# KyleKWKim/LLM-guided-Multimodal-MIL

Hardware: AMD Instinct MI355X
Metric: bags/sec fwd+bwd, N=1024 patches D=512 (higher is better)
Workload: dtype f32; 1 GPU; 32 bags/GPU x 1024 patches x 512 dims, image-only gated-attention MIL fwd+BCE+bwd+allreduce+Adam (BASELINE config 2; x1 GPUs = 32 bags); bags_per_gpu=32, patches=1024, dim=512, global_bags=32, parallelism=dp1, mode=train (dropout 0.5 on patches + 0.25 before the head, in-kernel masks), accum=1, batches_cycled=4, launch=eager

## Files before the change

### include/mil_hip.h

```cpp
#ifndef MIL_HIP_H
#define MIL_HIP_H

#include <stddef.h>
#include <stdint.h>

#ifdef __cplusplus
extern "C" {
#endif

#define MIL_OK 0
#define MIL_EINVAL (-22)
#define MIL_ENOSPC (-28)

#define MIL_GATE_D 192
#define MIL_POOL_TILE 32
#define MIL_LOSS_BCE 0
#define MIL_LOSS_CE_ON_SIGMOID 1
#define MIL_SMALL_ROWS 64

int mil_abi_version(void);

int mil_dropout_keep_bits(uint32_t* bits, int rows, int cols, float p_drop, uint64_t seed, uint64_t offset,
                          const int32_t* offset_dev, void* stream);
int mil_dropout_keep_bits_pair(uint32_t* xbits, int R, uint32_t* mbits, int B, int L, uint64_t seed, uint64_t mseed,
// ... 264 lines not shown
int mil_attn_seq_bwd(const float* q, const float* k, const float* v, int ld, const float* o, const float* dout,
                     const float* lse, const int32_t* q_off, int B, int Tmax, int H, int C, int causal, float* dq,
                     float* dk, float* dv, int ldd, void* stream);
int mil_quickgelu(const float* x, const float* dy, float* out, size_t n, void* stream);
int mil_absorb_query(const float* qp, const float* Wk, int B, int H, int C, int E, float* Qp, void* stream);
int mil_absorb_query_pad(const float* qp, const float* Wk, int B, int H, int C, int E, int T, int THp, float scale,
                         const float* bias, float* Qp, float* cb, void* stream);
int mil_absorb_query_bwd_pad(const float* qp, const float* Wk, const float* dQp, int B, int H, int C, int E, int T, int THp,
                             float scale, const float* bias, const float* dcb, float* dqp, float* dWk, float* dbias,
                             void* stream);
int mil_absorb_query_bwd(const float* qp, const float* Wk, const float* dQp, int B, int H, int C, int E, float* dqp,
                         float* dWk, void* stream);
int mil_absorbed_pool_fwd(const float* keys, const float* pe, const float* Qp, const int32_t* k_off,
                          const int32_t* tile_map, const int32_t* bag_tile_off, int ntiles, int B, int H, int C, int E,
                          float* pooled, float* lse, float* workspace, void* stream);
int mil_absorbed_pool_attn(const float* keys, const float* pe, const float* Qp, const float* lse, const int32_t* k_off,
                           const int32_t* tile_map, int ntiles, int B, int H, int C, int E, float* attn, void* stream);
int mil_absorbed_pool_bwd(const float* keys, const float* pe, const float* Qp, const float* lse, const float* dpooled,
                          const float* pooled, const int32_t* k_off, const int32_t* tile_map,
                          const int32_t* bag_tile_off, int ntiles, int n_keys, int B, int H, int C, int E,
                          const float* dkeys_acc, float* dkeys, float* dQp, float* workspace, void* stream);
int mil_lnbr_absorbed_pool_value_fwd(const float* x, const float* o, const float* gamma, const float* beta, float eps,
                                     const float* pe, const float* Qp, const int32_t* k_off, const int32_t* tile_map,
                                     const int32_t* bag_tile_off, int ntiles, int B, int H, int C, int E, const float* Wv,
                                     const float* bv, float* y, float* stats, float* pooled, float* lse, float* o_attn,
                                     float* workspace, void* stream);
int mil_lnbr_absorbed_pool_bwd(const float* x, const float* o, const float* gamma, const float* beta, const float* stats, const float* y,
                               const float* pe, const float* Qp, const float* lse, const float* dpooled, const float* pooled,
                               const int32_t* k_off, const int32_t* tile_map, const int32_t* bag_tile_off, int ntiles,
                               int n_keys, int B, int H, int C, int E, const float* dy_acc, float* dx, float* d_o,
                               float* dgamma, float* dbeta, float* dQp, float* workspace, void* stream);
int mil_value_proj(const float* pooled, const float* Wv, const float* bv, int B, int H, int C, int E, float* o,
                   void* stream);
int mil_value_proj_pad(const float* pooled, const float* Wv, const float* bv, int B, int H, int C, int E, int T, int THp,
                       float* o, void* stream);
int mil_absorbed_pool_value_fwd(const float* keys, const float* pe, const float* Qp, const int32_t* k_off,
                                const int32_t* tile_map, const int32_t* bag_tile_off, int ntiles, int B, int H, int C, int E,
                                const float* Wv, const float* bv, float* pooled, float* lse, float* o, float* workspace,
                                void* stream);
int mil_value_proj_bwd(const float* dO, const float* Wv, const float* pooled, int B, int H, int C, int E, float* dpooled,
                       float* dWv, float* dbv, void* stream);
int mil_grp_col_softmax(float* S, int ld, const int32_t* grp_off, int G, int max_group_rows, int TH, void* stream);
int mil_grp_col_softmax_bwd(const float* A, const float* dA, int ld, const int32_t* grp_off, int G, int max_group_rows,
                            int TH, float* dS, void* stream);
size_t mil_grp_col_softmax_workspace_floats(int G, int max_group_rows, int ld);
int mil_grp_col_softmax_ws(float* S, int ld, const int32_t* grp_off, int G, int max_group_rows, int TH, float* ws, void* stream);
int mil_grp_col_softmax_bwd_ws(const float* A, const float* dA, int ld, const int32_t* grp_off, int G, int max_group_rows,
                               int TH, float* dS, float* ws, void* stream);
int mil_row_softmax_t(float* S, int ld, int R, int T, int H, void* stream);
int mil_row_softmax_t_bwd(const float* A, const float* dA, int ld, int R, int T, int H, float* dS, void* stream);

int mil_layernorm_fwd(const float* x, const float* gamma, const float* beta, int rows, int E, float eps, float* y,
                      float* stats, void* stream);
int mil_layernorm_bwd_blocks(int rows);
int mil_layernorm_bwd(const float* x, const float* gamma, const float* dy, const float* stats, int rows, int E,
                      float* dx, float* dgamma, float* dbeta, float* workspace, void* stream);
int mil_layernorm_bwd_res(const float* x, const float* gamma, const float* dy, const float* stats, const float* dres,
                          int rows, int E, float* dx, float* dgamma, float* dbeta, float* workspace, void* stream);

int mil_layernorm_bagrow_fwd(const float* x, const float* o, const int32_t* row_bag, const float* gamma, const float* beta,
                             int rows, int E, float eps, float* y, float* stats, void* stream);
int mil_layernorm_bagrow_bwd(const float* x, const float* o, const int32_t* row_bag, const int32_t* row_off, int B,
                             const float* gamma, const float* dy, const float* stats, int rows, int E, float* dx, float* d_o,
                             float* dgamma, float* dbeta, float* workspace, void* stream);
int mil_layernorm_bagrow_rows_per_block(int rows);

int mil_add_pe(const float* x, const float* pe, const int32_t* row_bag, const int32_t* row_off, int rows, int E,
               float* out, void* stream);
int mil_add_bag_row(const float* x, const float* o, const int32_t* row_bag, int rows, int E, float* out,
                    void* stream);
int mil_segment_colsum(const float* Y, const int32_t* row_off, int B, int max_rows, int E, float* out,
                       float* workspace, void* stream);
int mil_ct_map_tokens(const float* ct, int B, int C, int D, int HW, int reduce, float* out, void* stream);
int mil_sinusoid_pe(float* pe, int n, int E, void* stream);

int mil_embed_tokens(const int64_t* ids, const float* table, const float* pos, int nseq, int ctx, int W,
                     float* out, void* stream);
int mil_gather_eot(const int64_t* ids, const float* x, int nseq, int ctx, int W, float* out, void* stream);

int mil_adam_step(float* param, const float* grad, float* exp_avg, float* exp_avg_sq, size_t n,
                  int step, float lr, float beta1, float beta2, float eps, float weight_decay,
                  float grad_scale, void* stream);
int mil_adam_step_counted(float* param, const float* grad, float* exp_avg, float* exp_avg_sq, size_t n,
                          int32_t* step_counter, float lr, float beta1, float beta2, float eps, float weight_decay,
                          float grad_scale, void* stream);
int mil_adam_step_counted_noinc(float* param, const float* grad, float* exp_avg, float* exp_avg_sq, size_t n,
                                const int32_t* step_counter, float lr, float beta1, float beta2, float eps,
                                float weight_decay, float grad_scale, void* stream);

int mil_adam_step_dev(float* param, const float* grad, float* exp_avg, float* exp_avg_sq, size_t n, int32_t* step_counter,
                      const float* lr_dev, float beta1, float beta2, float eps, float weight_decay, float grad_scale,
                      int inc, void* stream);
#define MIL_ADAM_MAX_SEGS 8
int mil_adam_step_dev_segs(float* param, const float* grad, float* exp_avg, float* exp_avg_sq, const size_t* seg_begin,
                           const size_t* seg_end, int nseg, int32_t* step_counter, const float* lr_dev,
                           int32_t* done_counter, float beta1, float beta2, float eps, float weight_decay, float grad_scale,
                           int inc, void* stream);

int mil_sgd_step(float* param, const float* grad, size_t n, float lr, float weight_decay, float grad_scale,
                 void* stream);

#define MIL_STAGE_DROPBITS 0x01u
#define MIL_STAGE_GATE_FWD 0x02u
#define MIL_STAGE_POOL     0x04u
#define MIL_STAGE_TAIL     0x08u
#define MIL_STAGE_GATE_BWD 0x10u
#define MIL_STAGE_REDUCE   0x20u
#define MIL_STAGE_ADAM     0x40u
#define MIL_STAGE_TILEMAP  0x80u
#define MIL_STAGE_ALL      0xffu
#define MIL_STAGE_POOL_FUSED 0x100u
typedef struct mil_image_only_step {
    uint32_t struct_bytes;
    uint32_t stages;
    const void* x;
    const float* y;
    const int32_t* tile_map;
    const int32_t* bag_tile_off;
    int32_t R, L, B, C, T;
    const int32_t* bag_len_dev;
    int32_t* rows_dev;
    int32_t x_bf16;
    float loss_scale;
    int32_t loss_kind;
    int32_t accumulate;
    const float *Wv, *bv, *Wu, *bu, *w, *b, *Wf, *bf;
    const uint16_t *Wv16, *Wu16;
    float *dWv, *dbv, *dWu, *dbu, *dw, *db, *dWf, *dbf;
    float* loss_out;
    float* scores;
    float* gates;
    uint16_t* gates16;
    float* partials;
    float* hrow;
    float* ds;
    float* dw_ws;
    uint64_t dw_ws_floats;
    float *M, *Mdrop, *lse, *logits, *prob, *loss_bag, *dz, *dM, *cdot;
    int32_t train;
    int32_t bf16_grad_mfma;
    uint32_t* xbits;
    uint32_t* mbits;
    uint64_t seed, offset;
    const int32_t* offset_dev;
    float *param_flat, *grad_flat, *exp_avg, *exp_avg_sq;
    uint64_t n_param;
    int32_t adam_step;
    int32_t* adam_step_dev;
    float lr, beta1, beta2, eps, weight_decay, grad_scale;
    const float* lr_dev;
    float* tail_ws;
    int32_t* done_dev;
    const uint16_t* Wp;
} mil_image_only_step;

int mil_image_only_step_run(const mil_image_only_step* a, void* stream);
int mil_image_only_step_time(const mil_image_only_step* a, uint32_t stages, int warm, int iters, float* ms_out,
                             void* stream);

#define MIL_ROUTE_MAIN_R32 0
#define MIL_ROUTE_MAIN_FWD2 1
#define MIL_ROUTE_MAIN_FWD2_PW 2
#define MIL_ROUTE_MAIN_LEGACY 3
#define MIL_ROUTE_TAIL_NONE 0
#define MIL_ROUTE_TAIL_SMALL 1
#define MIL_ROUTE_TAIL_BIG 2
#define MIL_ROUTE_TAIL_KERNEL_NONE 0
#define MIL_ROUTE_TAIL_KERNEL_LINEAR_SMALL 1
#define MIL_ROUTE_TAIL_KERNEL_R32 2
#define MIL_ROUTE_BITS_NONE 0
#define MIL_ROUTE_BITS_GIVEN 1
#define MIL_ROUTE_BITS_IN_KERNEL 2
#define MIL_ROUTE_BITS_GENERATOR 3
#define MIL_ROUTE_DW_KG1 0
#define MIL_ROUTE_DW_KG2 1
#define MIL_ROUTE_DW2 2
typedef struct mil_gate_route {
    int32_t main, rt;
    int32_t tail, tail_rows, tail_kernel, tail_rt;
    int32_t bits, pool_fused;
    int32_t dw, S, kc;
} mil_gate_route;
int mil_gate_step_route(int R, int L, int C, int save_gates, int keep, int pieces, int fused_pool, int bucketed, int ncu,
                        mil_gate_route* out);

#define MIL_GEMM_KERNEL_NT2 0
#define MIL_GEMM_KERNEL_G64 1
#define MIL_GEMM_KERNEL_G64N 2
#define MIL_GEMM_KERNEL_TAIL 3
#define MIL_GEMM_KERNEL_NT 4
#define MIL_GEMM_KERNEL_NN 5
#define MIL_GEMM_KERNEL_TN 6
#define MIL_GEMM_KERNEL_TN2 7
#define MIL_GEMM_KERNEL_TN_AX 8
typedef struct mil_gemm_plan {
    int32_t kernel, S, kchunk;
    int32_t rows_main, main_kernel;
    int32_t rows_honoured;
    uint64_t workspace_floats;
} mil_gemm_plan;
int mil_gemm_route(int M, int N, int K, int a_mode, int b_mode, int lda, int ldb, int ldc, int act, int has_residual,
                   int accumulate, int aux_mode, int has_workspace, int bucketed, int aligned16, int ncu, mil_gemm_plan* out);
int mil_linear_bwd_params_route(int rows, int n_out, int k_in, int lddy, int ldy, int ldx, int aligned16, int ncu,
                                mil_gemm_plan* out);

int mil_cosine_embedding_loss(const float* x1, const float* x2, int B, int E, float scale, float* loss, float* dx1,
                              float* dx2, void* stream);

int mil_build_fusion_segs(const int32_t* len_dev, int B, int P, int cap, int32_t* k_off, int32_t* k_bag, int32_t* tile64,
                          int32_t* bag_tile64_off, int T64, int32_t* tile32, int32_t* bag_tile32_off, int T32,
                          int32_t* row_bag, int32_t* rows_out, float* ds_zero, void* stream);

int mil_build_fusion_segs_tail(const int32_t* len_dev, int B, int nseg, const int32_t* seg_rows, int cap, int32_t* k_off,
                               int32_t* k_bag, int32_t* tile64, int32_t* bag_tile64_off, int T64, int32_t* tile32,
                               int32_t* bag_tile32_off, int T32, int32_t* row_bag, int32_t* rows_out, float* ds_zero,
                               void* stream);

int mil_image_only_step_profile(const mil_image_only_step* a, const uint32_t* groups, int ngroups, int warm, int iters,
                                float* ms_out, void* stream);
int mil_image_only_step_profile_rot(const mil_image_only_step* a, const void* const* xs, const float* const* ys, int nrot,
                                    const uint32_t* groups, int ngroups, int warm, int iters, float* ms_out, void* stream);

int mil_tm_bgemm(const float* A, long sAb, long sAi, long sAk, const float* B, long sBb, long sBk, long sBj, float* C, long sCb,
                 long sCi, long sCj, const float* D, int batch, int M, int N, int K, float alpha, float beta, float diag, int splits,
                 void* stream);
int mil_tm_softmax_rows(float* x, long rows, int cols, void* stream);
int mil_tm_softmax_rows_bwd(const float* p, float* dp, long rows, int cols, void* stream);
int mil_tm_row_gather(const float* src, const float* extra, const int32_t* idx, int rows, int E, float* dst, void* stream);
int mil_tm_row_gather_bwd(const float* ddst, const int32_t* idx, int rows, int E, float* dsrc, float* dextra, void* stream);
int mil_tm_seq_index(const int32_t* len_dev, int B, const int32_t* s_of_bag, int32_t* idx_out, int idx_rows, int32_t* rows_dev_out,
                     int32_t* flag_dev, float* x_tail, int x_rows, int L, void* stream);
int mil_tm_seq_index_segs(const int32_t* table_dev, int B, int total, int x_rows, int32_t* idx_out, int idx_rows, int32_t* flag_dev,
                          void* stream);
int mil_tm_landmarks(const float* qkv, int n_pad, float qscale, float* qL, float* kL, void* stream);
int mil_tm_landmarks_bwd(const float* dqL, const float* dkL, int n_pad, float qscale, float* dqkv, void* stream);
int mil_tm_pinv_init(const float* A2, float* scale, int32_t* arg, float* Z0, void* stream);
int mil_tm_pinv_init_bwd(const float* dZ0, const float* Z0, const float* scale, const int32_t* arg, float* dA2, float* ws,
                         void* stream);
int mil_tm_resconv(const float* qkv, const float* w, int n_pad, float* out, void* stream);
int mil_tm_resconv_bwd(const float* dout, const float* qkv, const float* w, int n_pad, float* dqkv, float* dw, void* stream);
int mil_tm_ppeg_fwd(const float* x, int s, const float* W7, const float* b7, const float* W5, const float* b5, const float* W3,
                    const float* b3, float* y, void* stream);
int mil_tm_ppeg_bwd(const float* dy, const float* x, int s, const float* W7, const float* W5, const float* W3, float* dx,
                    float* dWf, float* db, void* stream);
int mil_tm_cls_attn(const float* A1, const float* Z, const float* A3, int n_pad, int pad, int s, int n, const int32_t* len_dev,
                    int bag, float* t_ws, float* out, void* stream);
size_t mil_tm_lmk_attn_ws_floats(int n_pad, int backward);
int mil_tm_lmk_attn_fwd(const float* qkv, const float* qL, int n_pad, float* W, float* lse, float* ws, void* stream);
int mil_tm_lmk_attn_bwd(const float* qkv, const float* qL, const float* W, const float* lse, const float* dW, int n_pad,
                        float* dqkv, float* dqL, float* ws, void* stream);

#ifdef __cplusplus
}
#endif
#endif
```

### llm-guided-multimodal-mil_amd/_lib.py

```python
from __future__ import annotations

import ctypes
import os
import re
from ctypes import c_long, c_float, c_int, c_int32, c_size_t, c_uint32, c_uint64, c_void_p
from typing import Dict, List, Tuple

_HERE = os.path.dirname(os.path.abspath(__file__))
LIB_PATH = os.path.join(_HERE, "libmil_hip.so")
HEADER_PATH = os.path.join(os.path.dirname(_HERE), "include", "mil_hip.h")
ABI_VERSION = 12

_P = c_void_p
SIGNATURES: Dict[str, Tuple[object, List[object]]] = {
    "mil_abi_version": (c_int, []),
    "mil_dropout_keep_bits": (c_int, [_P, c_int, c_int, c_float, c_uint64, c_uint64, _P, _P]),
    "mil_dropout_keep_bits_pair": (c_int, [_P, c_int, _P, c_int, c_int, c_uint64, c_uint64, c_uint64, _P, _P, _P, c_int, _P]),
    "mil_dropout_apply_bits": (c_int, [_P, _P, c_int, c_int, c_float, _P]),
    "mil_counter_add": (c_int, [_P, c_int, _P]),
    "mil_gate_scores_fwd": (c_int, [_P] * 9 + [c_int, c_int, c_int, _P, c_float, _P]),
    "mil_gate_scores_fwd_draw": (c_int, [_P] * 9 + [c_int, c_int, c_int, _P, c_float, _P, c_int, c_uint64, c_uint64, c_uint64, _P, _P]),
    "mil_attn_pool_fwd": (c_int, [_P] * 4 + [c_int, c_int, c_int, _P, _P, _P, _P, c_float, _P]),
    "mil_bag_softmax": (c_int, [_P] * 3 + [c_int, _P, _P]),
    "mil_attn_pool_partial": (c_int, [_P] * 3 + [c_int, c_int, _P, _P, c_float, _P]),
    "mil_attn_pool_partial_h": (c_int, [_P] * 3 + [c_int, c_int, _P, _P, c_int, _P, _P, c_float, _P, c_float, _P]),
    "mil_attn_pool_bwd_from_h": (c_int, [_P] * 6 + [c_int, c_int, _P, _P]),
    "mil_pool_merge_head": (c_int, [_P] * 2 + [c_int, c_int, c_int, _P, _P, c_int, _P, c_float] + [_P] * 12
                            + [_P, c_float, _P, c_int, _P]),
    "mil_pool_merge_head_ws": (c_int, [_P] * 2 + [c_int, c_int, c_int, _P, _P, c_int, _P, c_float] + [_P] * 12
                               + [_P, c_float, _P, c_int, _P, _P]),
    "mil_pool_tail_workspace_floats": (c_size_t, [c_int]),
    "mil_set_i32": (c_int, [_P, _P, c_int, _P]),
    "mil_head_fwd": (c_int, [_P] * 5 + [c_int, c_int, c_int, _P]),
    "mil_bce_fwd_bwd": (c_int, [_P] * 4 + [c_int, c_int, c_float, _P]),
    "mil_head_bwd": (c_int, [_P] * 8 + [c_int, c_int, c_int, _P]),
    "mil_head_bwd_params": (c_int, [_P] * 4 + [c_int, c_int, c_int, _P, _P, _P]),
    "mil_head_bwd_params_acc": (c_int, [_P] * 4 + [c_int, c_int, c_int, _P, _P, c_int, _P]),
    "mil_clip_contrastive_loss": (c_int, [_P, _P, c_int, c_int, c_int, _P, _P, _P, _P]),
    "mil_cosine_embedding_loss": (c_int, [_P, _P, c_int, c_int, c_float, _P, _P, _P, _P]),
    "mil_rowdot": (c_int, [_P] * 3 + [c_int, c_int, _P]),
    "mil_attn_pool_bwd": (c_int, [_P] * 6 + [c_int, c_int, _P, _P, _P, c_float, _P]),
    "mil_gate_bwd_workspace_floats": (c_size_t, [c_int, c_int]),
    "mil_gate_bwd_params": (c_int, [_P] * 4 + [c_int, c_int, c_int, _P, c_size_t] + [_P] * 6 + [c_int, _P, c_float, _P]),
    "mil_gate_bwd_params_head": (c_int, [_P] * 4 + [c_int, c_int, c_int, _P, c_size_t] + [_P] * 6 + [c_int] + [_P] * 4
                                 + [c_int, c_int, _P, _P, _P, c_float, _P]),
    "mil_gate_bwd_partials": (c_int, [_P] * 4 + [c_int, c_int, c_int, _P, c_size_t, _P, _P]),
    "mil_gate_bwd_partials_rows": (c_int, [_P] * 4 + [c_int, c_int, c_int, _P, c_size_t, _P, _P, _P]),
    "mil_build_tile_map": (c_int, [_P, c_int, _P, _P, _P, c_int, _P]),
    "mil_gate_bwd_reduce": (c_int, [_P, c_int, c_int] + [_P] * 6 + [c_int, c_float, _P]),
    "mil_gate_bwd_reduce_head": (c_int, [_P, c_int, c_int] + [_P] * 6 + [c_int, c_float] + [_P] * 4 + [c_int, c_int, _P, _P, _P]),
    "mil_gate_bwd_reduce_head_adam": (c_int, [_P, c_int, c_int] + [_P] * 6 + [c_int, c_float] + [_P] * 4 + [c_int, c_int, _P, _P]
                                      + [_P, _P, c_size_t, _P, _P, c_int] + [c_float] * 6 + [_P]),
    "mil_gate_bwd_input": (c_int, [_P] * 5 + [c_int, c_int, c_int, _P, _P, c_float, _P]),
    "mil_gate_bwd_input_pool": (c_int, [_P] * 5 + [c_int, c_int, c_int, _P, _P, c_float, _P, _P, _P, _P, _P]),
    "mil_image_only_step_run": (c_int, [_P, _P]),
    "mil_image_only_step_time": (c_int, [_P, c_uint32, c_int, c_int, _P, _P]),
    "mil_gate_step_route": (c_int, [c_int] * 9 + [_P]),
    "mil_gemm_route": (c_int, [c_int] * 16 + [_P]),
    "mil_linear_bwd_params_route": (c_int, [c_int] * 8 + [_P]),
    "mil_image_only_step_profile": (c_int, [_P, _P, c_int, c_int, c_int, _P, _P]),
    "mil_image_only_step_profile_rot": (c_int, [_P, _P, _P, c_int, _P, c_int, c_int, c_int, _P, _P]),
    "mil_patch_drop_select": (c_int, [_P, _P, _P, c_int, c_int, c_uint64, c_uint64, _P, _P]),
    "mil_cohort_feed": (c_int, [_P, _P, _P, _P, _P, _P]),
    "mil_cast_bf16": (c_int, [_P, _P, c_size_t, _P]),
    "mil_gate_pieces": (c_int, [_P, _P, _P, c_int, _P]),
    "mil_gate_scores_fwd_bf16": (c_int, [_P] * 9 + [c_int, c_int, c_int, _P, _P, c_float, _P]),
    "mil_attn_pool_partial_bf16": (c_int, [_P] * 3 + [c_int, c_int, _P, _P, c_float, _P]),
    "mil_attn_pool_partial_h_bf16": (c_int, [_P, _P, _P, c_int, c_int, _P, _P, c_int, _P, _P, c_float, _P, c_float, _P]),
    "mil_attn_pool_bwd_bf16": (c_int, [_P] * 6 + [c_int, c_int, _P, _P, c_float, _P]),
    "mil_gate_bwd_workspace_floats_bf16": (c_size_t, [c_int, c_int]),
    "mil_gate_bwd_params_bf16": (c_int, [_P] * 4 + [c_int, c_int, c_int, _P, c_size_t] + [_P] * 6 + [c_int, _P, c_float, _P]),
    "mil_gate_bwd_params_x16": (c_int, [_P] * 4 + [c_int, c_int, c_int, _P, c_size_t] + [_P] * 6 + [c_int, _P, c_float, _P]),
    "mil_gemm_workspace_floats": (c_size_t, [c_int] * 4),
    "mil_gemm": (c_int, [_P, c_int, c_int, _P, c_int, c_int, _P, c_int, c_int, c_int, c_int, _P, c_int, _P, c_int, c_int,
                         _P, c_size_t, _P]),
    "mil_gemm_rows": (c_int, [_P, c_int, c_int, _P, c_int, c_int, _P, c_int, c_int, c_int, c_int, _P, c_int, _P, c_int, c_int,
                         _P, c_size_t, _P, _P]),
    "mil_gemm_nt2_ok": (c_int, [c_int] * 5),
    "mil_gemm_tn2_ok": (c_int, [c_int] * 6),
    "mil_gemm_tn2_splits": (c_int, [c_int] * 3),
    "mil_gemm_tn2": (c_int, [_P, c_int, _P, c_int, c_int, _P, c_int, c_int, c_int, c_int, _P, _P, _P]),
    "mil_gemm_nt2": (c_int, [_P, c_int, _P, c_int, _P, c_int, c_int, c_int, c_int, _P, c_int, _P]),
    "mil_split_bf16": (c_int, [_P, _P, c_size_t, c_int, _P]),
    "mil_gemm_split": (c_int, [_P, c_int, _P, c_int, c_int, _P, c_int, c_int, c_int, c_int, _P, c_int, _P, c_int, _P, c_int,
                               c_int, _P]),
    "mil_gemm_grouped": (c_int, [_P, c_int, c_int, _P, c_int, c_int, _P, c_int, _P, c_int, c_int, c_int, c_int, c_int,
                                 c_long, c_long, _P, c_long, _P, c_int, _P, c_size_t, _P]),
    "mil_gemm_grouped_pad": (c_int, [_P, c_int, c_int, _P, c_int, c_int, _P, c_int, _P, c_int, c_int, c_int, c_int, c_int,
                                 c_long, c_long, _P, c_long, _P, c_int, _P, c_size_t, c_int, _P]),
    "mil_gemm_grouped_workspace_floats": (c_size_t, [c_int, c_int, c_int, c_int, c_int]),
    "mil_gemm_aux": (c_int, [_P, c_int, c_int, _P, c_int, c_int, _P, c_int, c_int, c_int, c_int, _P, c_int, _P, c_int, c_int,
                         _P, c_size_t, _P, c_int, c_int, _P]),
    "mil_colsum_workspace_floats": (c_size_t, [c_int, c_int]),
    "mil_colsum": (c_int, [_P, c_int, c_int, c_int, _P, c_int, _P, _P]),
    "mil_act_bwd": (c_int, [_P, _P, _P, c_size_t, c_int, _P]),
    "mil_linear_small_fwd": (c_int, [_P, c_int, _P, c_int, _P, c_int, _P, c_int, _P, c_int, c_int, c_int, c_int, _P]),
    "mil_linear_small_bwd": (c_int, [_P, c_int, _P, c_int, c_int, _P, c_int, _P, c_int, _P, c_int, _P, c_int, _P,
                                     c_int, c_int, c_int, _P]),
    "mil_linear_small_fwd_add": (c_int, [_P, c_int, _P, c_int, _P, _P, c_int, _P, c_int, _P, c_int, _P, c_int, c_int, c_int,
                                         c_int, _P]),
    "mil_linear_small_bwd_sum": (c_int, [_P, c_int, _P, _P, _P, _P, _P, c_int, c_int, _P, c_int, _P, c_int, _P, c_int, _P,
                                         c_int, _P, c_int, c_int, c_int, _P]),
    "mil_linear_small_bwd_split": (c_int, [_P, c_int, _P, c_int, c_int, _P, c_int, _P, c_int, c_int, c_int, c_int, _P]),
    "mil_linear_small_ln_bwd5": (c_int, [_P, c_int, _P, c_int, _P, c_int, _P, _P, _P, c_int, _P, _P, _P, c_int, _P, c_int, _P, _P,
                                         _P, c_int, c_int, _P]),
    "mil_sum4": (c_int, [_P, _P, _P, _P, _P, c_int, _P]),
    "mil_linear_small_ln_bwd3": (c_int, [_P, c_int, _P, c_int, _P, c_int, _P, c_int, _P, _P, _P, c_int, _P, c_int, _P, _P, _P,
                                         c_int, c_int, _P]),
    "mil_linear_small_dw_grouped": (c_int, [_P, c_int, _P]),
    "mil_linear_small_ln_fwd": (c_int, [_P, c_int, _P, _P, c_float, _P, c_int, _P, c_int, _P, c_int, _P, c_int, _P, c_int, _P, _P, _P,
                                        c_int, c_int, _P]),
    "mil_linear_small_ln_bwd": (c_int, [_P, c_int, _P, c_int, _P, c_int, _P, _P, _P, c_int, _P, c_int, _P, _P, _P, c_int, c_int, _P]),
    "mil_attn_rows_fwd": (c_int, [_P] * 6 + [c_int] * 4 + [_P, _P, _P]),
    "mil_attn_rows_bwd": (c_int, [_P] * 9 + [c_int] * 4 + [_P] * 4 + [_P]),
    "mil_attn_rows_bwd_general": (c_int, [_P] * 10 + [c_int, c_int, c_int, c_int] + [_P] * 5),
    "mil_attn_pool_fwd_mh": (c_int, [_P] * 6 + [c_int] * 5 + [_P] * 3 + [_P]),
    "mil_attn_pool_bwd_mh": (c_int, [_P] * 9 + [c_int] * 5 + [_P] * 4 + [_P]),
    "mil_attn_seq_fwd": (c_int, [_P] * 3 + [c_int, _P] + [c_int] * 5 + [_P, _P, _P]),
    "mil_attn_seq_bwd": (c_int, [_P] * 3 + [c_int] + [_P] * 4 + [c_int] * 5 + [_P] * 3 + [c_int, _P]),
    "mil_quickgelu": (c_int, [_P, _P, _P, c_size_t, _P]),
    "mil_absorb_query": (c_int, [_P, _P, c_int, c_int, c_int, c_int, _P, _P]),
    "mil_absorb_query_bwd": (c_int, [_P, _P, _P, c_int, c_int, c_int, c_int, _P, _P, _P]),
    "mil_absorb_query_pad": (c_int, [_P, _P, c_int, c_int, c_int, c_int, c_int, c_int, c_float, _P, _P, _P, _P]),
    "mil_absorb_query_bwd_pad": (c_int, [_P, _P, _P, c_int, c_int, c_int, c_int, c_int, c_int, c_float, _P, _P, _P, _P, _P, _P]),
    "mil_absorbed_pool_fwd": (c_int, [_P] * 6 + [c_int] * 5 + [_P] * 3 + [_P]),
    "mil_absorbed_pool_attn": (c_int, [_P] * 6 + [c_int] * 5 + [_P] + [_P]),
    "mil_absorbed_pool_bwd": (c_int, [_P] * 9 + [c_int] * 6 + [_P] * 4 + [_P]),
    "mil_lnbr_absorbed_pool_value_fwd": (c_int, [_P] * 4 + [c_float] + [_P] * 5 + [c_int] * 5 + [_P] * 8 + [_P]),
    "mil_lnbr_absorbed_pool_bwd": (c_int, [_P] * 14 + [c_int] * 6 + [_P] * 7 + [_P]),
    "mil_absorbed_pool_value_fwd": (c_int, [_P] * 6 + [c_int] * 5 + [_P] * 6 + [_P]),
    "mil_value_proj_bwd": (c_int, [_P] * 3 + [c_int] * 4 + [_P] * 3 + [_P]),
    "mil_grp_col_softmax": (c_int, [_P, c_int, _P, c_int, c_int, c_int, _P]),
    "mil_grp_col_softmax_bwd": (c_int, [_P, _P, c_int, _P, c_int, c_int, c_int, _P, _P]),
    "mil_grp_col_softmax_workspace_floats": (c_size_t, [c_int, c_int, c_int]),
    "mil_grp_col_softmax_ws": (c_int, [_P, c_int, _P, c_int, c_int, c_int, _P, _P]),
    "mil_grp_col_softmax_bwd_ws": (c_int, [_P, _P, c_int, _P, c_int, c_int, c_int, _P, _P, _P]),
    "mil_row_softmax_t": (c_int, [_P, c_int, c_int, c_int, c_int, _P]),
    "mil_row_softmax_t_bwd": (c_int, [_P, _P, c_int, c_int, c_int, c_int, _P, _P]),
    "mil_value_proj": (c_int, [_P, _P, _P, c_int, c_int, c_int, c_int, _P, _P]),
    "mil_value_proj_pad": (c_int, [_P, _P, _P, c_int, c_int, c_int, c_int, c_int, c_int, _P, _P]),
    "mil_layernorm_fwd": (c_int, [_P] * 3 + [c_int, c_int, c_float, _P, _P, _P]),
    "mil_layernorm_bwd_blocks": (c_int, [c_int]),
    "mil_layernorm_bwd": (c_int, [_P] * 4 + [c_int, c_int] + [_P] * 4 + [_P]),
    "mil_layernorm_bwd_res": (c_int, [_P] * 5 + [c_int, c_int] + [_P] * 4 + [_P]),
    "mil_layernorm_bagrow_fwd": (c_int, [_P] * 5 + [c_int, c_int, c_float, _P, _P, _P]),
    "mil_layernorm_bagrow_bwd": (c_int, [_P] * 4 + [c_int] + [_P] * 3 + [c_int, c_int] + [_P] * 5 + [_P]),
    "mil_layernorm_bagrow_rows_per_block": (c_int, [c_int]),
    "mil_build_fusion_segs": (c_int, [_P, c_int, c_int, c_int, _P, _P, _P, _P, c_int, _P, _P, c_int, _P, _P, _P, _P]),
    "mil_build_fusion_segs_tail": (c_int, [_P, c_int, c_int, _P, c_int, _P, _P, _P, _P, c_int, _P, _P, c_int, _P, _P, _P, _P]),
    "mil_add_pe": (c_int, [_P] * 4 + [c_int, c_int, _P, _P]),
    "mil_add_bag_row": (c_int, [_P, _P, _P, c_int, c_int, _P, _P]),
    "mil_segment_colsum": (c_int, [_P, _P, c_int, c_int, c_int, _P, _P, _P]),
    "mil_sinusoid_pe": (c_int, [_P, c_int, c_int, _P]),
    "mil_ct_map_tokens": (c_int, [_P, c_int, c_int, c_int, c_int, c_int, _P, _P]),
    "mil_embed_tokens": (c_int, [_P] * 3 + [c_int] * 3 + [_P, _P]),
    "mil_gather_eot": (c_int, [_P, _P, c_int, c_int, c_int, _P, _P]),
    "mil_adam_step": (c_int, [_P] * 4 + [c_size_t, c_int] + [c_float] * 6 + [_P]),
    "mil_adam_step_counted": (c_int, [_P] * 4 + [c_size_t, _P] + [c_float] * 6 + [_P]),
    "mil_adam_step_counted_noinc": (c_int, [_P] * 4 + [c_size_t, _P] + [c_float] * 6 + [_P]),
    "mil_adam_step_dev": (c_int, [_P] * 4 + [c_size_t, _P, _P] + [c_float] * 5 + [c_int, _P]),
    "mil_adam_step_dev_segs": (c_int, [_P] * 4 + [_P, _P, c_int, _P, _P, _P] + [c_float] * 5 + [c_int, _P]),
    "mil_sgd_step": (c_int, [_P, _P, c_size_t] + [c_float] * 3 + [_P]),
    "mil_linear_mid_fwd": (c_int, [_P, c_int, _P, c_int, _P, c_int, _P, c_int, _P, c_int, c_int, c_int, c_int, _P]),
    "mil_linear_mid_bwd": (c_int, [_P, c_int, _P, c_int, c_int, _P, c_int, _P, c_int, _P, c_int, _P, c_int, _P, c_int, c_int,
                                   c_int, _P]),
    "mil_linear_bwd_params_workspace_floats": (c_size_t, [c_int] * 3),
    "mil_linear_bwd_params": (c_int, [_P, c_int, _P, c_int, c_int, _P, c_int, c_int, c_int, c_int, _P, c_int, _P, c_int, _P,
                                      c_size_t, _P]),
    "mil_linear_bwd_params_rows": (c_int, [_P, c_int, _P, c_int, c_int, _P, c_int, c_int, c_int, c_int, _P, c_int, _P, c_int, _P,
                                      c_size_t, _P, _P]),
    "mil_tm_bgemm": (c_int, [_P, c_long, c_long, c_long, _P, c_long, c_long, c_long, _P, c_long, c_long, c_long, _P]
                     + [c_int] * 4 + [c_float] * 3 + [c_int, _P]),
    "mil_tm_softmax_rows": (c_int, [_P, c_long, c_int, _P]),
    "mil_tm_softmax_rows_bwd": (c_int, [_P, _P, c_long, c_int, _P]),
    "mil_tm_row_gather": (c_int, [_P, _P, _P, c_int, c_int, _P, _P]),
    "mil_tm_row_gather_bwd": (c_int, [_P, _P, c_int, c_int, _P, _P, _P]),
    "mil_tm_seq_index": (c_int, [_P, c_int, _P, _P, c_int, _P, _P, _P, c_int, c_int, _P]),
    "mil_tm_seq_index_segs": (c_int, [_P, c_int, c_int, c_int, _P, c_int, _P, _P]),
    "mil_tm_landmarks": (c_int, [_P, c_int, c_float, _P, _P, _P]),
    "mil_tm_landmarks_bwd": (c_int, [_P, _P, c_int, c_float, _P, _P]),
    "mil_tm_pinv_init": (c_int, [_P] * 4 + [_P]),
    "mil_tm_pinv_init_bwd": (c_int, [_P] * 6 + [_P]),
    "mil_tm_resconv": (c_int, [_P, _P, c_int, _P, _P]),
    "mil_tm_resconv_bwd": (c_int, [_P, _P, _P, c_int, _P, _P, _P]),
    "mil_tm_ppeg_fwd": (c_int, [_P, c_int] + [_P] * 7 + [_P]),
    "mil_tm_ppeg_bwd": (c_int, [_P, _P, c_int] + [_P] * 6 + [_P]),
    "mil_tm_cls_attn": (c_int, [_P, _P, _P, c_int, c_int, c_int, c_int, _P, c_int, _P, _P, _P]),
    "mil_tm_lmk_attn_ws_floats": (c_size_t, [c_int, c_int]),
    "mil_tm_lmk_attn_fwd": (c_int, [_P, _P, c_int, _P, _P, _P, _P]),
    "mil_tm_lmk_attn_bwd": (c_int, [_P, _P, _P, _P, _P, c_int, _P, _P, _P, _P]),
}
VALUE_RETURNING = frozenset(n for n, (res, _) in SIGNATURES.items() if res is c_size_t) | frozenset((
    "mil_abi_version", "mil_gemm_nt2_ok", "mil_gemm_tn2_ok", "mil_gemm_tn2_splits", "mil_layernorm_bwd_blocks",
    "mil_layernorm_bagrow_rows_per_block"))

STAGE_DROPBITS, STAGE_GATE_FWD, STAGE_POOL, STAGE_TAIL, STAGE_GATE_BWD, STAGE_REDUCE, STAGE_ADAM = 1, 2, 4, 8, 16, 32, 64
STAGE_TILEMAP = 0x80
STAGE_ALL = 0xff
STAGE_POOL_FUSED = 0x100


class SmallDwDesc(ctypes.Structure):
    _fields_ = [("dy", c_void_p), ("yv", c_void_p), ("x", c_void_p), ("dW", c_void_p), ("db", c_void_p),
                ("lddy", c_int32), ("ldyv", c_int32), ("ldx", c_int32), ("lddw", c_int32), ("act", c_int32),
                ("M", c_int32), ("N", c_int32), ("K", c_int32)]


class GateRoute(ctypes.Structure):
    _fields_ = [(n, c_int32) for n in ("main", "rt", "tail", "tail_rows", "tail_kernel", "tail_rt", "bits", "pool_fused",
                                       "dw", "S", "kc")]


class GemmPlan(ctypes.Structure):
    _fields_ = [(n, c_int32) for n in ("kernel", "S", "kchunk", "rows_main", "main_kernel", "rows_honoured")] + \
               [("workspace_floats", c_uint64)]


GEMM_KERNELS = ("NT2", "G64", "G64N", "TAIL", "NT", "NN", "TN", "TN2", "TN_AX")


SMALL_DW_MAX = 32
FEED_MAX_BAGS, FEED_MAX_AUX = 8, 4


class CohortFeedDesc(ctypes.Structure):
    _fields_ = [("struct_bytes", c_uint32), ("nb", c_int32), ("L", c_int32), ("dst_row0", c_int32), ("dst_bag0", c_int32),
                ("naux", c_int32), ("sel_off", c_int32 * FEED_MAX_BAGS), ("src_row0", c_int32 * FEED_MAX_BAGS),
                ("rows", c_int32 * FEED_MAX_BAGS), ("bag_id", c_int32 * FEED_MAX_BAGS), ("aux_words", c_int32 * FEED_MAX_AUX),
                ("aux_table", c_void_p * FEED_MAX_AUX), ("aux_dst", c_void_p * FEED_MAX_AUX)]


class ImageOnlyStep(ctypes.Structure):
    _fields_ = (
        [("struct_bytes", c_uint32), ("stages", c_uint32),
         ("x", _P), ("y", _P), ("tile_map", _P), ("bag_tile_off", _P),
         ("R", c_int32), ("L", c_int32), ("B", c_int32), ("C", c_int32), ("T", c_int32),
         ("bag_len_dev", _P), ("rows_dev", _P),
         ("x_bf16", c_int32), ("loss_scale", c_float), ("loss_kind", c_int32), ("accumulate", c_int32)]
        + [(n, _P) for n in ("Wv", "bv", "Wu", "bu", "w", "b", "Wf", "bf", "Wv16", "Wu16")]
        + [(n, _P) for n in ("dWv", "dbv", "dWu", "dbu", "dw", "db", "dWf", "dbf", "loss_out")]
        + [(n, _P) for n in ("scores", "gates", "gates16", "partials", "hrow", "ds", "dw_ws")]
        + [("dw_ws_floats", c_uint64)]
        + [(n, _P) for n in ("M", "Mdrop", "lse", "logits", "prob", "loss_bag", "dz", "dM", "cdot")]
        + [("train", c_int32), ("bf16_grad_mfma", c_int32), ("xbits", _P), ("mbits", _P), ("seed", c_uint64),
           ("offset", c_uint64), ("offset_dev", _P)]
        + [(n, _P) for n in ("param_flat", "grad_flat", "exp_avg", "exp_avg_sq")]
        + [("n_param", c_uint64), ("adam_step", c_int32), ("adam_step_dev", _P)]
        + [(n, c_float) for n in ("lr", "beta1", "beta2", "eps", "weight_decay", "grad_scale")]
        + [("lr_dev", _P), ("tail_ws", _P), ("done_dev", _P), ("Wp", _P)])


_lib = None
_checked = _checked_of = None


class MilHipError(RuntimeError):
    pass


def header_symbols() -> List[str]:
    text = open(HEADER_PATH).read()
    text = re.sub(r"/\*.*?\*/", "", text, flags=re.S)
    return sorted(set(re.findall(r"\b(mil_[a-z0-9_]+)\s*\(", text)))


def lib() -> ctypes.CDLL:
    global _lib
    if _lib is None:
        path = os.environ.get("MIL_HIP_LIB") or LIB_PATH
        if not os.path.exists(path):
            raise MilHipError(
                f"{path} is missing: the HIP library is not built and there is no fallback path. "
                "Run __graft_entry__.build() or `make -C llm-guided-multimodal-mil_amd/csrc`.")
        import torch
        handle = ctypes.CDLL(path, mode=ctypes.RTLD_GLOBAL)
        for name, (res, args) in SIGNATURES.items():
            fn = getattr(handle, name)
            fn.restype = res
            fn.argtypes = args
        got = handle.mil_abi_version()
        if got != ABI_VERSION:
            raise MilHipError(f"libmil_hip.so ABI {got} != expected {ABI_VERSION}")
        _lib = handle
    return _lib


def _raise_on_status(result, func, args):
    if result != 0:
        check(result, func.__name__)
    return result


def checked() -> ctypes.CDLL:
    global _checked, _checked_of
    if _checked_of is not _lib or _lib is None:
        raw = lib()
        handle = ctypes.CDLL(raw._name, mode=ctypes.RTLD_GLOBAL)
        for name, (res, args) in SIGNATURES.items():
            fn = getattr(handle, name)
            fn.restype = res
            fn.argtypes = args
            if name not in VALUE_RETURNING:
                fn.errcheck = _raise_on_status
        _checked, _checked_of = handle, raw
    return _checked


SHIM_DIR = os.path.join(_HERE, "csrc", "shim_build")
SHIM_SRC = os.path.join(_HERE, "csrc", "torch_shim.cpp")
_shim = False


def build_shim(verbose: bool = False):
    from torch.utils.cpp_extension import load
    os.makedirs(SHIM_DIR, exist_ok=True)
    return load(name="mil_torch_shim", sources=[SHIM_SRC], extra_ldflags=[f"-L{_HERE}", "-lmil_hip", f"-Wl,-rpath,{_HERE}"],
                extra_cflags=["-O2"], build_directory=SHIM_DIR, with_cuda=False, verbose=verbose)


def shim():
    global _shim
    if _shim is False:
        _shim = None
        path = os.path.join(SHIM_DIR, "mil_torch_shim.so")
        if os.environ.get("MIL_TORCH_SHIM", "0") == "1" and os.path.exists(path) and not os.environ.get("MIL_HIP_LIB"):
            import importlib.util
            lib()
            try:
                spec = importlib.util.spec_from_file_location("mil_torch_shim", path)
                mod = importlib.util.module_from_spec(spec)
                spec.loader.exec_module(mod)
                if mod.abi_version() == ABI_VERSION:
                    _shim = mod
            except (ImportError, OSError, AttributeError):
                _shim = None
    return _shim


def check(rc: int, what: str) -> None:
    if rc != 0:
        kind = {-22: "invalid argument (MIL_EINVAL)", -28: "workspace too small (MIL_ENOSPC)"}.get(
            rc, f"hipError {rc}" if rc > 0 else f"error {rc}")
        raise MilHipError(f"{what}: {kind}")
```

### llm-guided-multimodal-mil_amd/csrc/gate_fwd.hip

```cpp
#include "mil_internal.h"
#include "philox.h"
#include <type_traits>

#define GF_TM 128
#define GF_BK 32

typedef __attribute__((address_space(3))) void lds_void;
typedef __attribute__((address_space(3))) const f32x4 lds_cf4;
typedef __attribute__((address_space(3))) f32x4 lds_f4;
typedef __attribute__((address_space(3))) float lds_f32;

struct GateFwdCoord {
    int tid, lane, wave;
    int wr, wc;
    int r, h;
    int row0, rows_here;
    unsigned lds0;
};
template <bool UNIFORM_WAVE = true>
__device__ __forceinline__ GateFwdCoord gate_fwd_coord(const float* smem, int R) {
    GateFwdCoord co;
    co.tid = threadIdx.x;
    co.lane = co.tid & 63;
    co.wave = UNIFORM_WAVE ? __builtin_amdgcn_readfirstlane(co.tid >> 6) : co.tid >> 6;
    co.wr = co.wave >> 1;
    co.wc = co.wave & 1;
    co.r = co.lane & 31;
    co.h = co.lane >> 5;
    co.row0 = blockIdx.x * GF_TM;
    co.rows_here = min(GF_TM, R - co.row0);
    co.lds0 = (unsigned)(uintptr_t)(lds_void*)smem;
    return co;
}

__device__ __forceinline__ void gate_acc_clear(f32x16 (&acc)[3][2]) {
#pragma unroll
    for (int c = 0; c < 3; ++c)
#pragma unroll
        for (int u = 0; u < 2; ++u)
#pragma unroll
            for (int i = 0; i < 16; ++i) acc[c][u][i] = 0.f;
}

#define GF_SRED_OFF 0
#define GF_SC_OFF (2 * GF_TM)
#define GF_PRED_OFF 1024
#define GF_PRED_FLOATS(NQ) (4 * 2 * (NQ) * 256)
static_assert(GF_SRED_OFF + 2 * GF_TM <= GF_SC_OFF && GF_SC_OFF + GF_TM <= GF_PRED_OFF, "epilogue LDS regions overlap");

template <bool DROP>
__device__ __forceinline__ void gate_fwd_scores_epilogue(const GateFwdCoord co, const f32x16 (&acc)[3][2], const float* bv,
                                                         const float* bu, const float* wvec, const float* battn,
                                                         float* scores, float* gates, int R, float xscale, lds_f32* smem,
                                                         bool copy_scores) {
    float part[16];
#pragma unroll
    for (int i = 0; i < 16; ++i) part[i] = 0.f;
#pragma unroll
    for (int c = 0; c < 3; ++c) {
        const int d = 32 * (3 * co.wc + c) + co.r;
        const float bvd = bv[d], bud = bu[d], wd = wvec[d];
#pragma unroll
        for (int i = 0; i < 16; ++i) {
            const float v = fast_tanh(DROP ? fmaf(acc[c][0][i], xscale, bvd) : acc[c][0][i] + bvd);
            const float u = fast_sigmoid(DROP ? fmaf(acc[c][1][i], xscale, bud) : acc[c][1][i] + bud);
            part[i] += wd * v * u;
            if (gates != nullptr) {
                const int gr = co.row0 + 32 * co.wr + mfma32_row(i, co.h);
                if (gr < R) {
                    gates[(size_t)gr * GF_NG + d] = v;
                    gates[(size_t)gr * GF_NG + 192 + d] = u;
                }
            }
        }
    }
    lds_f32* sred = smem + GF_SRED_OFF;
#pragma unroll
    for (int i = 0; i < 16; ++i) {
        const float v = half_sum_lane31(part[i]);
        if (co.r == 31) sred[co.wc * GF_TM + 32 * co.wr + mfma32_row(i, co.h)] = v;
    }
    __syncthreads();
    if (co.tid < GF_TM) {
        const int gr = co.row0 + co.tid;
        const float sc = sred[co.tid] + sred[GF_TM + co.tid] + battn[0];
        if (gr < R) scores[gr] = sc;
        if (copy_scores) smem[GF_SC_OFF + co.tid] = gr < R ? sc : -INFINITY;
    }
}

template <bool DROP>
__global__ __launch_bounds__(512) void k_gate_fwd(const float* __restrict__ x, const float* __restrict__ Wv,
                                                       const float* __restrict__ bv, const float* __restrict__ Wu,
                                                       const float* __restrict__ bu, const float* __restrict__ wvec,
                                                       const float* __restrict__ battn, float* __restrict__ scores,
                                                       float* __restrict__ gates, int R, int L,
                                                       const uint32_t* __restrict__ xbits, float xscale) {
    __shared__ __attribute__((aligned(16))) float smem[2 * (GF_TM + GF_NG) * 32];
    float* xs = smem;
    float* ws = smem + 2 * GF_TM * 32;
    const GateFwdCoord co = gate_fwd_coord<false>(smem, R);
    const int lane = co.lane, wave = co.wave, wr = co.wr, wc = co.wc, r = co.r, h = co.h, row0 = co.row0;
    const int prow = lane >> 3, pch = lane & 7;
    const float* gsrc[8];
    int ldst[8];
#pragma unroll
    for (int i = 0; i < 8; ++i) {
        if (i < 2) {
            const int lr = (2 * wave + i) * 8 + prow;
            const int gr = min(row0 + lr, R - 1);
            gsrc[i] = x + (size_t)gr * L + 4 * (pch ^ ((lr >> 1) & 7));
            ldst[i] = (2 * wave + i) * 8 * 32;
        } else {
            const int wrow = (6 * wave + (i - 2)) * 8 + prow;
            gsrc[i] = (wrow < 192 ? Wv + (size_t)wrow * L : Wu + (size_t)(wrow - 192) * L) + 4 * (pch ^ ((wrow >> 1) & 7));
            ldst[i] = (6 * wave + (i - 2)) * 8 * 32;
        }
    }
    auto dma_piece = [&](int i, int buf, int k0) {
        float* dst = (i < 2 ? xs + buf * GF_TM * 32 : ws + buf * GF_NG * 32) + ldst[i];
        __builtin_amdgcn_global_load_lds(gsrc[i] + k0, (lds_void*)dst, 16, 0, 0);
    };
    f32x16 acc[3][2];
    gate_acc_clear(acc);

    const int nslice = L / GF_BK;
    const uint32_t* mrow = nullptr;
    unsigned mnext = 0;
    if (DROP) {
        mrow = xbits + (size_t)min(row0 + 32 * wr + r, R - 1) * nslice;
        mnext = mrow[0];
    }
#pragma unroll
    for (int i = 0; i < 8; ++i) dma_piece(i, 0, 0);
    __syncthreads();
    const int fx = (r >> 1) & 7;
    for (int s = 0; s < nslice; ++s) {
        const int buf = s & 1;
        const int k1 = min(s + 1, nslice - 1) * GF_BK;
        unsigned mcur = 0;
        if (DROP) {
            mcur = mnext >> (4 * h);
            mnext = mrow[min(s + 1, nslice - 1)];
        }
        const float* xa = xs + (buf * GF_TM + 32 * wr + r) * 32;
        const float* wb = ws + (buf * GF_NG + 32 * 3 * wc + r) * 32;
        f32x4 a[2], b[2][3][2];
        auto frag_piece = [&](int t, int q, int p) {
            const int ch = 4 * ((2 * t + h) ^ fx);
            if (p == 0) {
                a[q] = *reinterpret_cast<const f32x4*>(xa + ch);
            } else {
                const int c = (p - 1) >> 1, u = (p - 1) & 1;
                b[q][c][u] = *reinterpret_cast<const f32x4*>(wb + (u * 192 + 32 * c) * 32 + ch);
            }
        };
#pragma unroll
        for (int p = 0; p < 7; ++p) frag_piece(0, 0, p);
#pragma unroll
        for (int t = 0; t < 4; ++t) {
            const int q = t & 1;
#pragma unroll
            for (int j = 0; j < 4; ++j) {
                const int g = 4 * t + j;
                if (g < 8) dma_piece(g, buf ^ 1, k1);
                if (t < 3) {
                    frag_piece(t + 1, q ^ 1, 2 * j);
                    if (2 * j + 1 < 7) frag_piece(t + 1, q ^ 1, 2 * j + 1);
                }
                const float av = DROP ? keep_if(a[q][j], mcur, 8 * t + j) : a[q][j];
#pragma unroll
                for (int c = 0; c < 3; ++c)
#pragma unroll
                    for (int u = 0; u < 2; ++u)
                        acc[c][u] = __builtin_amdgcn_mfma_f32_32x32x2f32(av, b[q][c][u][j], acc[c][u], 0, 0, 0);
                __builtin_amdgcn_sched_barrier(0);
            }
        }
        __syncthreads();
    }
    gate_fwd_scores_epilogue<DROP>(co, acc, bv, bu, wvec, battn, scores, gates, R, xscale, (lds_f32*)smem, false);
}

#define GF2_XS_BYTES (GF_TM * 32 * 4)
#define GF2_WS_BYTES (GF_NG * 32 * 4)
#define GP_XS_BYTES (GF_TM * 16 * 4)
#define GP_WS_BYTES (GP_SLICE_ELEMS * 2)
constexpr int gate_fwd2_smem_floats(bool pw) { return pw ? 2 * (GP_XS_BYTES + GP_WS_BYTES) / 4 : 2 * (GF2_XS_BYTES + GF2_WS_BYTES) / 4; }
static_assert(GF_PRED_OFF + GF_PRED_FLOATS(2) <= gate_fwd2_smem_floats(false) &&
                  GF_PRED_OFF + GF_PRED_FLOATS(2) <= gate_fwd2_smem_floats(true),
              "the epilogue / pool regions must fit the LDS image of either K loop");

struct GateFwdGen {
    uint32_t* xbits_out;
    uint32_t* mbits_out;
    int B;
    uint32_t seed_lo, seed_hi, mseed_lo, mseed_hi;
    uint64_t offset;
    const int32_t* offset_dev;
};

template <bool DROP, bool GEN>
struct GateKeepWords {
    uint32_t* mlds;
    __amdgpu_buffer_rsrc_t srd_m;
    int vmask;
    unsigned w0;
    uint64_t off;

    __device__ __forceinline__ void init(const GateFwdCoord co, const uint32_t* xbits, const GateFwdGen& gen, uint32_t* lds,
                                         int L) {
        const int nslice = L / GF_BK;
        mlds = lds;
        vmask = 0;
        w0 = 0;
        off = 0;
        if (DROP && !GEN) {
            srd_m = __builtin_amdgcn_make_buffer_rsrc((void*)(xbits + (size_t)co.row0 * nslice), 0, co.rows_here * nslice * 4,
                                                      MIL_SRD_FLAGS);
            vmask = (32 * co.wr + co.r) * nslice * 4;
            w0 = __builtin_amdgcn_raw_buffer_load_b32(srd_m, vmask, 0, 0);
        }
        if (GEN) {
            off = gen.offset;
            if (gen.offset_dev != nullptr) off += (uint64_t)(uint32_t)gen.offset_dev[0];
            const size_t blk0 = (size_t)co.row0 * nslice / 4;
            const int nblk = co.rows_here * nslice / 4;
            for (int q = co.tid; q < nblk; q += 512) {
                const uint4 wds = philox_keep_words_half(blk0 + q, off, gen.seed_lo, gen.seed_hi);
                *reinterpret_cast<uint4*>(gen.xbits_out + 4 * (blk0 + q)) = wds;
                *reinterpret_cast<uint4*>(mlds + 4 * q) = wds;
            }
            if (blockIdx.x == 0 && gen.mbits_out != nullptr) {
                const int nw = gen.B * (L >> 5);
                for (int q = co.tid; 2 * q < nw; q += 512) {
                    const uint2 wds = philox_keep_words_quarter((uint64_t)q, off, gen.mseed_lo, gen.mseed_hi);
                    gen.mbits_out[2 * q] = wds.x;
                    gen.mbits_out[2 * q + 1] = wds.y;
                }
// ... 66 lines not shown
            mnext = kw.word(s1);
        }
        f32x4 a[2], b[2][3][2];
        auto frag_piece = [&](int t, int q, int p) {
            if (p == 0) {
                a[q] = *(lds_cf4*)(uintptr_t)(fa_addr[t] + (unsigned)(buf * GF2_XS_BYTES));
            } else {
                const int c = (p - 1) >> 1, u = (p - 1) & 1;
                b[q][c][u] = *(lds_cf4*)(uintptr_t)(fb_addr[buf][t] + (unsigned)((u * 192 + 32 * c) * 128));
            }
        };
#pragma unroll
        for (int p = 0; p < 7; ++p) frag_piece(0, 0, p);
#pragma unroll
        for (int t = 0; t < 4; ++t) {
            const int q = t & 1;
#pragma unroll
            for (int j = 0; j < 4; ++j) {
                const int g = 4 * t + j;
                if (g < 8) dma_piece(g, buf ^ 1, k1bytes);
                if (t < 3) {
                    frag_piece(t + 1, q ^ 1, 2 * j);
                    if (2 * j + 1 < 7) frag_piece(t + 1, q ^ 1, 2 * j + 1);
                }
                const float av = DROP ? keep_if(a[q][j], mcur, 8 * t + j) : a[q][j];
#pragma unroll
                for (int c = 0; c < 3; ++c)
#pragma unroll
                    for (int u = 0; u < 2; ++u)
                        acc[c][u] = __builtin_amdgcn_mfma_f32_32x32x2f32(av, b[q][c][u][j], acc[c][u], 0, 0, 0);
                __builtin_amdgcn_sched_barrier(0);
            }
        }
    };
    int s = 0;
    for (; s + 1 < nslice; s += 2) {
        slice(s, std::integral_constant<int, 0>{});
        __syncthreads();
        slice(s + 1, std::integral_constant<int, 1>{});
        __syncthreads();
    }
    if (s < nslice) {
        slice(s, std::integral_constant<int, 0>{});
        __syncthreads();
    }
}

template <bool DROP, bool GEN>
__device__ __forceinline__ void gate_kloop_pw(const GateFwdCoord co, const GateKeepWords<DROP, GEN>& kw, const float* x,
                                              const unsigned short* Wp, int L, f32x16 (&acc)[3][2]) {
    const int lane = co.lane, wave = co.wave, wr = co.wr, wc = co.wc, r = co.r, h = co.h;
    const unsigned lds0 = co.lds0;
    const int nslice = L / GF_BK, n16 = L / 16;
    const __amdgpu_buffer_rsrc_t srd_x =
        __builtin_amdgcn_make_buffer_rsrc((void*)(x + (size_t)co.row0 * L), 0, co.rows_here * L * 4, MIL_SRD_FLAGS);
    const __amdgpu_buffer_rsrc_t srd_p = __builtin_amdgcn_make_buffer_rsrc((void*)Wp, 0, n16 * GP_WS_BYTES, MIL_SRD_FLAGS);
    const int xrow = 16 * wave + (lane >> 2);
    const int xsrc = (xrow * L + 4 * ((lane & 3) ^ ((xrow >> 2) & 3))) * 4;
    auto dma16 = [&](int buf, int s16) {
        const unsigned xdst = lds0 + (unsigned)(buf * GP_XS_BYTES + wave * 1024);
        __builtin_amdgcn_raw_ptr_buffer_load_lds(srd_x, (lds_void*)(uintptr_t)xdst, 16, xsrc, s16 * 64, 0, 0);
#pragma unroll
        for (int i = 0; i < 5; ++i) {
            const int p = wave + 8 * i;
            if (i < 4 || p < 36) {
                const unsigned wdst = lds0 + (unsigned)(2 * GP_XS_BYTES + buf * GP_WS_BYTES + p * 1024);
                __builtin_amdgcn_raw_ptr_buffer_load_lds(srd_p, (lds_void*)(uintptr_t)wdst, 16, lane * 16,
                                                         s16 * GP_WS_BYTES + p * 1024, 0, 0);
            }
        }
    };
    const unsigned xr = (unsigned)((32 * wr + r) * 64);
    const unsigned pa0 = xr + 16u * (unsigned)((2 * h) ^ ((r >> 2) & 3));
    const unsigned pa1 = xr + 16u * (unsigned)((2 * h + 1) ^ ((r >> 2) & 3));
    const unsigned pb = (unsigned)(2 * GP_XS_BYTES + (h * GF_NG + 96 * wc + r) * 16);
    auto slice16 = [&](int s16, unsigned mw, auto buf_c) {
        constexpr int buf = decltype(buf_c)::value;
        const f32x4 xa0 = *(lds_cf4*)(uintptr_t)(lds0 + pa0 + (unsigned)(buf * GP_XS_BYTES));
        const f32x4 xa1 = *(lds_cf4*)(uintptr_t)(lds0 + pa1 + (unsigned)(buf * GP_XS_BYTES));
        f32x4 bq[3][3][2];
#pragma unroll
        for (int q = 2; q >= 0; --q)
#pragma unroll
            for (int c = 0; c < 3; ++c)
#pragma unroll
                for (int u = 0; u < 2; ++u)
                    bq[q][c][u] = *(lds_cf4*)(uintptr_t)(lds0 + pb + (unsigned)(buf * GP_WS_BYTES + (q * 2 * GF_NG + u * 192 + 32 * c) * 16));
        dma16(buf ^ 1, min(s16 + 1, n16 - 1));
        gp_bf16x8 ap[3];
#pragma unroll
        for (int j = 0; j < 8; ++j) {
            float v = j < 4 ? xa0[j] : xa1[j - 4];
            if (DROP) v = keep_if(v, mw, j);
            unsigned short p0, p1, p2;
            gp_split3(v, p0, p1, p2);
            ap[0][j] = __builtin_bit_cast(__bf16, p0);
            ap[1][j] = __builtin_bit_cast(__bf16, p1);
            ap[2][j] = __builtin_bit_cast(__bf16, p2);
        }
        constexpr int TP[6] = {0, 1, 2, 0, 1, 0}, TQ[6] = {2, 1, 0, 1, 0, 0};
#pragma unroll
        for (int t = 0; t < 6; ++t)
#pragma unroll
            for (int c = 0; c < 3; ++c)
#pragma unroll
                for (int u = 0; u < 2; ++u)
                    acc[c][u] = __builtin_amdgcn_mfma_f32_32x32x16_bf16(ap[TP[t]], __builtin_bit_cast(gp_bf16x8, bq[TQ[t]][c][u]),
                                                                        acc[c][u], 0, 0, 0);
        __builtin_amdgcn_sched_barrier(0);
    };
    dma16(0, 0);
    __syncthreads();
    unsigned mnext = kw.first();
    for (int s = 0; s < nslice; ++s) {
        unsigned mw = 0;
        if (DROP) {
            mw = mnext;
            mnext = kw.word(min(s + 1, nslice - 1));
        }
        slice16(2 * s, mw >> (8 * h), std::integral_constant<int, 0>{});
        __syncthreads();
        slice16(2 * s + 1, mw >> (16 + 8 * h), std::integral_constant<int, 1>{});
        __syncthreads();
    }
}

struct GateFwdPool {
    const int32_t* tile_map;
    float* partials;
    int T;
    const float* Wf;
    float* hrow;
    const uint32_t* mbits;
    float mscale;
};
template <int NQ>
struct GatePoolRows {
    f32x4 v[2][MIL_POOL_TILE / 4][NQ];
};
template <int NQ>
__device__ __forceinline__ void gate_pool_request_rows(const GateFwdCoord co, const float* x, int R, int L, GatePoolRows<NQ>& pv) {
    const int trow0 = co.row0 + 32 * co.wr;
    if (trow0 < R) {
#pragma unroll
        for (int j = 0; j < 2; ++j)
#pragma unroll
            for (int i = 0; i < MIL_POOL_TILE / 4; ++i) {
                const float* xr = x + (size_t)(trow0 + 2 * co.wc + j + 4 * i) * L + 4 * co.lane;
#pragma unroll
                for (int q = 0; q < NQ; ++q) pv.v[j][i][q] = *reinterpret_cast<const f32x4*>(xr + 256 * q);
            }
    }
}
template <bool DROP, bool GEN, int NQ>
__device__ __forceinline__ void gate_fwd_pool_pass(const GateFwdCoord co, const GateKeepWords<DROP, GEN>& kw, GatePoolRows<NQ>& pv,
                                                   const uint32_t* xbits, int R, int L, float xscale, const GateFwdGen& gen,
                                                   const GateFwdPool& pool, lds_f32* smem) {
    const int lane = co.lane, wr = co.wr, wc = co.wc;
    const int nslice = L / GF_BK;
    const lds_f32* sc_lds = smem + GF_SC_OFF;
    lds_f32* pred = smem + GF_PRED_OFF;
    __syncthreads();
    const int trow0 = co.row0 + 32 * wr;
    const bool live = trow0 < R;
    const int t = trow0 >> 5;
    const float s_ = lane < 32 ? sc_lds[32 * wr + lane] : -INFINITY;
    const float m_ = wave_allmax(s_);
    const float p_ = lane < 32 ? expf(s_ - m_) : 0.f;
    const float l_ = wave_allsum(p_);
    const float xs = DROP ? xscale : 1.0f;
    f32x4 pacc[2][NQ];
    if (live) {
        auto& v = pv.v;
        const int sh = 4 * (lane & 7);
        if (DROP) {
#pragma unroll
            for (int j = 0; j < 2; ++j)
#pragma unroll
                for (int i = 0; i < MIL_POOL_TILE / 4; ++i) {
                    const int rr = 2 * wc + j + 4 * i;
#pragma unroll
                    for (int q = 0; q < NQ; ++q) {
                        const unsigned wd = GEN ? kw.mlds[(32 * wr + rr) * nslice + 8 * q + (lane >> 3)]
                                                : xbits[(size_t)(trow0 + rr) * (L >> 5) + 8 * q + (lane >> 3)];
                        const unsigned mm = wd >> sh;
#pragma unroll
                        for (int e = 0; e < 4; ++e) v[j][i][q][e] = keep_if(v[j][i][q][e], mm, e);
                    }
                }
        }
#pragma unroll
        for (int j = 0; j < 2; ++j) {
#pragma unroll
            for (int q = 0; q < NQ; ++q) pacc[j][q] = f32x4{0, 0, 0, 0};
#pragma unroll
            for (int i = 0; i < MIL_POOL_TILE / 4; ++i) {
                const int rr = 2 * wc + j + 4 * i;
                const float pw = __int_as_float(__builtin_amdgcn_readlane(__float_as_int(p_), rr)) * xs;
#pragma unroll
                for (int q = 0; q < NQ; ++q) pacc[j][q] += pw * v[j][i][q];
            }
        }
        const int bag_ = pool.tile_map[4 * t];
        f32x4 wf[2][NQ];
#pragma unroll
        for (int c = 0; c < 2; ++c)
#pragma unroll
            for (int q = 0; q < NQ; ++q) {
                f32x4 w = *reinterpret_cast<const f32x4*>(pool.Wf + (size_t)c * L + 256 * q + 4 * lane) * xs;
                if (DROP) {
                    const int widx = bag_ * (L >> 5) + 8 * q + (lane >> 3);
                    unsigned wd;
                    if (GEN) {
                        const uint2 pr = philox_keep_words_quarter((uint64_t)(widx >> 1), kw.off, gen.mseed_lo, gen.mseed_hi);
                        wd = (widx & 1) ? pr.y : pr.x;
                    } else {
                        wd = pool.mbits[widx];
                    }
                    const unsigned mm = wd >> sh;
#pragma unroll
                    for (int e = 0; e < 4; ++e) w[e] = keep_if(w[e], mm, e) * pool.mscale;
                }
                wf[c][q] = w;
            }
#pragma unroll
        for (int j = 0; j < 2; ++j) {
            float d16[16];
#pragma unroll
            for (int c = 0; c < 2; ++c)
#pragma unroll
                for (int i = 0; i < MIL_POOL_TILE / 4; ++i) {
                    float d = 0.f;
#pragma unroll
                    for (int q = 0; q < NQ; ++q)
                        d += v[j][i][q][0] * wf[c][q][0] + v[j][i][q][1] * wf[c][q][1] + v[j][i][q][2] * wf[c][q][2] + v[j][i][q][3] * wf[c][q][3];
                    d16[2 * i + c] = d;
                }
            const float tot = wave_reduce16(d16, lane);
            const int k = wave_reduce16_index(lane), rr = 2 * wc + j + 4 * (k >> 1);
            if ((lane & 3) == 0) pool.hrow[(size_t)(trow0 + rr) * 2 + (k & 1)] = tot;
        }
        if (wc == 1) {
#pragma unroll
            for (int j = 0; j < 2; ++j)
#pragma unroll
                for (int q = 0; q < NQ; ++q)
                    *(lds_f4*)(pred + ((wr * 2 + j) * NQ + q) * 256 + 4 * lane) = pacc[j][q];
        }
    }
    __syncthreads();
    if (live && wc == 0) {
        float* out = pool.partials + (size_t)t * L;
#pragma unroll
        for (int q = 0; q < NQ; ++q) {
            f32x4 vv = pacc[0][q];
            vv += pacc[1][q];
            vv += *(lds_cf4*)(pred + ((wr * 2 + 0) * NQ + q) * 256 + 4 * lane);
            vv += *(lds_cf4*)(pred + ((wr * 2 + 1) * NQ + q) * 256 + 4 * lane);
            *reinterpret_cast<f32x4*>(out + 256 * q + 4 * lane) = vv;
        }
        if (lane == 0) {
            float* ml = pool.partials + (size_t)pool.T * L + 2 * t;
            ml[0] = m_;
            ml[1] = l_;
        }
    }
}

template <bool DROP, bool GEN, int PQ, bool PW = false>
__global__ __launch_bounds__(512) void k_gate_fwd2(const float* __restrict__ x, const float* __restrict__ Wv,
                                                   const float* __restrict__ bv, const float* __restrict__ Wu,
                                                   const float* __restrict__ bu, const float* __restrict__ wvec,
                                                   const float* __restrict__ battn, float* __restrict__ scores,
                                                   float* __restrict__ gates, int R, int L,
                                                   const uint32_t* __restrict__ xbits, float xscale, GateFwdGen gen,
                                                   GateFwdPool pool, const unsigned short* __restrict__ Wp = nullptr) {
    __shared__ __attribute__((aligned(16))) float smem[gate_fwd2_smem_floats(PW)];
    __shared__ __attribute__((aligned(16))) uint32_t mlds[GEN ? GF_TM * 32 : 4];
    const GateFwdCoord co = gate_fwd_coord(smem, R);
    GateKeepWords<DROP, GEN> kw;
    kw.init(co, xbits, gen, mlds, L);
    f32x16 acc[3][2];
    gate_acc_clear(acc);
    if constexpr (PW) gate_kloop_pw<DROP, GEN>(co, kw, x, Wp, L, acc);
    else gate_kloop_f32<DROP, GEN>(co, kw, x, Wv, Wu, L, acc);
    GatePoolRows<(PQ > 0 ? PQ : 1)> pv;
    if constexpr (PQ > 0) gate_pool_request_rows(co, x, R, L, pv);
    gate_fwd_scores_epilogue<DROP>(co, acc, bv, bu, wvec, battn, scores, gates, R, xscale, (lds_f32*)smem, PQ > 0);
    if constexpr (PQ > 0) gate_fwd_pool_pass<DROP, GEN, PQ>(co, kw, pv, xbits, R, L, xscale, gen, pool, (lds_f32*)smem);
}

#define GS_TM 32
#define GS_LS 36
#define GS_THREADS 768
template <bool DROP, int RT>
__global__ __launch_bounds__(GS_THREADS) void k_gate_fwd_r32(const float* __restrict__ x, const float* __restrict__ Wv,
                                                             const float* __restrict__ bv, const float* __restrict__ Wu,
                                                             const float* __restrict__ bu, const float* __restrict__ wvec,
                                                             const float* __restrict__ battn, float* __restrict__ scores,
                                                             float* __restrict__ gates, int R, int L,
                                                             const uint32_t* __restrict__ xbits, float xscale,
                                                             const int32_t* __restrict__ rows_dev) {
    constexpr int TM = GS_TM * RT;
    if (rows_dev != nullptr && (int)(blockIdx.x * TM) >= __builtin_amdgcn_readfirstlane(rows_dev[0])) return;
    __shared__ __attribute__((aligned(16))) float smem[2 * (TM + GF_NG) * GS_LS];
    float* xs = smem;
    float* ws = smem + 2 * TM * GS_LS;
    const int tid = threadIdx.x, lane = tid & 63, wave = tid >> 6;
    const int c = wave >> 1, isu = wave & 1;
    const int r = lane & 31, h = lane >> 5;
    const int row0 = blockIdx.x * TM;
    const float* wsrc[4];
    int wdst[4];
#pragma unroll
    for (int i = 0; i < 4; ++i) {
        const int id = tid + GS_THREADS * i, wrow = id >> 3, ch = id & 7;
        wsrc[i] = (wrow < 192 ? Wv + (size_t)wrow * L : Wu + (size_t)(wrow - 192) * L) + 4 * ch;
        wdst[i] = wrow * GS_LS + 4 * ch;
    }
    const int xrow = (tid % (256 * RT)) >> 3, xch = tid & 7;
    const float* xsrc = x + (size_t)min(row0 + xrow, R - 1) * L + 4 * xch;
    const uint32_t* msrc = DROP ? xbits + (size_t)min(row0 + xrow, R - 1) * (L / 32) : nullptr;
    const int xdst = xrow * GS_LS + 4 * xch;
    f32x4 wreg[2][4], xreg[2];
    unsigned mreg[2] = {0, 0};
    auto gload = [&](int set, int k0) {
#pragma unroll
        for (int i = 0; i < 4; ++i) wreg[set][i] = *reinterpret_cast<const f32x4*>(wsrc[i] + k0);
        xreg[set] = *reinterpret_cast<const f32x4*>(xsrc + k0);
        if (DROP) mreg[set] = msrc[k0 >> 5];
    };
    auto swrite = [&](int set, int buf) {
#pragma unroll
        for (int i = 0; i < 4; ++i) *reinterpret_cast<f32x4*>(ws + buf * GF_NG * GS_LS + wdst[i]) = wreg[set][i];
        if (tid < 256 * RT) {
            f32x4 v = xreg[set];
            if (DROP) {
                const unsigned m = mreg[set] >> (4 * xch);
#pragma unroll
                for (int e = 0; e < 4; ++e) v[e] = keep_if(v[e], m, e) * xscale;
            }
            *reinterpret_cast<f32x4*>(xs + buf * TM * GS_LS + xdst) = v;
        }
    };
    f32x16 acc[RT];
#pragma unroll
    for (int q = 0; q < RT; ++q)
#pragma unroll
        for (int i = 0; i < 16; ++i) acc[q][i] = 0.f;
    const int nslice = L / GF_BK;
    gload(0, 0);
    swrite(0, 0);
    gload(1, min(1, nslice - 1) * GF_BK);
    gload(0, min(2, nslice - 1) * GF_BK);
    __syncthreads();
    auto iteration = [&](int s, int set) {
        const int buf = s & 1;
        const float* xa = xs + buf * TM * GS_LS + r * GS_LS + 4 * h;
        const float* wb = ws + buf * GF_NG * GS_LS + (192 * isu + 32 * c + r) * GS_LS + 4 * h;
        f32x4 fa[RT][4], fb[4];
#pragma unroll
        for (int t = 0; t < 4; ++t) {
#pragma unroll
            for (int q = 0; q < RT; ++q) fa[q][t] = *reinterpret_cast<const f32x4*>(xa + q * GS_TM * GS_LS + 8 * t);
            fb[t] = *reinterpret_cast<const f32x4*>(wb + 8 * t);
        }
        swrite(set, buf ^ 1);
        gload(set, min(s + 3, nslice - 1) * GF_BK);
        __builtin_amdgcn_sched_barrier(0);
#pragma unroll
        for (int t = 0; t < 4; ++t)
#pragma unroll
            for (int jj = 0; jj < 4; ++jj)
#pragma unroll
                for (int q = 0; q < RT; ++q) acc[q] = __builtin_amdgcn_mfma_f32_32x32x2f32(fa[q][t][jj], fb[t][jj], acc[q], 0, 0, 0);
        __syncthreads();
    };
    for (int s = 0; s < nslice; s += 2) {
        iteration(s, 1);
        if (s + 1 < nslice) iteration(s + 1, 0);
    }
    const int d = 32 * c + r;
    float* uex = smem;
    float* sred = smem + 6 * 32 * 33;
#pragma unroll
    for (int q = 0; q < RT; ++q) {
        float gv[16];
        if (q > 0) __syncthreads();
        if (isu) {
            const float bud = bu[d];
#pragma unroll
            for (int i = 0; i < 16; ++i) {
                gv[i] = fast_sigmoid(acc[q][i] + bud);
                uex[(c * 32 + mfma32_row(i, h)) * 33 + r] = gv[i];
            }
        } else {
            const float bvd = bv[d];
#pragma unroll
            for (int i = 0; i < 16; ++i) gv[i] = fast_tanh(acc[q][i] + bvd);
        }
        if (gates != nullptr) {
#pragma unroll
            for (int i = 0; i < 16; ++i) {
                const int gr = row0 + GS_TM * q + mfma32_row(i, h);
                if (gr < R) gates[(size_t)gr * GF_NG + 192 * isu + d] = gv[i];
            }
        }
        __syncthreads();
        if (!isu) {
            const float wd = wvec[d];
#pragma unroll
            for (int i = 0; i < 16; ++i) {
                const int lr = mfma32_row(i, h);
                const float part = half_allsum(wd * gv[i] * uex[(c * 32 + lr) * 33 + r]);
                if (r == 0) sred[c * GS_TM + lr] = part;
            }
        }
        __syncthreads();
        if (tid < GS_TM && row0 + GS_TM * q + tid < R) {
            float sc = battn[0];
#pragma unroll
            for (int cc = 0; cc < 6; ++cc) sc += sred[cc * GS_TM + tid];
            scores[row0 + GS_TM * q + tid] = sc;
        }
    }
}

__global__ __launch_bounds__(64) void k_gate_tail_scores(const float* __restrict__ gates, const float* __restrict__ wvec,
                                                         const float* __restrict__ battn, float* __restrict__ scores) {
    const int row = blockIdx.x, lane = threadIdx.x;
    const float* gr = gates + (size_t)row * GF_NG;
    float v = 0.f;
#pragma unroll
    for (int q = 0; q < 3; ++q) v += wvec[64 * q + lane] * gr[64 * q + lane] * gr[192 + 64 * q + lane];
    v = wave_allsum(v);
    if (lane == 0) scores[row] = v + battn[0];
}

struct GateRouteIn {
    int R, L;
    bool save_gates;
    int keep;
    bool pieces;
    bool fused_pool;
};
int gate_tail_rows(int R, int tiles_per_round) {
    const int tail = R % GF_TM, full = R / GF_TM;
    return (tail >= 1 && tail <= MIL_SMALL_ROWS && full >= tiles_per_round && full % tiles_per_round == 0) ? tail : 0;
}
static inline int gate_r32_rt(int rows, int ncu) {
    const int tiles = (rows + GS_TM - 1) / GS_TM;
    return tiles <= ncu ? 1 : tiles <= 2 * ncu ? 2 : 3;
}
static mil_gate_route gate_route_plan(const GateRouteIn& in, int ncu) {
    const int R = in.R, L = in.L;
    mil_gate_route p{};
    const bool r32 = (R + GF_TM - 1) / GF_TM < (3 * ncu) / 4;
    const bool fwd2 = L <= 4096;
    p.main = r32 ? MIL_ROUTE_MAIN_R32 : !fwd2 ? MIL_ROUTE_MAIN_LEGACY : in.pieces ? MIL_ROUTE_MAIN_FWD2_PW : MIL_ROUTE_MAIN_FWD2;
    p.rt = r32 ? gate_r32_rt(R, ncu) : 0;
    if (!r32) {
        const int few = in.save_gates ? gate_tail_rows(R, ncu) : 0, per_round = GF_TM * ncu, over = R % per_round;
        if (few > 0) {
            p.tail = MIL_ROUTE_TAIL_SMALL;
            p.tail_rows = few;
        } else if (R >= per_round && over > 0 && over <= 1024) {
            p.tail = MIL_ROUTE_TAIL_BIG;
            p.tail_rows = over;
        }
    }
    if (p.tail != MIL_ROUTE_TAIL_NONE) {
        const bool small_linear = p.tail == MIL_ROUTE_TAIL_SMALL && in.keep == MIL_ROUTE_BITS_NONE;
        p.tail_kernel = small_linear ? MIL_ROUTE_TAIL_KERNEL_LINEAR_SMALL : MIL_ROUTE_TAIL_KERNEL_R32;
        p.tail_rt = small_linear ? 0 : gate_r32_rt(p.tail_rows, ncu);
    }
    const bool all_fwd2 = !r32 && p.tail == MIL_ROUTE_TAIL_NONE && fwd2;
    p.bits = in.keep == MIL_ROUTE_BITS_NONE || in.keep == MIL_ROUTE_BITS_GIVEN ? in.keep
             : all_fwd2 && L <= 1024 && (L % 128) == 0 ? MIL_ROUTE_BITS_IN_KERNEL : MIL_ROUTE_BITS_GENERATOR;
    p.pool_fused = in.fused_pool && all_fwd2 && L == 512 && (R % 32) == 0;
    p.dw = -1;
    if ((L % 128) == 0) {
        const GateDwPlan d = gate_dw_plan(R, L, ncu);
        p.dw = d.dw;
        p.S = d.S;
        p.kc = d.kc;
    }
    return p;
}

extern "C" int mil_gate_step_route(int R, int L, int C, int save_gates, int keep, int pieces, int fused_pool, int bucketed,
                                   int ncu, mil_gate_route* out) {
    if (!out || R <= 0 || L <= 0 || (L % GF_BK) != 0 || C <= 0) return MIL_EINVAL;
    if (keep != MIL_ROUTE_BITS_NONE && keep != MIL_ROUTE_BITS_GIVEN) keep = MIL_ROUTE_BITS_GENERATOR;
    (void)bucketed;
    *out = gate_route_plan(GateRouteIn{R, L, save_gates != 0, keep, pieces != 0, fused_pool != 0}, ncu > 0 ? ncu : MIL_NUM_CU);
    return MIL_OK;
}

using GateFwdR32Kernel = decltype(&k_gate_fwd_r32<false, 1>);
static const GateFwdR32Kernel GATE_FWD_R32_KERNELS[2][3] = {
    {k_gate_fwd_r32<false, 1>, k_gate_fwd_r32<false, 2>, k_gate_fwd_r32<false, 3>},
    {k_gate_fwd_r32<true, 1>, k_gate_fwd_r32<true, 2>, k_gate_fwd_r32<true, 3>}};
using GateFwd2Kernel = decltype(&k_gate_fwd2<false, false, 0, false>);
static const GateFwd2Kernel GATE_FWD2_KERNELS[3][2][2] = {
    {{k_gate_fwd2<false, false, 0, false>, k_gate_fwd2<false, false, 0, true>}, {k_gate_fwd2<false, false, 2, false>, k_gate_fwd2<false, false, 2, true>}},
    {{k_gate_fwd2<true, false, 0, false>, k_gate_fwd2<true, false, 0, true>}, {k_gate_fwd2<true, false, 2, false>, k_gate_fwd2<true, false, 2, true>}},
    {{k_gate_fwd2<true, true, 0, false>, k_gate_fwd2<true, true, 0, true>}, {k_gate_fwd2<true, true, 2, false>, k_gate_fwd2<true, true, 2, true>}}};

static int launch_gate_fwd_r32(const float* x, const float* Wv, const float* bv, const float* Wu, const float* bu,
                               const float* w, const float* b, float* scores, float* gates, int R, int L,
                               const uint32_t* xbits, float xscale, int rt, hipStream_t st, const int32_t* rows_dev = nullptr) {
    const dim3 grid((R + GS_TM * rt - 1) / (GS_TM * rt));
    const float xs = xbits ? xscale : 1.0f;
    hipLaunchKernelGGL(GATE_FWD_R32_KERNELS[xbits != nullptr][rt <= 1 ? 0 : rt == 2 ? 1 : 2], grid, dim3(GS_THREADS), 0, st, x, Wv, bv, Wu, bu, w, b, scores,
                       gates, R, L, xbits, xs, rows_dev);
    MIL_CHECK_LAUNCH();
    return MIL_OK;
}
static void launch_gate_fwd2(bool draw, bool pool_fused, bool pw, dim3 grid, hipStream_t st, const float* x, const float* Wv,
                             const float* bv, const float* Wu, const float* bu, const float* w, const float* b, float* scores,
                             float* gates, int R, int L, const uint32_t* xbits, float xs, const GateFwdGen& gen,
                             const GateFwdPool& pool, const uint16_t* Wp) {
    hipLaunchKernelGGL(GATE_FWD2_KERNELS[draw ? 2 : xbits ? 1 : 0][pool_fused][pw], grid, dim3(512), 0, st, x, Wv, bv, Wu, bu, w, b,
                       scores, gates, R, L, xbits, xs, gen, pool, pw ? (const unsigned short*)Wp : nullptr);
}

static int gate_scores_fwd_impl(const float* x, const float* Wv, const float* bv, const float* Wu, const float* bu,
                                const float* w, const float* b, float* scores, float* gates, int R, int L, int D,
                                const uint32_t* xbits, float xscale, const GateFwdGen* gen, void* stream,
                                const GateFwdPool* pool = nullptr, int* fused = nullptr, const int32_t* rows_dev = nullptr,
                                const TileMapJob* tmap = nullptr, const uint16_t* Wp = nullptr) {
    if (!x || !Wv || !bv || !Wu || !bu || !w || !b || !scores) return MIL_EINVAL;
    if (D != MIL_GATE_D || L <= 0 || (L % GF_BK) != 0 || R < 0) return MIL_EINVAL;
    if (R == 0) return MIL_OK;
    hipStream_t st = (hipStream_t)stream;
    if (fused != nullptr) *fused = 0;
    const bool pool_ok = pool != nullptr && fused != nullptr && pool->T * MIL_POOL_TILE == R && pool->tile_map &&
                         pool->partials && pool->Wf && pool->hrow &&
                         (gen ? gen->mbits_out != nullptr : (xbits != nullptr) == (pool->mbits != nullptr));
    const int keep = gen ? MIL_ROUTE_BITS_GENERATOR : xbits ? MIL_ROUTE_BITS_GIVEN : MIL_ROUTE_BITS_NONE;
    const mil_gate_route p = gate_route_plan(GateRouteIn{R, L, gates != nullptr, keep, Wp != nullptr, pool_ok}, MIL_NUM_CU);

    int rc = MIL_OK;
    if (p.bits == MIL_ROUTE_BITS_GENERATOR) {
        const uint64_t seed = ((uint64_t)gen->seed_hi << 32) | gen->seed_lo, mseed = ((uint64_t)gen->mseed_hi << 32) | gen->mseed_lo;
        if (gen->mbits_out != nullptr && tmap != nullptr) {
            rc = dropout_keep_bits_pair_tilemap(gen->xbits_out, R, gen->mbits_out, gen->B, L, seed, mseed, gen->offset,
                                                gen->offset_dev, *tmap, stream);
            tmap = nullptr;
        } else if (gen->mbits_out != nullptr)
            rc = dropout_keep_bits_pair(gen->xbits_out, R, gen->mbits_out, gen->B, L, seed, mseed, gen->offset, gen->offset_dev, stream);
        else
            rc = mil_dropout_keep_bits(gen->xbits_out, R, L, 0.5f, seed, gen->offset, gen->offset_dev, stream);
        if (rc != MIL_OK) return rc;
        xbits = gen->xbits_out;
    }
    if (tmap != nullptr) {
        rc = mil_build_tile_map(tmap->bag_len, tmap->B, tmap->tile_map, tmap->bag_tile_off, tmap->rows_out, tmap->T_cap, stream);
        if (rc != MIL_OK) return rc;
    }
    if (p.main == MIL_ROUTE_MAIN_R32)
        return launch_gate_fwd_r32(x, Wv, bv, Wu, bu, w, b, scores, gates, R, L, xbits, xscale, p.rt, st, rows_dev);

    const bool draw = p.bits == MIL_ROUTE_BITS_IN_KERNEL;
    if (draw) xbits = gen->xbits_out;
    const int Rm = R - p.tail_rows;
    const dim3 grid((Rm + GF_TM - 1) / GF_TM);
    const float xs = xbits ? xscale : 1.0f;
    if (p.main == MIL_ROUTE_MAIN_LEGACY) {
        hipLaunchKernelGGL(xbits ? k_gate_fwd<true> : k_gate_fwd<false>, grid, dim3(512), 0, st, x, Wv, bv, Wu, bu, w, b, scores, gates,
                           Rm, L, xbits, xs);
    } else {
        const GateFwdGen fgen = draw ? *gen : GateFwdGen{};
        const GateFwdPool fpool = p.pool_fused ? *pool : GateFwdPool{};
        launch_gate_fwd2(draw, p.pool_fused, p.main == MIL_ROUTE_MAIN_FWD2_PW, grid, st, x, Wv, bv, Wu, bu, w, b, scores, gates, Rm, L,
                         xbits, xs, fgen, fpool, Wp);
    }
    if (p.pool_fused) *fused = 1;
    MIL_CHECK_LAUNCH();
    if (p.tail_kernel == MIL_ROUTE_TAIL_KERNEL_R32)
        return launch_gate_fwd_r32(x + (size_t)Rm * L, Wv, bv, Wu, bu, w, b, scores + Rm,
                                   gates ? gates + (size_t)Rm * GF_NG : nullptr, p.tail_rows, L,
                                   xbits ? xbits + (size_t)Rm * (L / 32) : nullptr, xscale, p.tail_rt, st);
    if (p.tail_kernel == MIL_ROUTE_TAIL_KERNEL_LINEAR_SMALL) {
        const float* xt = x + (size_t)Rm * L;
        float* gt = gates + (size_t)Rm * GF_NG;
        rc = mil_linear_small_fwd(xt, L, Wv, L, bv, 1 , nullptr, 0, gt, GF_NG, p.tail_rows, MIL_GATE_D, L, stream);
        if (rc != MIL_OK) return rc;
        rc = mil_linear_small_fwd(xt, L, Wu, L, bu, 4 , nullptr, 0, gt + MIL_GATE_D, GF_NG, p.tail_rows, MIL_GATE_D, L,
                                  stream);
        if (rc != MIL_OK) return rc;
        hipLaunchKernelGGL(k_gate_tail_scores, dim3(p.tail_rows), dim3(64), 0, st, gt, w, b, scores + Rm);
        MIL_CHECK_LAUNCH();
    }
    return MIL_OK;
}

extern "C" int mil_gate_scores_fwd(const float* x, const float* Wv, const float* bv, const float* Wu, const float* bu,
                                   const float* w, const float* b, float* scores, float* gates, int R, int L, int D,
                                   const uint32_t* xbits, float xscale, void* stream) {
    return gate_scores_fwd_impl(x, Wv, bv, Wu, bu, w, b, scores, gates, R, L, D, xbits, xscale, nullptr, stream);
}

static GateFwdGen gate_fwd_gen(uint32_t* xbits_out, uint32_t* mbits_out, int B, uint64_t seed, uint64_t mseed, uint64_t offset,
                               const int32_t* offset_dev) {
    GateFwdGen g{};
    g.xbits_out = xbits_out;
    g.mbits_out = mbits_out;
    g.B = B;
    g.seed_lo = (uint32_t)seed;
    g.seed_hi = (uint32_t)(seed >> 32);
    g.mseed_lo = (uint32_t)mseed;
    g.mseed_hi = (uint32_t)(mseed >> 32);
    g.offset = offset;
    g.offset_dev = offset_dev;
    return g;
}

extern "C" int mil_gate_scores_fwd_draw(const float* x, const float* Wv, const float* bv, const float* Wu, const float* bu,
                                        const float* w, const float* b, float* scores, float* gates, int R, int L, int D,
                                        uint32_t* xbits_out, float xscale, uint32_t* mbits_out, int B, uint64_t seed,
                                        uint64_t mseed, uint64_t offset, const int32_t* offset_dev, void* stream) {
    if (!xbits_out || (L % 64) != 0 || (mbits_out && B <= 0)) return MIL_EINVAL;
    const GateFwdGen gen = gate_fwd_gen(xbits_out, mbits_out, B, seed, mseed, offset, offset_dev);
    return gate_scores_fwd_impl(x, Wv, bv, Wu, bu, w, b, scores, gates, R, L, D, nullptr, xscale, &gen, stream);
}

int gate_fwd_rows_dev(const float* x, const float* Wv, const float* bv, const float* Wu, const float* bu, const float* w,
                      const float* b, float* scores, float* gates, int R, int L, int draw, uint32_t* xbits, float xscale,
                      uint32_t* mbits, int B, uint64_t seed, uint64_t mseed, uint64_t offset, const int32_t* offset_dev,
                      const int32_t* rows_dev, void* stream, const TileMapJob* tmap, const uint16_t* Wp) {
    if (draw && (!xbits || (L % 64) != 0 || (mbits && B <= 0))) return MIL_EINVAL;
    const GateFwdGen gen = gate_fwd_gen(xbits, mbits, B, seed, mseed, offset, offset_dev);
    return gate_scores_fwd_impl(x, Wv, bv, Wu, bu, w, b, scores, gates, R, L, MIL_GATE_D, draw ? nullptr : xbits, xscale,
                                draw ? &gen : nullptr, stream, nullptr, nullptr, rows_dev, tmap, Wp);
}

int gate_fwd_with_pool(const float* x, const float* Wv, const float* bv, const float* Wu, const float* bu, const float* w,
                       const float* b, float* scores, float* gates, int R, int L, int draw, uint32_t* xbits, float xscale,
                       uint32_t* mbits, float mscale, int B, uint64_t seed, uint64_t mseed, uint64_t offset,
                       const int32_t* offset_dev, const int32_t* tile_map, int T, float* partials, const float* Wf, float* hrow,
                       int* fused, void* stream, const uint16_t* Wp) {
    if (draw && (!xbits || !mbits || (L % 64) != 0 || B <= 0)) return MIL_EINVAL;
    GateFwdPool pl{};
    pl.tile_map = tile_map;
    pl.partials = partials;
    pl.T = T;
    pl.Wf = Wf;
    pl.hrow = hrow;
    pl.mbits = draw ? nullptr : mbits;
    pl.mscale = mscale;
    const GateFwdGen gen = gate_fwd_gen(xbits, mbits, B, seed, mseed, offset, offset_dev);
    return gate_scores_fwd_impl(x, Wv, bv, Wu, bu, w, b, scores, gates, R, L, MIL_GATE_D, draw ? nullptr : xbits, xscale,
                                draw ? &gen : nullptr, stream, &pl, fused, nullptr, nullptr, Wp);
}

__global__ __launch_bounds__(256) void k_gate_pieces(const float* __restrict__ Wv, const float* __restrict__ Wu,
                                                     unsigned short* __restrict__ Wp, int L) {
    const int L4 = L / 4;
    const int idx = blockIdx.x * 256 + threadIdx.x;
    if (idx >= GF_NG * L4) return;
    const int n = idx / L4, k = 4 * (idx % L4);
    const float* src = (n < MIL_GATE_D ? Wv + (size_t)n * L : Wu + (size_t)(n - MIL_GATE_D) * L) + k;
    gp_store4(Wp, n, k, *reinterpret_cast<const f32x4*>(src));
}

extern "C" int mil_gate_pieces(const float* Wv, const float* Wu, uint16_t* Wp, int L, void* stream) {
    if (!Wv || !Wu || !Wp || L <= 0 || (L % 32) != 0) return MIL_EINVAL;
    if ((reinterpret_cast<uintptr_t>(Wv) | reinterpret_cast<uintptr_t>(Wu) | reinterpret_cast<uintptr_t>(Wp)) & 15) return MIL_EINVAL;
    hipLaunchKernelGGL(k_gate_pieces, dim3((GF_NG * (L / 4) + 255) / 256), dim3(256), 0, (hipStream_t)stream, Wv, Wu,
                       (unsigned short*)Wp, L);
    MIL_CHECK_LAUNCH();
    return MIL_OK;
}
```

### llm-guided-multimodal-mil_amd/csrc/head_loss.hip

```cpp
#include "mil_common.h"

template <int NT>
__device__ __forceinline__ float block_allsum_nt(float v, float* red) {
    const int tid = threadIdx.x;
    v = wave_allsum(v);
    __syncthreads();
    if ((tid & 63) == 0) red[tid >> 6] = v;
    __syncthreads();
    float t = red[0];
#pragma unroll
    for (int w = 1; w < NT / 64; ++w) t += red[w];
    return t;
}
__device__ __forceinline__ float block_allsum_256(float v, float* red) {
    const int tid = threadIdx.x;
    v = wave_allsum(v);
    __syncthreads();
    if ((tid & 63) == 0) red[tid >> 6] = v;
    __syncthreads();
    return red[0] + red[1] + red[2] + red[3];
}

__global__ __launch_bounds__(256) void k_head_fwd(const float* __restrict__ M, const float* __restrict__ Wf,
                                                  const float* __restrict__ bf, float* __restrict__ z,
                                                  float* __restrict__ p, int L, int C) {
    __shared__ float red[4];
    const int b = blockIdx.x, tid = threadIdx.x;
    for (int c = 0; c < C; ++c) {
        float v = 0.f;
        for (int j = tid; j < L; j += 256) v += M[(size_t)b * L + j] * Wf[(size_t)c * L + j];
        v = block_allsum_256(v, red);
        if (tid == 0) {
            const float zz = v + bf[c];
            z[b * C + c] = zz;
            p[b * C + c] = 1.0f / (1.0f + expf(-zz));
        }
    }
}

__global__ __launch_bounds__(256) void k_bce_fwd_bwd(const float* __restrict__ p, const float* __restrict__ y,
                                                     float* __restrict__ loss_sum, float* __restrict__ dz, int n,
                                                     float scale) {
    __shared__ float red[4];
    float acc = 0.f;
    for (int i = threadIdx.x; i < n; i += 256) {
        const float pi = p[i], yi = y[i];
        const float lp = fmaxf(logf(pi), -100.0f);
        const float l1p = fmaxf(logf(1.0f - pi), -100.0f);
        acc += -(yi * lp + (1.0f - yi) * l1p);
        dz[i] = (pi - yi) * scale;
    }
    acc = block_allsum_256(acc, red);
    if (threadIdx.x == 0) atomicAdd(loss_sum, acc * scale);
}

__global__ __launch_bounds__(256) void k_head_bwd_dm(const float* __restrict__ dz_or_dp, const float* __restrict__ p,
                                                     const float* __restrict__ M, const float* __restrict__ Wf,
                                                     float* __restrict__ dM, float* __restrict__ cdot, int L, int C) {
    __shared__ float red[4];
    __shared__ float dzs[32];
    const int b = blockIdx.x, tid = threadIdx.x;
    if (tid < C) {
        float g = dz_or_dp[b * C + tid];
        if (p != nullptr) { const float pp = p[b * C + tid]; g = g * pp * (1.0f - pp); }
        dzs[tid] = g;
    }
    __syncthreads();
    float dot = 0.f;
    for (int j = tid; j < L; j += 256) {
        float v = 0.f;
        for (int c = 0; c < C; ++c) v += dzs[c] * Wf[(size_t)c * L + j];
        dM[(size_t)b * L + j] = v;
        dot += v * M[(size_t)b * L + j];
    }
    dot = block_allsum_256(dot, red);
    if (tid == 0) cdot[b] = dot;
}

__global__ __launch_bounds__(256) void k_head_bwd_params(const float* __restrict__ dz_or_dp, const float* __restrict__ p,
                                                         const float* __restrict__ M, float* __restrict__ dWf,
                                                         float* __restrict__ dbf, int B, int L, int C,
                                                         const float* __restrict__ loss_bag, float* __restrict__ loss_out,
                                                         int accumulate) {
    __shared__ float red[4][64];
    const int nlb = (L + 63) / 64;
    const int lane = threadIdx.x & 63, g = threadIdx.x >> 6;
    if ((int)blockIdx.x < C * nlb) {
        const int c = blockIdx.x / nlb, j = (blockIdx.x % nlb) * 64 + lane;
        float v = 0.f;
        if (j < L)
            for (int b = g; b < B; b += 4) {
                float gz = dz_or_dp[b * C + c];
                if (p != nullptr) { const float pp = p[b * C + c]; gz = gz * pp * (1.0f - pp); }
                v += gz * M[(size_t)b * L + j];
            }
        red[g][lane] = v;
        __syncthreads();
        if (g == 0 && j < L) {
            const float t = red[0][lane] + red[1][lane] + red[2][lane] + red[3][lane];
            dWf[(size_t)c * L + j] = accumulate ? dWf[(size_t)c * L + j] + t : t;
        }
    } else {
        if ((int)threadIdx.x < C) {
            const int c = threadIdx.x;
            float v = 0.f;
            for (int b = 0; b < B; ++b) {
                float gz = dz_or_dp[b * C + c];
                if (p != nullptr) { const float pp = p[b * C + c]; gz = gz * pp * (1.0f - pp); }
                v += gz;
            }
            dbf[c] = accumulate ? dbf[c] + v : v;
        }
        if (loss_bag != nullptr && g == 1) {
            float v = 0.f;
            for (int b = lane; b < B; b += 64) v += loss_bag[b];
            v = wave_allsum(v);
            if (lane == 0) loss_out[0] = accumulate ? loss_out[0] + v : v;
        }
    }
}


template <int AD_U>
__global__ __launch_bounds__(256) void k_adam(float* __restrict__ param, const float* __restrict__ grad,
                                              float* __restrict__ m, float* __restrict__ v, size_t n, float lr, float b1,
                                              float b2, float eps, float wd, float gscale, float bc1, float bc2_sqrt,
                                              const int* __restrict__ step_dev, const float* __restrict__ lr_dev) {
    __shared__ float bc[2];
    if (step_dev != nullptr) {
        if (threadIdx.x == 0) {
            const double st = (double)(*step_dev + 1);
            bc[0] = (float)(1.0 - pow((double)b1, st));
            bc[1] = (float)sqrt(1.0 - pow((double)b2, st));
        }
        __syncthreads();
        bc1 = bc[0];
        bc2_sqrt = bc[1];
    }
    if (lr_dev != nullptr) lr = *lr_dev;
    const float lr_bc1 = lr / bc1;
    const size_t base = (size_t)blockIdx.x * (256 * 4 * AD_U);
    if (base + 256 * 4 * AD_U <= n) {
        f32x4 p4[AD_U], g4[AD_U], m4[AD_U], v4[AD_U];
#pragma unroll
        for (int u = 0; u < AD_U; ++u) {
            const size_t i = base + ((size_t)u * 256 + threadIdx.x) * 4;
            p4[u] = *reinterpret_cast<const f32x4*>(param + i);
            g4[u] = *reinterpret_cast<const f32x4*>(grad + i);
            m4[u] = *reinterpret_cast<const f32x4*>(m + i);
            v4[u] = *reinterpret_cast<const f32x4*>(v + i);
        }
#pragma unroll
        for (int u = 0; u < AD_U; ++u) {
// ... 703 lines not shown
#pragma unroll
    for (int i = 0; i < 5; ++i) sums[i] = wave_allsum(sums[i]);
    if (lane == 0)
#pragma unroll
        for (int i = 0; i < 5; ++i) red[wv][1 + i] = sums[i];
    __syncthreads();
    if (tid < 6) {
        float* o = ws + ((size_t)b * TAIL_S_MAX + s) * 8;
        o[tid] = tid == 0 ? m : (red[0][tid] + red[1][tid]) + (red[2][tid] + red[3][tid]);
    }
}

__global__ __launch_bounds__(256) void k_tail_apply(const float* __restrict__ partials, const int32_t* __restrict__ bag_tile_off,
                                                    int T, int L, const float* __restrict__ Wf, const float* __restrict__ bf,
                                                    int C, const float* __restrict__ y, float scale, float* __restrict__ M,
                                                    float* __restrict__ lse, float* __restrict__ z, float* __restrict__ p,
                                                    float* __restrict__ loss_sum, float* __restrict__ dz,
                                                    float* __restrict__ dM, float* __restrict__ cdot,
                                                    const int32_t* __restrict__ tile_map, const float* __restrict__ scores,
                                                    const float* __restrict__ hrow, float* __restrict__ ds,
                                                    const uint32_t* __restrict__ mbits, float mscale,
                                                    float* __restrict__ Mdrop, int loss_kind, int S,
                                                    const float* __restrict__ ws) {
    constexpr int DSP = 4;
    __shared__ __attribute__((aligned(16))) float part_lds[16 * 64];
    const int b = blockIdx.x, yb = blockIdx.y, tid = threadIdx.x;
    const int t0 = bag_tile_off[b], t1 = bag_tile_off[b + 1], nt = t1 - t0;
    int row[DSP];
    float sc[DSP], hh[DSP][4];
    if (yb < S) tail_rows_load<DSP>(tile_map, scores, hrow, C, t0, t1, yb, S, tid, row, sc, hh);
    const float* wb = ws + (size_t)b * TAIL_S_MAX * 8;
    float m = -INFINITY;
    for (int i = 0; i < S; ++i) m = fmaxf(m, wb[8 * i]);
    float sums[5] = {0.f, 0.f, 0.f, 0.f, 0.f};
    for (int i = 0; i < S; ++i) {
        const float mw = wb[8 * i];
        const float f = mw > -INFINITY ? expf(mw - m) : 0.f;
#pragma unroll
        for (int q = 0; q < 5; ++q) sums[q] += f * wb[8 * i + 1 + q];
    }
    const float l = sums[0];
    const float inv = nt > 0 && l > 0.f ? 1.0f / l : 0.f;
    const float lse_b = nt > 0 ? m + logf(l) : -INFINITY;
    float bfr[4], yr[4], zz[4], pp[4], dzr[4];
    float lossacc = 0.f, dot = 0.f;
#pragma unroll
    for (int c = 0; c < 4; ++c) {
        bfr[c] = c < C ? bf[c] : 0.f;
        yr[c] = c < C ? y[b * C + c] : 0.f;
        zz[c] = sums[1 + c] * inv + bfr[c];
        pp[c] = 1.0f / (1.0f + expf(-zz[c]));
        dzr[c] = 0.f;
    }
    if (loss_kind == 0) {
#pragma unroll
        for (int c = 0; c < 4; ++c)
            if (c < C) {
                lossacc += -(yr[c] * fmaxf(logf(pp[c]), -100.0f) + (1.0f - yr[c]) * fmaxf(logf(1.0f - pp[c]), -100.0f));
                dzr[c] = (pp[c] - yr[c]) * scale;
            }
    } else {
        float mx = -INFINITY, se = 0.f, sy = 0.f;
#pragma unroll
        for (int c = 0; c < 4; ++c) if (c < C) mx = fmaxf(mx, pp[c]);
#pragma unroll
        for (int c = 0; c < 4; ++c) if (c < C) se += expf(pp[c] - mx);
        const float lse_p = mx + logf(se);
#pragma unroll
        for (int c = 0; c < 4; ++c)
            if (c < C) {
                sy += yr[c];
                lossacc += -yr[c] * (pp[c] - lse_p);
            }
#pragma unroll
        for (int c = 0; c < 4; ++c)
            if (c < C) dzr[c] = (expf(pp[c] - lse_p) * sy - yr[c]) * scale * pp[c] * (1.0f - pp[c]);
    }
#pragma unroll
    for (int c = 0; c < 4; ++c) dot += dzr[c] * (zz[c] - bfr[c]);
    if (yb < S) {
#pragma unroll
        for (int k = 0; k < DSP; ++k)
            if (row[k] >= 0) {
                float gd = 0.f;
#pragma unroll
                for (int c = 0; c < 4; ++c) gd += dzr[c] * hh[k][c];
                ds[row[k]] = expf(sc[k] - m) * inv * (gd - dot);
            }
        for (int g8 = t0 + (DSP * S + yb) * 8 + (tid >> 5); g8 < t1; g8 += 8 * S) {
            const int row0 = tile_map[4 * g8 + 1], nrows = tile_map[4 * g8 + 2], lr = tid & 31;
            if (lr < nrows) {
                const size_t r_ = (size_t)(row0 + lr);
                float gd = 0.f;
                for (int c = 0; c < C; ++c) gd += dzr[c] * hrow[r_ * C + c];
                ds[r_] = expf(scores[r_] - m) * inv * (gd - dot);
            }
        }
        if (yb == 0) {
            if (tid == 0) {
                lse[b] = lse_b;
                cdot[b] = dot;
                loss_sum[b] = lossacc * scale;
            }
#pragma unroll
            for (int c = 0; c < 4; ++c)
                if (tid == c && c < C) {
                    z[b * C + c] = zz[c];
                    p[b * C + c] = pp[c];
                    dz[b * C + c] = dzr[c];
                }
            for (int j = tid; j < L; j += 256) {
                float keep = 1.0f;
                if (mbits != nullptr) keep = ((mbits[(size_t)b * (L >> 5) + (j >> 5)] >> (j & 31)) & 1u) ? mscale : 0.f;
                float d = 0.f;
                for (int c = 0; c < C; ++c) d += dzr[c] * Wf[(size_t)c * L + j];
                dM[(size_t)b * L + j] = d * keep;
            }
        }
        return;
    }
    const int j0 = 64 * (yb - S), c4 = tid & 15, tg = tid >> 4;
    const float* ml = partials + (size_t)T * L;
    f32x4 acc = {0, 0, 0, 0};
    int k = tg;
    for (; k + 48 < nt; k += 64) {
        f32x4 v[4];
        float w[4];
#pragma unroll
        for (int e = 0; e < 4; ++e) {
            v[e] = *reinterpret_cast<const f32x4*>(partials + (size_t)(t0 + k + 16 * e) * L + j0 + 4 * c4);
            w[e] = ml[2 * (t0 + k + 16 * e)];
        }
#pragma unroll
        for (int e = 0; e < 4; ++e) acc += expf(w[e] - lse_b) * v[e];
    }
    for (; k < nt; k += 16)
        acc += expf(ml[2 * (t0 + k)] - lse_b) * *reinterpret_cast<const f32x4*>(partials + (size_t)(t0 + k) * L + j0 + 4 * c4);
    *reinterpret_cast<f32x4*>(part_lds + tg * 64 + 4 * c4) = acc;
    __syncthreads();
    if (tid < 64) {
        float v = 0.f;
#pragma unroll
        for (int q = 0; q < 16; ++q) v += part_lds[q * 64 + tid];
        const int j = j0 + tid;
        M[(size_t)b * L + j] = v;
        if (Mdrop != nullptr) {
            float keep = 1.0f;
            if (mbits != nullptr) keep = ((mbits[(size_t)b * (L >> 5) + (j >> 5)] >> (j & 31)) & 1u) ? mscale : 0.f;
            Mdrop[(size_t)b * L + j] = v * keep;
        }
    }
}

extern "C" size_t mil_pool_tail_workspace_floats(int B) { return (size_t)(B > 0 ? B : 0) * TAIL_S_MAX * 8; }

extern "C" int mil_pool_merge_head_ws(const float* partials, const int32_t* bag_tile_off, int T, int B, int L,
                                      const float* Wf, const float* bf, int C, const float* y, float scale, float* M,
                                      float* lse, float* z, float* p, float* loss_sum, float* dz, float* dM, float* cdot,
                                      const int32_t* tile_map, const float* scores, const float* hrow, float* ds,
                                      const uint32_t* mbits, float mscale, float* Mdrop, int loss_kind, float* tail_ws,
                                      void* stream) {
    if (!partials || !bag_tile_off || !Wf || !bf || !M || !lse || !z || !p) return MIL_EINVAL;
    if (loss_kind != MIL_LOSS_BCE && loss_kind != MIL_LOSS_CE_ON_SIGMOID) return MIL_EINVAL;
    if (y && (!loss_sum || !dz || !dM || !cdot)) return MIL_EINVAL;
    if (ds && (!y || !tile_map || !scores || !hrow)) return MIL_EINVAL;
    if (!(L == 256 || L == 512 || L == 768 || L == 1024) || C <= 0 || C > 32 || B < 0) return MIL_EINVAL;
    if (B == 0) return MIL_OK;
    const char* tail_env = getenv("MIL_TAIL_H");
    const bool short_chain = C <= 4 && y && ds && hrow && !(tail_env != nullptr && tail_env[0] == '0');
    if (short_chain && tail_ws != nullptr && T >= 64 * B && B <= 8 && (tail_env == nullptr || tail_env[0] != '1')) {
        int S = (T / B + 31) / 32;
        if (S > TAIL_S_MAX) S = TAIL_S_MAX;
        hipLaunchKernelGGL(k_tail_stats, dim3(B, S), dim3(256), 0, (hipStream_t)stream, bag_tile_off, tile_map, scores, hrow, C, S,
                           tail_ws);
        MIL_CHECK_LAUNCH();
        hipLaunchKernelGGL(k_tail_apply, dim3(B, S + L / 64), dim3(256), 0, (hipStream_t)stream, partials, bag_tile_off, T, L, Wf, bf,
                           C, y, scale, M, lse, z, p, loss_sum, dz, dM, cdot, tile_map, scores, hrow, ds, mbits, mscale, Mdrop,
                           loss_kind, S, (const float*)tail_ws);
        MIL_CHECK_LAUNCH();
        return MIL_OK;
    }
    if (short_chain) {
        if (T >= 48 * B)
            hipLaunchKernelGGL(k_pool_tail_h<1024>, dim3(B, 2), dim3(1024), 0, (hipStream_t)stream, partials, bag_tile_off, T, L, Wf, bf,
                               C, y, scale, M, lse, z, p, loss_sum, dz, dM, cdot, tile_map, scores, hrow, ds, mbits, mscale, Mdrop,
                               loss_kind);
        else
            hipLaunchKernelGGL(k_pool_tail_h<256>, dim3(B, 2), dim3(256), 0, (hipStream_t)stream, partials, bag_tile_off, T, L, Wf, bf,
                               C, y, scale, M, lse, z, p, loss_sum, dz, dM, cdot, tile_map, scores, hrow, ds, mbits, mscale, Mdrop,
                               loss_kind);
        MIL_CHECK_LAUNCH();
        return MIL_OK;
    }
    if (T >= 48 * B)
        hipLaunchKernelGGL(k_pool_merge_head<1024>, dim3(B), dim3(1024), 0, (hipStream_t)stream, partials, bag_tile_off, T, L, Wf,
                           bf, C, y, scale, M, lse, z, p, loss_sum, dz, dM, cdot, tile_map, scores, hrow, ds, mbits, mscale,
                           Mdrop, loss_kind);
    else
        hipLaunchKernelGGL(k_pool_merge_head<256>, dim3(B), dim3(256), 0, (hipStream_t)stream, partials, bag_tile_off, T, L, Wf,
                           bf, C, y, scale, M, lse, z, p, loss_sum, dz, dM, cdot, tile_map, scores, hrow, ds, mbits, mscale,
                           Mdrop, loss_kind);
    MIL_CHECK_LAUNCH();
    return MIL_OK;
}

extern "C" int mil_pool_merge_head(const float* partials, const int32_t* bag_tile_off, int T, int B, int L,
                                   const float* Wf, const float* bf, int C, const float* y, float scale, float* M,
                                   float* lse, float* z, float* p, float* loss_sum, float* dz, float* dM, float* cdot,
                                   const int32_t* tile_map, const float* scores, const float* hrow, float* ds,
                                   const uint32_t* mbits, float mscale, float* Mdrop, int loss_kind, void* stream) {
    return mil_pool_merge_head_ws(partials, bag_tile_off, T, B, L, Wf, bf, C, y, scale, M, lse, z, p, loss_sum, dz, dM, cdot, tile_map,
                                  scores, hrow, ds, mbits, mscale, Mdrop, loss_kind, nullptr, stream);
}

extern "C" int mil_head_fwd(const float* M, const float* Wf, const float* bf, float* z, float* p, int B, int L, int C,
                            void* stream) {
    if (!M || !Wf || !bf || !z || !p) return MIL_EINVAL;
    if (B < 0 || L <= 0 || C <= 0 || C > 32) return MIL_EINVAL;
    if (B == 0) return MIL_OK;
    hipLaunchKernelGGL(k_head_fwd, dim3(B), dim3(256), 0, (hipStream_t)stream, M, Wf, bf, z, p, L, C);
    MIL_CHECK_LAUNCH();
    return MIL_OK;
}

extern "C" int mil_bce_fwd_bwd(const float* p, const float* y, float* loss_sum, float* dz, int B, int C, float scale,
                               void* stream) {
    if (!p || !y || !loss_sum || !dz) return MIL_EINVAL;
    if (B <= 0 || C <= 0) return MIL_EINVAL;
    hipLaunchKernelGGL(k_bce_fwd_bwd, dim3(1), dim3(256), 0, (hipStream_t)stream, p, y, loss_sum, dz, B * C, scale);
    MIL_CHECK_LAUNCH();
    return MIL_OK;
}

extern "C" int mil_head_bwd(const float* dz_or_dp, const float* p, const float* M, const float* Wf, float* dM,
                            float* dWf, float* dbf, float* cdot, int B, int L, int C, void* stream) {
    if (!dz_or_dp || !M || !Wf || !dM || !dWf || !dbf || !cdot) return MIL_EINVAL;
    if (B <= 0 || L <= 0 || C <= 0 || C > 32) return MIL_EINVAL;
    hipStream_t st = (hipStream_t)stream;
    hipLaunchKernelGGL(k_head_bwd_dm, dim3(B), dim3(256), 0, st, dz_or_dp, p, M, Wf, dM, cdot, L, C);
    MIL_CHECK_LAUNCH();
    hipLaunchKernelGGL(k_head_bwd_params, dim3(C * ((L + 63) / 64) + 1), dim3(256), 0, st, dz_or_dp, p, M, dWf, dbf, B, L,
                       C, (const float*)nullptr, (float*)nullptr, 0);
    MIL_CHECK_LAUNCH();
    return MIL_OK;
}

extern "C" int mil_head_bwd_params_acc(const float* dz, const float* M, float* dWf, float* dbf, int B, int L, int C,
                                       const float* loss_bag, float* loss_out, int accumulate, void* stream) {
    if (!dz || !M || !dWf || !dbf) return MIL_EINVAL;
    if (B <= 0 || L <= 0 || C <= 0 || C > 32 || (loss_bag && !loss_out)) return MIL_EINVAL;
    hipLaunchKernelGGL(k_head_bwd_params, dim3(C * ((L + 63) / 64) + 1), dim3(256), 0, (hipStream_t)stream, dz,
                       (const float*)nullptr, M, dWf, dbf, B, L, C, loss_bag, loss_out, accumulate);
    MIL_CHECK_LAUNCH();
    return MIL_OK;
}
extern "C" int mil_head_bwd_params(const float* dz, const float* M, float* dWf, float* dbf, int B, int L, int C,
                                   const float* loss_bag, float* loss_out, void* stream) {
    return mil_head_bwd_params_acc(dz, M, dWf, dbf, B, L, C, loss_bag, loss_out, 0, stream);
}

static void launch_adam(float* param, const float* grad, float* m, float* v, size_t n, float lr, float b1, float b2,
                        float eps, float wd, float gscale, float bc1, float bc2_sqrt, const int* step_dev, hipStream_t st,
                        const float* lr_dev = nullptr) {
    if (n >= ((size_t)1 << 21))
        hipLaunchKernelGGL(k_adam<4>, dim3((unsigned)((n + 4095) / 4096)), dim3(256), 0, st, param, grad, m, v, n, lr, b1, b2, eps,
                           wd, gscale, bc1, bc2_sqrt, step_dev, lr_dev);
    else
        hipLaunchKernelGGL(k_adam<1>, dim3((unsigned)((n + 1023) / 1024)), dim3(256), 0, st, param, grad, m, v, n, lr, b1, b2, eps,
                           wd, gscale, bc1, bc2_sqrt, step_dev, lr_dev);
}

extern "C" int mil_adam_step(float* param, const float* grad, float* exp_avg, float* exp_avg_sq, size_t n, int step,
                             float lr, float beta1, float beta2, float eps, float weight_decay, float grad_scale,
                             void* stream) {
    if (!param || !grad || !exp_avg || !exp_avg_sq || step < 1) return MIL_EINVAL;
    if (n == 0) return MIL_OK;
    if ((reinterpret_cast<uintptr_t>(param) | reinterpret_cast<uintptr_t>(grad) | reinterpret_cast<uintptr_t>(exp_avg) |
         reinterpret_cast<uintptr_t>(exp_avg_sq)) & 15)
        return MIL_EINVAL;
    const double bc1 = 1.0 - pow((double)beta1, (double)step);
    const double bc2 = 1.0 - pow((double)beta2, (double)step);
    launch_adam(param, grad, exp_avg, exp_avg_sq, n, lr, beta1, beta2, eps, weight_decay, grad_scale, (float)bc1,
                (float)sqrt(bc2), (const int*)nullptr, (hipStream_t)stream);
    MIL_CHECK_LAUNCH();
    return MIL_OK;
}

extern "C" int mil_adam_step_counted_noinc(float* param, const float* grad, float* exp_avg, float* exp_avg_sq, size_t n,
                                           const int32_t* step_counter, float lr, float beta1, float beta2, float eps,
                                           float weight_decay, float grad_scale, void* stream) {
    if (!param || !grad || !exp_avg || !exp_avg_sq || !step_counter) return MIL_EINVAL;
    if ((reinterpret_cast<uintptr_t>(param) | reinterpret_cast<uintptr_t>(grad) | reinterpret_cast<uintptr_t>(exp_avg) |
         reinterpret_cast<uintptr_t>(exp_avg_sq)) & 15)
        return MIL_EINVAL;
    if (n == 0) return MIL_OK;
    launch_adam(param, grad, exp_avg, exp_avg_sq, n, lr, beta1, beta2, eps, weight_decay, grad_scale, 1.f, 1.f,
                (const int*)step_counter, (hipStream_t)stream);
    MIL_CHECK_LAUNCH();
    return MIL_OK;
}
extern "C" int mil_adam_step_counted(float* param, const float* grad, float* exp_avg, float* exp_avg_sq, size_t n,
                                     int32_t* step_counter, float lr, float beta1, float beta2, float eps,
                                     float weight_decay, float grad_scale, void* stream) {
    if (!param || !grad || !exp_avg || !exp_avg_sq || !step_counter) return MIL_EINVAL;
    if ((reinterpret_cast<uintptr_t>(param) | reinterpret_cast<uintptr_t>(grad) | reinterpret_cast<uintptr_t>(exp_avg) |
         reinterpret_cast<uintptr_t>(exp_avg_sq)) & 15)
        return MIL_EINVAL;
    hipStream_t st = (hipStream_t)stream;
    if (n > 0) {
        launch_adam(param, grad, exp_avg, exp_avg_sq, n, lr, beta1, beta2, eps, weight_decay, grad_scale, 1.f, 1.f,
                    (const int*)step_counter, st);
        MIL_CHECK_LAUNCH();
    }
    hipLaunchKernelGGL(k_step_inc, dim3(1), dim3(1), 0, st, step_counter);
    MIL_CHECK_LAUNCH();
    return MIL_OK;
}

extern "C" int mil_adam_step_dev(float* param, const float* grad, float* exp_avg, float* exp_avg_sq, size_t n,
                                 int32_t* step_counter, const float* lr_dev, float beta1, float beta2, float eps,
                                 float weight_decay, float grad_scale, int inc, void* stream) {
    if (!param || !grad || !exp_avg || !exp_avg_sq || !step_counter || !lr_dev) return MIL_EINVAL;
    if ((reinterpret_cast<uintptr_t>(param) | reinterpret_cast<uintptr_t>(grad) | reinterpret_cast<uintptr_t>(exp_avg) |
// ... 185 lines not shown
```

### llm-guided-multimodal-mil_amd/csrc/mil_internal.h

```cpp
#pragma once
#include "mil_common.h"

#define MIL_HIDDEN __attribute__((visibility("hidden")))

MIL_HIDDEN int gate_tail_rows(int R, int tiles_per_round);
int gate_fwd_with_pool(const float* x, const float* Wv, const float* bv, const float* Wu, const float* bu, const float* w,
                       const float* b, float* scores, float* gates, int R, int L, int draw, uint32_t* xbits, float xscale,
                       uint32_t* mbits, float mscale, int B, uint64_t seed, uint64_t mseed, uint64_t offset,
                       const int32_t* offset_dev, const int32_t* tile_map, int T, float* partials, const float* Wf, float* hrow,
                       int* fused, void* stream, const uint16_t* Wp);
int gate_fwd_rows_dev(const float* x, const float* Wv, const float* bv, const float* Wu, const float* bu, const float* w,
                      const float* b, float* scores, float* gates, int R, int L, int draw, uint32_t* xbits, float xscale,
                      uint32_t* mbits, int B, uint64_t seed, uint64_t mseed, uint64_t offset, const int32_t* offset_dev,
                      const int32_t* rows_dev, void* stream, const TileMapJob* tmap, const uint16_t* Wp);

struct GateDwPlan {
    int dw, S, kc;
};
MIL_HIDDEN GateDwPlan gate_dw_plan(int R, int L, int ncu);
int gate_bwd_reduce_head_adam_impl(const float* workspace, int R, int L, float* dWv, float* dbv, float* dWu, float* dbu,
                                   float* dw, float* db, int accumulate, float xscale, const float* dz, const float* M,
                                   float* dWf, float* dbf, int B, int C, const float* loss_bag, float* loss_out,
                                   float* param_flat, const float* grad_flat, size_t n_param, float* exp_avg,
                                   float* exp_avg_sq, int step, const int* step_dev, float lr, const float* lr_dev, float beta1,
                                   float beta2, float eps, float weight_decay, float grad_scale, void* stream,
                                   int* done = nullptr, uint16_t* Wp = nullptr);

int gate_bwd_params_bf16_tail(const uint16_t* x, const uint16_t* gates, const float* ds, const float* w, int R, int L,
                              float* workspace, size_t workspace_floats, float* dWv, float* dbv, float* dWu, float* dbu,
                              float* dw, float* db, int accumulate, const uint32_t* xbits, float xscale, const float* dz,
                              const float* M, float* dWf, float* dbf, int B, int C, const float* loss_bag, float* loss_out,
                              float* param_flat, const float* grad_flat, size_t n_param, float* exp_avg, float* exp_avg_sq,
                              int step, const int* step_dev, float lr, const float* lr_dev, float beta1, float beta2, float eps,
                              float weight_decay, float grad_scale, uint16_t* Wv16, uint16_t* Wu16, void* stream, int* done);
int gate_fwd_bf16_with_pool(const uint16_t* x, const uint16_t* Wv, const float* bv, const uint16_t* Wu, const float* bu,
                            const float* w, const float* b, float* scores, uint16_t* gates16, int R, int L, const uint32_t* xbits,
                            float xscale, const int32_t* tile_map, int T, float* partials, const float* Wf, float* hrow,
                            const uint32_t* mbits, float mscale, int* fused, void* stream);

int dropout_keep_bits_pair(uint32_t* xbits, int R, uint32_t* mbits, int B, int L, uint64_t seed, uint64_t mseed, uint64_t offset,
                           const int32_t* offset_dev, void* stream);
int dropout_keep_bits_pair_tilemap(uint32_t* xbits, int R, uint32_t* mbits, int B, int L, uint64_t seed, uint64_t mseed,
                                   uint64_t offset, const int32_t* offset_dev, const TileMapJob& tm, void* stream);

MIL_HIDDEN int gemm_tn2_plan(int rows, int N, int K, int ncu, int* KC_out);
MIL_HIDDEN int gemm_tn2_ok(int lddy, int ldy, int ldx, int rows, int N, int K, int ncu);
int mil_gemm_tn2_rows(const float* dY, int lddy, const float* Y, int ldy, int act, const float* X, int ldx, int rows, int N, int K,
                      float* partial, float* cs_partial, const int32_t* rows_dev, void* stream);
```

### llm-guided-multimodal-mil_amd/csrc/step.hip

```cpp
#include <stdlib.h>

#include "mil_internal.h"

static int step_check(const mil_image_only_step* a) {
    if (!a || a->struct_bytes != sizeof(mil_image_only_step)) return MIL_EINVAL;
    if (!a->x || !a->tile_map || !a->bag_tile_off) return MIL_EINVAL;
    if (a->R < 0 || a->B < 0 || a->T < 0 || a->L <= 0 || a->C <= 0 || a->C > 32) return MIL_EINVAL;
    if (!a->Wv || !a->bv || !a->Wu || !a->bu || !a->w || !a->b || !a->Wf || !a->bf) return MIL_EINVAL;
    if (!a->scores || !a->partials || !a->M || !a->lse || !a->logits || !a->prob) return MIL_EINVAL;
    if (a->x_bf16 && (!a->Wv16 || !a->Wu16)) return MIL_EINVAL;
    if (a->bag_len_dev && (a->x_bf16 || !a->rows_dev || a->B > 1024)) return MIL_EINVAL;
    if (a->train && (!a->xbits || !a->mbits || !a->Mdrop)) return MIL_EINVAL;
    if (a->lr_dev && !a->adam_step_dev) return MIL_EINVAL;
    if (a->y) {
        if ((!a->gates && !a->gates16) || !a->ds || !a->loss_bag || !a->dz || !a->dM || !a->cdot) return MIL_EINVAL;
    }
    return MIL_OK;
}

static bool fuse_pool_enabled() {
    const char* e = getenv("MIL_FUSE_POOL");
    return e == nullptr || e[0] != '0';
}

static bool fuse_pool16_enabled(bool train) {
    const char* e = getenv("MIL_FUSE_POOL16");
    (void)train;
    return e != nullptr && e[0] != '0';
}

extern "C" int mil_abi_version(void) { return 12; }

extern "C" int mil_image_only_step_run(const mil_image_only_step* a, void* stream) {
    int rc = step_check(a);
    if (rc != MIL_OK) return rc;
    const uint32_t st = a->stages;
    const bool train = a->train != 0;
    const bool grads = a->y != nullptr;
    const float xscale = train ? 2.0f : 1.0f;
    const float mscale = train ? 1.0f / 0.75f : 1.0f;
    const uint32_t* xbits = train ? a->xbits : nullptr;
    const uint32_t* mbits = train ? a->mbits : nullptr;
    const bool use_h = a->hrow != nullptr && grads && a->C <= 4;
    const uint16_t* Wp = (!a->x_bf16 && a->Wp) ? a->Wp : nullptr;
    bool adam_in_reduce = false;
    int pool_fused = 0;

    const bool draw_in_fwd = (st & MIL_STAGE_DROPBITS) && (st & MIL_STAGE_GATE_FWD) && train && !a->x_bf16;
    const bool gen_launch = (st & MIL_STAGE_DROPBITS) && train && !draw_in_fwd;
    const bool want_tmap = (st & MIL_STAGE_TILEMAP) && a->bag_len_dev;
    const TileMapJob tmj{a->bag_len_dev, a->B, const_cast<int32_t*>(a->tile_map), const_cast<int32_t*>(a->bag_tile_off), a->rows_dev,
                         a->T};
    const bool tmap_with_fwd = want_tmap && (st & MIL_STAGE_GATE_FWD) && !a->x_bf16 && a->rows_dev != nullptr && !gen_launch;
    if (want_tmap && gen_launch) {
        rc = dropout_keep_bits_pair_tilemap(a->xbits, a->R, a->mbits, a->B, a->L, a->seed, a->seed ^ 0x9E3779B97F4A7C15ull,
                                            a->offset, a->offset_dev, tmj, stream);
        if (rc != MIL_OK) return rc;
    } else if (want_tmap && !tmap_with_fwd) {
        rc = mil_build_tile_map(a->bag_len_dev, a->B, const_cast<int32_t*>(a->tile_map), const_cast<int32_t*>(a->bag_tile_off),
                                a->rows_dev, a->T, stream);
        if (rc != MIL_OK) return rc;
    }
    if (gen_launch && !((st & MIL_STAGE_TILEMAP) && a->bag_len_dev)) {
        rc = dropout_keep_bits_pair(a->xbits, a->R, a->mbits, a->B, a->L, a->seed, a->seed ^ 0x9E3779B97F4A7C15ull, a->offset,
                                    a->offset_dev, stream);
        if (rc != MIL_OK) return rc;
    }
    if (st & MIL_STAGE_GATE_FWD) {
        float* gates = grads ? a->gates : nullptr;
        const bool g16 = a->x_bf16 && a->bf16_grad_mfma && (a->L % 256) == 0 && a->gates16 != nullptr;
        if (a->x_bf16 && g16 && grads && (st & MIL_STAGE_POOL) && (st & MIL_STAGE_POOL_FUSED) && use_h && a->C == 2 &&
            fuse_pool_enabled() && fuse_pool16_enabled(train))
            rc = gate_fwd_bf16_with_pool((const uint16_t*)a->x, a->Wv16, a->bv, a->Wu16, a->bu, a->w, a->b, a->scores, a->gates16,
                                         a->R, a->L, xbits, xscale, a->tile_map, a->T, a->partials, a->Wf, a->hrow, mbits, mscale,
                                         &pool_fused, stream);
        else if (a->x_bf16)
            rc = mil_gate_scores_fwd_bf16((const uint16_t*)a->x, a->Wv16, a->bv, a->Wu16, a->bu, a->w, a->b, a->scores,
                                          g16 ? nullptr : gates, a->R, a->L, MIL_GATE_D, (grads && g16) ? a->gates16 : nullptr,
                                          xbits, xscale, stream);
        else if ((st & MIL_STAGE_POOL) && (st & MIL_STAGE_POOL_FUSED) && use_h && a->C == 2 && !a->bag_len_dev &&
                 (!train || draw_in_fwd) && fuse_pool_enabled())
            rc = gate_fwd_with_pool((const float*)a->x, a->Wv, a->bv, a->Wu, a->bu, a->w, a->b, a->scores, gates, a->R, a->L,
                                    draw_in_fwd ? 1 : 0, a->xbits, xscale, a->mbits, mscale, a->B, a->seed,
                                    a->seed ^ 0x9E3779B97F4A7C15ull, a->offset, a->offset_dev, a->tile_map, a->T, a->partials,
                                    a->Wf, a->hrow, &pool_fused, stream, Wp);
        else if (a->bag_len_dev && a->rows_dev)
            rc = gate_fwd_rows_dev((const float*)a->x, a->Wv, a->bv, a->Wu, a->bu, a->w, a->b, a->scores, gates, a->R, a->L,
                                   draw_in_fwd ? 1 : 0, a->xbits, xscale, a->mbits, a->B, a->seed, a->seed ^ 0x9E3779B97F4A7C15ull,
                                   a->offset, a->offset_dev, a->rows_dev, stream, tmap_with_fwd ? &tmj : nullptr, Wp);
        else if (Wp != nullptr)
            rc = gate_fwd_rows_dev((const float*)a->x, a->Wv, a->bv, a->Wu, a->bu, a->w, a->b, a->scores, gates, a->R, a->L,
                                   draw_in_fwd ? 1 : 0, draw_in_fwd ? a->xbits : const_cast<uint32_t*>(xbits), xscale, a->mbits,
                                   a->B, a->seed, a->seed ^ 0x9E3779B97F4A7C15ull, a->offset, a->offset_dev, nullptr, stream,
                                   nullptr, Wp);
        else if (draw_in_fwd)
            rc = mil_gate_scores_fwd_draw((const float*)a->x, a->Wv, a->bv, a->Wu, a->bu, a->w, a->b, a->scores, gates, a->R,
                                          a->L, MIL_GATE_D, a->xbits, xscale, a->mbits, a->B, a->seed,
                                          a->seed ^ 0x9E3779B97F4A7C15ull, a->offset, a->offset_dev, stream);
        else
            rc = mil_gate_scores_fwd((const float*)a->x, a->Wv, a->bv, a->Wu, a->bu, a->w, a->b, a->scores, gates, a->R, a->L,
                                     MIL_GATE_D, xbits, xscale, stream);
        if (rc != MIL_OK) return rc;
    }
    if ((st & MIL_STAGE_POOL) && !pool_fused) {
        if (a->x_bf16) {
            rc = use_h ? mil_attn_pool_partial_h_bf16((const uint16_t*)a->x, a->scores, a->tile_map, a->T, a->L, a->partials,
                                                      a->Wf, a->C, a->hrow, xbits, xscale, mbits, mscale, stream)
                       : mil_attn_pool_partial_bf16((const uint16_t*)a->x, a->scores, a->tile_map, a->T, a->L, a->partials,
                                                    xbits, xscale, stream);
        } else {
            rc = use_h ? mil_attn_pool_partial_h((const float*)a->x, a->scores, a->tile_map, a->T, a->L, a->partials, a->Wf,
                                                 a->C, a->hrow, xbits, xscale, mbits, mscale, stream)
                       : mil_attn_pool_partial((const float*)a->x, a->scores, a->tile_map, a->T, a->L, a->partials, xbits,
                                               xscale, stream);
        }
        if (rc != MIL_OK) return rc;
    }
    if (st & MIL_STAGE_TAIL) {
        rc = mil_pool_merge_head_ws(a->partials, a->bag_tile_off, a->T, a->B, a->L, a->Wf, a->bf, a->C, a->y, a->loss_scale, a->M,
                                    a->lse, a->logits, a->prob, grads ? a->loss_bag : nullptr, grads ? a->dz : nullptr,
                                    grads ? a->dM : nullptr, grads ? a->cdot : nullptr, use_h ? a->tile_map : nullptr,
                                    use_h ? a->scores : nullptr, use_h ? a->hrow : nullptr, use_h ? a->ds : nullptr, mbits, mscale,
                                    train ? a->Mdrop : nullptr, a->loss_kind, a->tail_ws, stream);
        if (rc != MIL_OK) return rc;
        if (grads && !use_h) {
            rc = a->x_bf16 ? mil_attn_pool_bwd_bf16((const uint16_t*)a->x, a->scores, a->lse, a->dM, a->cdot, a->tile_map, a->T,
                                                    a->L, a->ds, xbits, xscale, stream)
                           : mil_attn_pool_bwd((const float*)a->x, a->scores, a->lse, a->dM, a->cdot, a->tile_map, a->T, a->L,
                                               a->ds, nullptr, xbits, xscale, stream);
            if (rc != MIL_OK) return rc;
        }
    }
    if (!grads) return MIL_OK;
    if (!a->dWv || !a->dbv || !a->dWu || !a->dbu || !a->dw || !a->db || !a->dWf || !a->dbf || !a->loss_out || !a->dw_ws)
        return (st & (MIL_STAGE_GATE_BWD | MIL_STAGE_REDUCE)) ? MIL_EINVAL : MIL_OK;
    const float* Mhead = train ? a->Mdrop : a->M;
    if (a->x_bf16) {
        const bool tail16 = a->bf16_grad_mfma && (a->L % 256) == 0 && a->gates16 && (st & MIL_STAGE_GATE_BWD) &&
                            (st & MIL_STAGE_REDUCE);
        if (tail16) {
            adam_in_reduce = (st & MIL_STAGE_ADAM) && a->param_flat && a->grad_flat && a->exp_avg && a->exp_avg_sq &&
                             (a->adam_step_dev || a->adam_step >= 1);
            rc = gate_bwd_params_bf16_tail((const uint16_t*)a->x, a->gates16, a->ds, a->w, a->R, a->L, a->dw_ws,
                                           (size_t)a->dw_ws_floats, a->dWv, a->dbv, a->dWu, a->dbu, a->dw, a->db, a->accumulate,
                                           xbits, xscale, a->dz, Mhead, a->dWf, a->dbf, a->B, a->C, a->loss_bag, a->loss_out,
                                           adam_in_reduce ? a->param_flat : nullptr, a->grad_flat, (size_t)a->n_param, a->exp_avg,
                                           a->exp_avg_sq, a->adam_step, a->adam_step_dev, a->lr, a->lr_dev, a->beta1, a->beta2,
                                           a->eps, a->weight_decay, a->grad_scale, const_cast<uint16_t*>(a->Wv16),
                                           const_cast<uint16_t*>(a->Wu16), stream, a->done_dev);
            if (rc == MIL_OK && adam_in_reduce && a->adam_step_dev && !a->done_dev) rc = mil_counter_add(a->adam_step_dev, 1, stream);
            if (rc != MIL_OK) return rc;
        } else if (st & (MIL_STAGE_GATE_BWD | MIL_STAGE_REDUCE)) {
            if (a->bf16_grad_mfma && (a->L % 256) == 0 && a->gates16)
                rc = mil_gate_bwd_params_bf16((const uint16_t*)a->x, a->gates16, a->ds, a->w, a->R, a->L, MIL_GATE_D, a->dw_ws,
                                              (size_t)a->dw_ws_floats, a->dWv, a->dbv, a->dWu, a->dbu, a->dw, a->db,
                                              a->accumulate, xbits, xscale, stream);
            else
                rc = mil_gate_bwd_params_x16((const uint16_t*)a->x, a->gates, a->ds, a->w, a->R, a->L, MIL_GATE_D, a->dw_ws,
                                             (size_t)a->dw_ws_floats, a->dWv, a->dbv, a->dWu, a->dbu, a->dw, a->db,
                                             a->accumulate, xbits, xscale, stream);
            if (rc != MIL_OK) return rc;
        }
        if ((st & MIL_STAGE_REDUCE) && !tail16) {
            rc = mil_head_bwd_params_acc(a->dz, Mhead, a->dWf, a->dbf, a->B, a->L, a->C, a->loss_bag, a->loss_out, a->accumulate,
                                         stream);
            if (rc != MIL_OK) return rc;
        }
    } else {
        if (st & MIL_STAGE_GATE_BWD) {
            rc = mil_gate_bwd_partials_rows((const float*)a->x, a->gates, a->ds, a->w, a->R, a->L, MIL_GATE_D, a->dw_ws,
                                            (size_t)a->dw_ws_floats, xbits, a->bag_len_dev ? a->rows_dev : nullptr, stream);
            if (rc != MIL_OK) return rc;
        }
        if (st & MIL_STAGE_REDUCE) {
            adam_in_reduce = (st & MIL_STAGE_ADAM) && a->param_flat && a->grad_flat && a->exp_avg && a->exp_avg_sq &&
                             (a->adam_step_dev || a->adam_step >= 1);
            if (adam_in_reduce) {
                rc = gate_bwd_reduce_head_adam_impl(a->dw_ws, a->R, a->L, a->dWv, a->dbv, a->dWu, a->dbu, a->dw, a->db,
                                                    a->accumulate, xscale, a->dz, Mhead, a->dWf, a->dbf, a->B, a->C, a->loss_bag,
                                                    a->loss_out, a->param_flat, a->grad_flat, (size_t)a->n_param, a->exp_avg,
                                                    a->exp_avg_sq, a->adam_step, a->adam_step_dev, a->lr, a->lr_dev, a->beta1,
                                                    a->beta2, a->eps, a->weight_decay, a->grad_scale, stream, a->done_dev,
                                                    const_cast<uint16_t*>(a->Wp));
                if (rc == MIL_OK && a->adam_step_dev && !a->done_dev) rc = mil_counter_add(a->adam_step_dev, 1, stream);
            }
            else
                rc = mil_gate_bwd_reduce_head(a->dw_ws, a->R, a->L, a->dWv, a->dbv, a->dWu, a->dbu, a->dw, a->db, a->accumulate,
                                              xscale, a->dz, Mhead, a->dWf, a->dbf, a->B, a->C, a->loss_bag, a->loss_out, stream);
            if (rc != MIL_OK) return rc;
        }
    }
    if ((st & MIL_STAGE_ADAM) && !adam_in_reduce) {
        if (!a->param_flat || !a->grad_flat || !a->exp_avg || !a->exp_avg_sq) return MIL_EINVAL;
        if (a->adam_step_dev && a->lr_dev)
            rc = mil_adam_step_dev(a->param_flat, a->grad_flat, a->exp_avg, a->exp_avg_sq, (size_t)a->n_param,
                                   a->adam_step_dev, a->lr_dev, a->beta1, a->beta2, a->eps, a->weight_decay, a->grad_scale, 1,
                                   stream);
        else if (a->adam_step_dev)
            rc = mil_adam_step_counted(a->param_flat, a->grad_flat, a->exp_avg, a->exp_avg_sq, (size_t)a->n_param,
                                       a->adam_step_dev, a->lr, a->beta1, a->beta2, a->eps, a->weight_decay, a->grad_scale,
                                       stream);
        else
            rc = mil_adam_step(a->param_flat, a->grad_flat, a->exp_avg, a->exp_avg_sq, (size_t)a->n_param, a->adam_step, a->lr,
                               a->beta1, a->beta2, a->eps, a->weight_decay, a->grad_scale, stream);
        if (rc != MIL_OK) return rc;
        if (!a->x_bf16 && a->Wp) {
            rc = mil_gate_pieces(a->Wv, a->Wu, const_cast<uint16_t*>(a->Wp), a->L, stream);
            if (rc != MIL_OK) return rc;
        }
        if (a->x_bf16) {
            rc = mil_cast_bf16(a->Wv, const_cast<uint16_t*>(a->Wv16), (size_t)MIL_GATE_D * a->L, stream);
            if (rc != MIL_OK) return rc;
            rc = mil_cast_bf16(a->Wu, const_cast<uint16_t*>(a->Wu16), (size_t)MIL_GATE_D * a->L, stream);
            if (rc != MIL_OK) return rc;
        }
    }
    return MIL_OK;
}

extern "C" int mil_image_only_step_time(const mil_image_only_step* a, uint32_t stages, int warm, int iters, float* ms_out,
                                        void* stream) {
    if (!a || !ms_out || iters <= 0 || warm < 0) return MIL_EINVAL;
    mil_image_only_step s = *a;
    s.stages = stages;
    hipStream_t st = (hipStream_t)stream;
    hipEvent_t e0, e1;
    if (hipEventCreate(&e0) != hipSuccess) return MIL_EINVAL;
    if (hipEventCreate(&e1) != hipSuccess) { (void)hipEventDestroy(e0); return MIL_EINVAL; }
    int rc = MIL_OK;
    for (int i = 0; i < warm && rc == MIL_OK; ++i) rc = mil_image_only_step_run(&s, stream);
    if (rc == MIL_OK) {
        (void)hipEventRecord(e0, st);
        for (int i = 0; i < iters && rc == MIL_OK; ++i) rc = mil_image_only_step_run(&s, stream);
        (void)hipEventRecord(e1, st);
        const hipError_t e = hipEventSynchronize(e1);
        if (rc == MIL_OK && e != hipSuccess) rc = (int)e;
        float ms = 0.f;
        if (rc == MIL_OK && hipEventElapsedTime(&ms, e0, e1) == hipSuccess) *ms_out = ms / (float)iters;
    }
    (void)hipEventDestroy(e0);
    (void)hipEventDestroy(e1);
    return rc;
}

extern "C" int mil_image_only_step_profile_rot(const mil_image_only_step* a, const void* const* xs, const float* const* ys,
                                               int nrot, const uint32_t* groups, int ngroups, int warm, int iters,
                                               float* ms_out, void* stream) {
    if (!a || !groups || !ms_out || ngroups <= 0 || ngroups > 16 || iters <= 0 || iters > 256 || warm < 0) return MIL_EINVAL;
    if (nrot < 0 || nrot > 64 || (nrot > 0 && (!xs || !ys))) return MIL_EINVAL;
    for (int i = 0; i < nrot; ++i)
        if (!xs[i] || !ys[i]) return MIL_EINVAL;
    mil_image_only_step s = *a;
    hipStream_t st = (hipStream_t)stream;
    const int per = ngroups + 1, nev = per * iters;
    hipEvent_t* ev = (hipEvent_t*)malloc(sizeof(hipEvent_t) * (size_t)nev);
    if (!ev) return MIL_EINVAL;
    int made = 0, rc = MIL_OK, turn = 0;
    for (; made < nev; ++made)
        if (hipEventCreate(&ev[made]) != hipSuccess) { rc = MIL_EINVAL; break; }
    for (int i = 0; i < warm && rc == MIL_OK; ++i, ++turn) {
        if (nrot > 0) { s.x = xs[turn % nrot]; s.y = ys[turn % nrot]; }
        for (int g = 0; g < ngroups && rc == MIL_OK; ++g) { s.stages = groups[g]; rc = mil_image_only_step_run(&s, stream); }
    }
    for (int i = 0; i < iters && rc == MIL_OK; ++i, ++turn) {
        if (nrot > 0) { s.x = xs[turn % nrot]; s.y = ys[turn % nrot]; }
        (void)hipEventRecord(ev[i * per], st);
        for (int g = 0; g < ngroups && rc == MIL_OK; ++g) {
            s.stages = groups[g];
            rc = mil_image_only_step_run(&s, stream);
            (void)hipEventRecord(ev[i * per + g + 1], st);
        }
    }
    if (rc == MIL_OK && hipStreamSynchronize(st) != hipSuccess) rc = MIL_EINVAL;
    if (rc == MIL_OK) {
        for (int g = 0; g <= ngroups; ++g) ms_out[g] = 0.f;
        for (int i = 0; i < iters; ++i) {
            float ms = 0.f;
            for (int g = 0; g < ngroups; ++g)
                if (hipEventElapsedTime(&ms, ev[i * per + g], ev[i * per + g + 1]) == hipSuccess) ms_out[g] += ms;
            if (hipEventElapsedTime(&ms, ev[i * per], ev[i * per + ngroups]) == hipSuccess) ms_out[ngroups] += ms;
        }
        for (int g = 0; g <= ngroups; ++g) ms_out[g] /= (float)iters;
    }
    for (int i = 0; i < made; ++i) (void)hipEventDestroy(ev[i]);
    free(ev);
    return rc;
}

extern "C" int mil_image_only_step_profile(const mil_image_only_step* a, const uint32_t* groups, int ngroups, int warm,
                                           int iters, float* ms_out, void* stream) {
    return mil_image_only_step_profile_rot(a, nullptr, nullptr, 0, groups, ngroups, warm, iters, ms_out, stream);
}
```

### llm-guided-multimodal-mil_amd/trainer.py

```python
from __future__ import annotations

from typing import Dict, Optional

import os

import torch
import torch.distributed as dist

import ctypes

from . import _lib, ops
from .bags import BagLayout, DeviceBagLayout, bucket_rows
from .dist_utils import allreduce_flat, broadcast_flat

PARAM_ORDER = [
    "aggregator.attention_V.0.weight", "aggregator.attention_V.0.bias",
    "aggregator.attention_U.0.weight", "aggregator.attention_U.0.bias",
    "aggregator.attention_weights.weight", "aggregator.attention_weights.bias",
    "fc.1.weight", "fc.1.bias",
]


class FlatParams:

    def __init__(self, params: Dict[str, torch.Tensor], device, order=None):
        self.order = list(order or params.keys())
        self.shapes = {k: tuple(params[k].shape) for k in self.order}
        sizes = [int(params[k].numel()) for k in self.order]
        self.offsets = {}
        off = 0
        for k, n in zip(self.order, sizes):
            self.offsets[k] = off
            off += (n + 3) // 4 * 4
        self.numel = off
        self.flat = torch.zeros(off, device=device, dtype=torch.float32)
        self.grad_ext = torch.zeros(off + 4, device=device, dtype=torch.float32)
        self.grad = self.grad_ext[:off]
        self.loss_slot = self.grad_ext[off:off + 1]
        self.exp_avg = torch.zeros_like(self.flat)
        self.exp_avg_sq = torch.zeros_like(self.flat)
        for k in self.order:
            self.view(self.flat, k).copy_(params[k])

    def view(self, buf: torch.Tensor, k: str) -> torch.Tensor:
        o = self.offsets[k]
        n = 1
        for s in self.shapes[k]:
            n *= s
        return buf[o:o + n].view(self.shapes[k])

    def p(self, k):
        return self.view(self.flat, k)

    def g(self, k):
        return self.view(self.grad, k)

    def state_dict(self):
        return {k: self.p(k).clone() for k in self.order}


class ImageOnlyTrainer:

    def __init__(self, params: Dict[str, torch.Tensor], device, lr: float = 1e-5, betas=(0.9, 0.999),
                 weight_decay: float = 1e-7, eps: float = 1e-8, world_size: int = 1, bf16_grad_mfma: bool = True,
                 train_mode: bool = False, accum: int = 1, seed: int = 1234, counted: bool = False,
                 loss: Optional[str] = None):
        self.device = device
        self.fp = FlatParams(params, device, PARAM_ORDER)
        self.lr, self.betas, self.wd, self.eps = lr, betas, weight_decay, eps
        self.world = world_size
        self.force_collectives = os.environ.get("MIL_FORCE_COLLECTIVES") == "1"
        self.bf16_grad_mfma = bf16_grad_mfma
        self.step_count = 0
        C = int(params["fc.1.weight"].shape[0])
        self.loss = loss if loss is not None else ("ce" if C > 2 else "bce")
        if self.loss not in ("bce", "ce"):
            raise ValueError("loss must be 'bce' or 'ce'")
        self.loss_sum = self.fp.loss_slot
        self.train_mode = bool(train_mode)
        self.seed, self.drop_pass = int(seed), 0
        self.accum = max(1, int(accum))
        self._micro = 0
        self.step_counter = torch.zeros(1, device=device, dtype=torch.int32) if counted else None
        self.lr_dev = torch.full((1,), float(lr), device=device, dtype=torch.float32) if counted else None
        self.done_dev = torch.zeros(1, device=device, dtype=torch.int32) if counted else None
        self._lr_on_dev = float(lr)
        self._ws: Dict[str, torch.Tensor] = {}
        self._args: Optional[_lib.ImageOnlyStep] = None
        self._args_key = None
        self._keep = None
        self._w16: Optional[Dict[str, torch.Tensor]] = None
        self._w16_version, self._param_version = -1, 0
        self._wp: Optional[torch.Tensor] = None
        self._wp_version = -1
        self.gate_pieces = os.environ.get("MIL_GATE_PIECES", "1") != "0"
        self._graph = None
        self.last = {}
        if self.world > 1:
            broadcast_flat(self.fp.flat, src=0)

    def _buf(self, name: str, numel: int, dtype=torch.float32) -> torch.Tensor:
        t = self._ws.get(name)
        if t is None or t.numel() < numel or t.dtype != dtype:
            t = self._ws[name] = torch.empty(max(1, numel), device=self.device, dtype=dtype)
        return t

    def _shadows(self):
        fp = self.fp
        if self._w16 is None:
            self._w16 = {k: torch.empty(fp.p(k).shape, device=self.device, dtype=torch.bfloat16)
                         for k in ("aggregator.attention_V.0.weight", "aggregator.attention_U.0.weight")}
        if self._w16_version != self._param_version:
            for k, t in self._w16.items():
                ops.cast_bf16(fp.p(k), out=t)
            self._w16_version = self._param_version
        return self._w16

    def _pieces(self):
        fp = self.fp
        Wv, Wu = fp.p("aggregator.attention_V.0.weight"), fp.p("aggregator.attention_U.0.weight")
        if self._wp is None:
            self._wp = torch.empty(3 * 2 * Wv.numel(), device=self.device, dtype=torch.int16)
        if self._wp_version != self._param_version and not torch.cuda.is_current_stream_capturing():
            _lib.checked().mil_gate_pieces(Wv.data_ptr(), Wu.data_ptr(), self._wp.data_ptr(), Wv.shape[1], ops._stream())
            self._wp_version = self._param_version
        return self._wp

    def _fill(self, x: torch.Tensor, layout: BagLayout, y: Optional[torch.Tensor], global_bags: Optional[int]):
        b16 = x.dtype == torch.bfloat16
        if not x.is_cuda or x.dtype not in (torch.float32, torch.bfloat16):
            raise _lib.MilHipError("ImageOnlyTrainer: x must be a float32 / bfloat16 tensor on the MI355X (no CPU path)")
        if not x.is_contiguous():
            x = x.contiguous()
        R, L = x.shape
        if R != layout.R:
            raise _lib.MilHipError(f"ImageOnlyTrainer: x has {R} rows but the bag layout covers {layout.R}")
        fp = self.fp
        C = fp.p("fc.1.weight").shape[0]
        if fp.p("fc.1.weight").shape[1] != L:
            raise _lib.MilHipError("ImageOnlyTrainer: the head's input width must equal the patch width L")
        train = self.train_mode and y is not None
        key = (x.data_ptr(), R, L, b16, id(layout), None if y is None else y.data_ptr(), global_bags, train)
        if self._args is not None and key == self._args_key:
            return self._args
        B, T = layout.B, layout.T
        a = _lib.ImageOnlyStep()
        a.struct_bytes = ctypes.sizeof(_lib.ImageOnlyStep)
        pv = lambda t: None if t is None else t.data_ptr()
        a.x, a.y, a.tile_map, a.bag_tile_off = pv(x), pv(y), pv(layout.tile_map), pv(layout.bag_tile_off)
        a.R, a.L, a.B, a.C, a.T, a.x_bf16 = R, L, B, C, T, int(b16)
        if isinstance(layout, DeviceBagLayout):
            if b16:
                raise _lib.MilHipError("device-side bag lengths are supported on the fp32 path only")
            a.bag_len_dev, a.rows_dev = pv(layout.bag_len_dev), pv(layout.rows_dev)
        nb = global_bags if global_bags is not None else B * self.world
        a.loss_kind = 1 if self.loss == "ce" else 0
        a.loss_scale = 1.0 / (max(1, nb) * (C if self.loss == "bce" else 1) * self.accum)
        names = {"Wv": "aggregator.attention_V.0.weight", "bv": "aggregator.attention_V.0.bias",
                 "Wu": "aggregator.attention_U.0.weight", "bu": "aggregator.attention_U.0.bias",
                 "w": "aggregator.attention_weights.weight", "b": "aggregator.attention_weights.bias",
                 "Wf": "fc.1.weight", "bf": "fc.1.bias"}
        for f, k in names.items():
            setattr(a, f, fp.p(k).data_ptr())
            setattr(a, "d" + f, fp.g(k).data_ptr())
        if b16:
            w16 = self._shadows()
            a.Wv16, a.Wu16 = w16[names["Wv"]].data_ptr(), w16[names["Wu"]].data_ptr()
        elif self.gate_pieces and L % 32 == 0:
            a.Wp = self._pieces().data_ptr()
        a.loss_out = self.loss_sum.data_ptr()
        grads = y is not None
        st = dict(scores=self._buf("scores", R), partials=self._buf("partials", T * (L + 2)),
                  M=self._buf("M", B * L), lse=self._buf("lse", B), logits=self._buf("logits", B * C),
                  prob=self._buf("prob", B * C), tail_ws=self._buf("tail_ws", _lib.lib().mil_pool_tail_workspace_floats(B)))
        if grads:
            if b16:
                need = _lib.lib().mil_gate_bwd_workspace_floats_bf16(R, L) if (self.bf16_grad_mfma and L % 256 == 0) else \
                    _lib.lib().mil_gate_bwd_workspace_floats(R, L)
            else:
                need = _lib.lib().mil_gate_bwd_workspace_floats(R, L)
            if b16 and os.environ.get("MIL_BF16_GATES") == "0":
                self.bf16_grad_mfma = False
            g16 = b16 and self.bf16_grad_mfma and L % 256 == 0
            st.update(gates=None if g16 else self._buf("gates", R * 2 * ops.GATE_D),
                      gates16=self._buf("gates16", R * 2 * ops.GATE_D, torch.bfloat16) if g16 else None, ds=self._buf("ds", R),
                      hrow=self._buf("hrow", R * C) if C <= 4 else None, dw_ws=self._buf("dw_ws", need),
                      Mdrop=self._buf("Mdrop", B * L), loss_bag=self._buf("loss_bag", B), dz=self._buf("dz", B * C),
                      dM=self._buf("dM", B * L), cdot=self._buf("cdot", B))
            a.dw_ws_floats = st["dw_ws"].numel()
        if train:
            st.update(xbits=self._buf("xbits", R * (L // 32), torch.int32), mbits=self._buf("mbits", B * (L // 32), torch.int32))
        for k, t in st.items():
            setattr(a, k, pv(t))
        a.train, a.bf16_grad_mfma, a.seed = int(train), int(self.bf16_grad_mfma), self.seed
        a.offset_dev = pv(self.step_counter)
        a.param_flat, a.grad_flat = fp.flat.data_ptr(), fp.grad.data_ptr()
        a.exp_avg, a.exp_avg_sq, a.n_param = fp.exp_avg.data_ptr(), fp.exp_avg_sq.data_ptr(), fp.flat.numel()
        a.adam_step_dev = pv(self.step_counter)
        a.lr_dev = pv(self.lr_dev)
        a.done_dev = pv(self.done_dev)
        a.tail_ws = st["tail_ws"].data_ptr()
        a.beta1, a.beta2, a.eps, a.weight_decay, a.grad_scale = self.betas[0], self.betas[1], self.eps, self.wd, 1.0
        self._args, self._args_key = a, key
        self._keep = (x, y, layout, dict(st), self._w16)
        self.last = dict(x=x, layout=layout, scores=st["scores"][:R], M=st["M"][:B * L].view(B, L), lse=st["lse"][:B],
                         logits=st["logits"][:B * C].view(B, C), prob=st["prob"][:B * C].view(B, C))
        if grads:
            gsaved = st["gates"] if st["gates"] is not None else st["gates16"]
            self.last.update(gates=gsaved[:R * 2 * ops.GATE_D].view(R, 2 * ops.GATE_D), ds=st["ds"][:R],
                             hrow=None if st["hrow"] is None else st["hrow"][:R * C].view(R, C),
                             dz=st["dz"][:B * C].view(B, C), dM=st["dM"][:B * L].view(B, L), cdot=st["cdot"][:B],
                             loss_bag=st["loss_bag"][:B], Mdrop=st["Mdrop"][:B * L].view(B, L))
        if train:
            self.last.update(xbits=st["xbits"][:R * (L // 32)].view(R, L // 32), mbits=st["mbits"][:B * (L // 32)].view(B, L // 32))
        return a

    def _sync_lr(self):
        if self.lr_dev is not None and self._lr_on_dev != float(self.lr) and not torch.cuda.is_current_stream_capturing():
            self.lr_dev.fill_(float(self.lr))
            self._lr_on_dev = float(self.lr)

    def _run(self, a, stages: int, keep=None):
        self._sync_lr()
        if a.Wp and self._wp_version != self._param_version:
            self._pieces()
        keep = self._keep if keep is None else keep
        if getattr(keep[2], "aligned32", False) and (stages & _lib.STAGE_GATE_FWD) and (stages & _lib.STAGE_POOL):
            stages |= _lib.STAGE_POOL_FUSED
        a.stages = stages
        a.accumulate = int(self._micro > 0)
        a.lr = self.lr
        a.adam_step = self.step_count + 1
        a.offset = (self._micro << 32) | (0 if self.step_counter is not None else (self.drop_pass & 0xFFFFFFFF))
        _lib.checked().mil_image_only_step_run(ctypes.byref(a), ops._stream())

    def forward(self, x: torch.Tensor, layout: BagLayout, y: Optional[torch.Tensor] = None,
                global_bags: Optional[int] = None):
        a = self._fill(x, layout, y, global_bags)
        if a.train:
            self.drop_pass += 1
        self._run(a, _lib.STAGE_TILEMAP | _lib.STAGE_DROPBITS | _lib.STAGE_GATE_FWD | _lib.STAGE_POOL | _lib.STAGE_TAIL)
        return self.last["prob"], self.last["logits"]

    def backward(self):
        if self._args is None or not self._args.y:
            raise _lib.MilHipError("ImageOnlyTrainer.backward: call forward(x, layout, y) with labels first")
        self._run(self._args, _lib.STAGE_GATE_BWD | _lib.STAGE_REDUCE)
        return self.loss_sum

    def reduce_only(self):
        if self.world > 1 or self.force_collectives:
            allreduce_flat(self.fp.grad_ext)

    def _adam(self, a=None, keep=None):
        a = self._args if a is None else a
        self._run(a, _lib.STAGE_ADAM, keep)
        self.step_count += 1
        self._param_version += 1
        if a.x_bf16:
            self._w16_version = self._param_version
        if a.Wp:
            self._wp_version = self._param_version

    def reduce_and_step(self, a=None, keep=None):
        self.reduce_only()
        self._adam(a, keep)

    def train_step(self, x: torch.Tensor, layout: BagLayout, y: torch.Tensor):
        a = self._fill(x, layout, y, None)
        if a.train:
            self.drop_pass += 1
        last = self._micro == self.accum - 1
        fused_adam = last and not (self.world > 1 or self.force_collectives)
        self._run(a, _lib.STAGE_ALL if fused_adam else _lib.STAGE_ALL & ~_lib.STAGE_ADAM)
        if fused_adam:
            self.step_count += 1
            self._param_version += 1
            if a.x_bf16:
                self._w16_version = self._param_version
            if a.Wp:
                self._wp_version = self._param_version
        elif last:
            self.reduce_and_step()
        self._micro = 0 if last else self._micro + 1
        return self.loss_sum, self.last["prob"]

    def reset_dropout_stream(self):
        self.drop_pass = 0

    def model_state_dict(self, prefix_map=(("aggregator.", "extractor_pathology."),)):
        out = {}
        for k, v in self.fp.state_dict().items():
            for a, b in prefix_map:
                if k.startswith(a):
                    k = b + k[len(a):]
                    break
            out[k] = v
        return out

    def load_model_state_dict(self, sd, prefix_map=(("extractor_pathology.", "aggregator."),)):
        for k, v in sd.items():
            for a, b in prefix_map:
                if k.startswith(a):
                    k = b + k[len(a):]
                    break
            if k in self.fp.offsets:
                self.fp.p(k).copy_(v)
        self._param_version += 1

    def optimizer_state_dict(self):
        step = int(self.step_counter.item()) if self.step_counter is not None else self.step_count
        return {"step": step, "exp_avg": self.fp.exp_avg.clone(), "exp_avg_sq": self.fp.exp_avg_sq.clone(),
                "order": list(self.fp.order), "drop_pass": self.drop_pass,
                "param_groups": [{"lr": self.lr, "betas": tuple(self.betas), "eps": self.eps, "weight_decay": self.wd}]}

    def load_optimizer_state_dict(self, sd):
        if list(sd.get("order", self.fp.order)) != list(self.fp.order):
            raise ValueError("optimizer state was saved for another parameter order")
        self.fp.exp_avg.copy_(sd["exp_avg"])
        self.fp.exp_avg_sq.copy_(sd["exp_avg_sq"])
        self.step_count = int(sd["step"])
        self.drop_pass = int(sd.get("drop_pass", 0))
        if self.step_counter is not None:
            self.step_counter.fill_(self.step_count)

    def time_pieces(self, x: torch.Tensor, layout: BagLayout, y: torch.Tensor, iters: int = 20, warm: int = 3):
        a = self._fill(x, layout, y, None)
        self._run(a, _lib.STAGE_ALL & ~_lib.STAGE_ADAM)
        fwd = _lib.STAGE_GATE_FWD | (_lib.STAGE_DROPBITS if a.train else 0)
        groups = [("gate_fwd", fwd), ("pool_partial", _lib.STAGE_POOL),
                  ("merge_head_loss_ds", _lib.STAGE_TAIL), ("gate_bwd_dw", _lib.STAGE_GATE_BWD),
                  ("gate_bwd_reduce_and_head_params", _lib.STAGE_REDUCE)]
        if a.x_bf16:
            groups = [g for g in groups if g[0] not in ("gate_bwd_dw", "gate_bwd_reduce_and_head_params")]
            groups.append(("gate_bwd_dw", _lib.STAGE_GATE_BWD | _lib.STAGE_REDUCE))
        if not a.x_bf16 and getattr(layout, "aligned32", False):
            groups.append(("gate_fwd_with_pool_fused", fwd | _lib.STAGE_POOL | _lib.STAGE_POOL_FUSED))
        out = {}
        ms = ctypes.c_float(0.0)
        for name, stg in groups:
            a.accumulate = 0
            _lib.checked().mil_image_only_step_time(ctypes.byref(a), stg, warm, iters, ctypes.byref(ms), ops._stream())
            out[name] = float(ms.value)
        fp = self.fp
        a2 = _lib.ImageOnlyStep.from_buffer_copy(a)
        scratch = [fp.flat.clone(), fp.exp_avg.clone(), fp.exp_avg_sq.clone()]
        a2.param_flat, a2.exp_avg, a2.exp_avg_sq = (t.data_ptr() for t in scratch)
        if a2.Wp:
            scratch.append(self._wp.clone())
            a2.Wp = scratch[-1].data_ptr()
        a2.adam_step_dev, a2.adam_step, a2.lr, a2.x_bf16 = None, 1, self.lr, 0
        _lib.checked().mil_image_only_step_time(ctypes.byref(a2), _lib.STAGE_ADAM, warm, iters, ctypes.byref(ms), ops._stream())
        out["adam"] = float(ms.value)
        return out

    def time_step_groups(self, x: torch.Tensor, layout: BagLayout, y: torch.Tensor, iters: int = 50, warm: int = 5, rot=None):
        a = self._fill(x, layout, y, None)
        self._run(a, _lib.STAGE_ALL & ~_lib.STAGE_ADAM)
        fp = self.fp
        a2 = _lib.ImageOnlyStep.from_buffer_copy(a)
        scratch = [fp.flat.clone(), fp.exp_avg.clone(), fp.exp_avg_sq.clone()]
        a2.param_flat, a2.exp_avg, a2.exp_avg_sq = (t.data_ptr() for t in scratch)
        if a2.Wp:
            scratch.append(self._wp.clone())
            a2.Wp = scratch[-1].data_ptr()
        a2.adam_step_dev, a2.lr_dev, a2.adam_step, a2.lr, a2.accumulate = None, None, 1, self.lr, 0
        S = _lib
        fwd = S.STAGE_TILEMAP | S.STAGE_DROPBITS | S.STAGE_GATE_FWD
        fused_pool = getattr(layout, "aligned32", False) and (not a.x_bf16 or (a.L in (512, 1024) and a.R >= 256 * 256
                                                                               and bool(a.gates16) and a.C == 2
                                                                               and os.environ.get("MIL_FUSE_POOL", "1") != "0"
                                                                               and os.environ.get("MIL_FUSE_POOL16", "0") != "0"))
        groups = []
        if fused_pool:
            groups.append(("gate_fwd_with_pool_fused", fwd | S.STAGE_POOL | S.STAGE_POOL_FUSED))
        else:
            groups += [("gate_fwd", fwd), ("pool_partial", S.STAGE_POOL)]
        groups.append(("merge_head_loss_ds", S.STAGE_TAIL))
        collective = self.world > 1 or self.force_collectives
        if a.x_bf16 and collective:
            groups += [("gate_bwd_dw_reduce_head", S.STAGE_GATE_BWD | S.STAGE_REDUCE), ("adam", S.STAGE_ADAM)]
        elif a.x_bf16:
            groups += [("gate_bwd_dw_reduce_head_adam", S.STAGE_GATE_BWD | S.STAGE_REDUCE | S.STAGE_ADAM)]
        elif collective:
            groups += [("gate_bwd_dw", S.STAGE_GATE_BWD), ("gate_bwd_reduce_head", S.STAGE_REDUCE), ("adam", S.STAGE_ADAM)]
        else:
            groups += [("gate_bwd_dw", S.STAGE_GATE_BWD), ("gate_bwd_reduce_head_adam", S.STAGE_REDUCE | S.STAGE_ADAM)]
        masks = (ctypes.c_uint32 * len(groups))(*[m for _, m in groups])
        nb = 5 if iters >= 20 else 1
        per = max(1, iters // nb)
        runs = []
        nrot = len(rot) if rot else 0
        for xr, yr in (rot or []):
            if xr.shape != x.shape or xr.dtype != x.dtype or yr.shape != y.shape or not xr.is_contiguous():
                raise _lib.MilHipError("time_step_groups: every rotated batch must have the shape of the first")
        xs_arr = (ctypes.c_void_p * max(1, nrot))(*[t[0].data_ptr() for t in (rot or [])])
        ys_arr = (ctypes.c_void_p * max(1, nrot))(*[t[1].data_ptr() for t in (rot or [])])
        for b in range(nb):
            out = (ctypes.c_float * (len(groups) + 1))()
            _lib.checked().mil_image_only_step_profile_rot(ctypes.byref(a2), xs_arr if nrot else None, ys_arr if nrot else None,
                                                           nrot, masks, len(groups), warm if b == 0 else 1, per, out,
                                                           ops._stream())
            runs.append([float(v) for v in out])
        med = [sorted(r[i] for r in runs)[nb // 2] for i in range(len(groups) + 1)]
        return {n: med[i] for i, (n, _) in enumerate(groups)}, med[len(groups)]

    def capture(self, x: torch.Tensor, layout: BagLayout, y: torch.Tensor, collective_in_graph: Optional[bool] = None):
        if self.accum != 1:
            raise _lib.MilHipError("ImageOnlyTrainer.capture: gradient accumulation (accum > 1) cannot be replayed from one graph")
        a = self._fill(x, layout, y, None)
        if a.train and self.step_counter is None:
            raise _lib.MilHipError("ImageOnlyTrainer.capture in train mode needs counted=True: the dropout stream position "
                                   "must live on the device, or every replay would draw the same mask")
        collective = self.world > 1 or self.force_collectives
        if collective_in_graph is None:
            collective_in_graph = os.environ.get("MIL_GRAPH_COLLECTIVE") == "1"
        collective_in_graph = bool(collective_in_graph) and collective and self.step_counter is not None and self.accum == 1
        in_graph_adam = self.step_counter is not None and self.accum == 1 and (not collective or collective_in_graph)
        stages = _lib.STAGE_ALL if in_graph_adam else _lib.STAGE_ALL & ~_lib.STAGE_ADAM
        side = torch.cuda.Stream()
        side.wait_stream(torch.cuda.current_stream())
        with torch.cuda.stream(side):
            self._run(a, _lib.STAGE_ALL & ~_lib.STAGE_ADAM)
            if collective_in_graph:
                self.reduce_only()
        torch.cuda.current_stream().wait_stream(side)
        graph = torch.cuda.CUDAGraph()
        with torch.cuda.graph(graph):
            if collective_in_graph:
                self._run(a, _lib.STAGE_ALL & ~_lib.STAGE_ADAM)
                self.reduce_only()
                self._run(a, _lib.STAGE_ADAM)
            else:
                self._run(a, stages)
        self._graph = dict(graph=graph, keep=(self._keep, dict(self._ws)), args=a, adam=in_graph_adam, last=dict(self.last),
                           collective=collective_in_graph)
        return self

    def replay_step(self):
        g = self._graph
        self._sync_lr()
        g["graph"].replay()
        self.last = g["last"]
        if g["adam"]:
            self.step_count += 1
            self._param_version += 1
            if g["args"].Wp:
                self._wp_version = self._param_version
        else:
            self.reduce_and_step(g["args"], g["keep"][0])
        return self.loss_sum, self.last["prob"]


class RaggedImageOnlyStepper:

    class Slot:
        def __init__(self, cap, B, L, C, device):
            self.cap, self.visits, self.graph = cap, 0, None
            self.x = torch.zeros((cap, L), device=device, dtype=torch.float32)
            self.y = torch.zeros((B, C), device=device, dtype=torch.float32)
            self.layout = DeviceBagLayout(cap, B, device)

    def __init__(self, trainer: ImageOnlyTrainer, B: int = 1, use_graph: bool = True):
        self.tr, self.B, self.use_graph = trainer, int(B), bool(use_graph)
        if self.use_graph and trainer.step_counter is None:
            raise ValueError("graph replay needs ImageOnlyTrainer(counted=True): step number and dropout stream on the device")
        self.slots = {}
        self.replays = self.eager_steps = 0

    def slot(self, n_rows: int) -> "RaggedImageOnlyStepper.Slot":
        cap = bucket_rows(n_rows)
        s = self.slots.get(cap)
        if s is None:
            L = self.tr.fp.p("fc.1.weight").shape[1]
            C = self.tr.fp.p("fc.1.weight").shape[0]
            s = self.slots[cap] = self.Slot(cap, self.B, L, C, self.tr.device)
        return s

    def step(self, slot: "RaggedImageOnlyStepper.Slot", lengths, on_device: bool = False):
        tr = self.tr
        if on_device:
            slot.layout.note_lengths(lengths)
        else:
            slot.layout.set_lengths(lengths)
        slot.visits += 1
        if slot.graph is None and self.use_graph and slot.visits >= 2:
            tr.capture(slot.x, slot.layout, slot.y)
            slot.graph = tr._graph
        if slot.graph is not None:
            tr._graph = slot.graph
            self.replays += 1
            return tr.replay_step()
        self.eager_steps += 1
        return tr.train_step(slot.x, slot.layout, slot.y)
```

Baseline: 187,900 bags/s.

## Fuse pool merge, head and loss tail into fused gate-forward kernel via last-block tickets

The gate-forward+pool kernel now publishes scores, h-rows, partials and max/sum values with agent-scope atomic stores. A per-bag ticket counter lets the last finishing workgroup for each bag run the merge, classifier head, BCE loss, dM and ds computation in-kernel. This removes the separate merge_head_loss launch and the round trip of reloading partials. The cost is atomic publish stores, extra LDS/register pressure from the tail path, and serialised per-bag tail work on the last block, which could delay the kernel's end.

```diff
diff --git a/include/mil_hip.h b/include/mil_hip.h
--- a/include/mil_hip.h
+++ b/include/mil_hip.h
@@ -440,9 +440,11 @@
     float* tail_ws;
     int32_t* done_dev;
     const uint16_t* Wp;
+    int32_t* tail_cnt;
 } mil_image_only_step;
 
 int mil_image_only_step_run(const mil_image_only_step* a, void* stream);
+int mil_image_only_step_tail_fused(const mil_image_only_step* a, int* tail_fused);
 int mil_image_only_step_time(const mil_image_only_step* a, uint32_t stages, int warm, int iters, float* ms_out,
                              void* stream);
 
@@ -468,6 +470,7 @@
     int32_t tail, tail_rows, tail_kernel, tail_rt;
     int32_t bits, pool_fused;
     int32_t dw, S, kc;
+    int32_t tail_fused;
 } mil_gate_route;
 int mil_gate_step_route(int R, int L, int C, int save_gates, int keep, int pieces, int fused_pool, int bucketed, int ncu,
                         mil_gate_route* out);
diff --git a/llm-guided-multimodal-mil_amd/_lib.py b/llm-guided-multimodal-mil_amd/_lib.py
--- a/llm-guided-multimodal-mil_amd/_lib.py
+++ b/llm-guided-multimodal-mil_amd/_lib.py
@@ -9,7 +9,7 @@
 _HERE = os.path.dirname(os.path.abspath(__file__))
 LIB_PATH = os.path.join(_HERE, "libmil_hip.so")
 HEADER_PATH = os.path.join(os.path.dirname(_HERE), "include", "mil_hip.h")
-ABI_VERSION = 12
+ABI_VERSION = 13
 
 _P = c_void_p
 SIGNATURES: Dict[str, Tuple[object, List[object]]] = {
@@ -54,6 +54,7 @@
     "mil_gate_bwd_input": (c_int, [_P] * 5 + [c_int, c_int, c_int, _P, _P, c_float, _P]),
     "mil_gate_bwd_input_pool": (c_int, [_P] * 5 + [c_int, c_int, c_int, _P, _P, c_float, _P, _P, _P, _P, _P]),
     "mil_image_only_step_run": (c_int, [_P, _P]),
+    "mil_image_only_step_tail_fused": (c_int, [_P, _P]),
     "mil_image_only_step_time": (c_int, [_P, c_uint32, c_int, c_int, _P, _P]),
     "mil_gate_step_route": (c_int, [c_int] * 9 + [_P]),
     "mil_gemm_route": (c_int, [c_int] * 16 + [_P]),
@@ -208,7 +209,7 @@
 
 class GateRoute(ctypes.Structure):
     _fields_ = [(n, c_int32) for n in ("main", "rt", "tail", "tail_rows", "tail_kernel", "tail_rt", "bits", "pool_fused",
-                                       "dw", "S", "kc")]
+                                       "dw", "S", "kc", "tail_fused")]
 
 
 class GemmPlan(ctypes.Structure):
@@ -247,7 +248,7 @@
         + [(n, _P) for n in ("param_flat", "grad_flat", "exp_avg", "exp_avg_sq")]
         + [("n_param", c_uint64), ("adam_step", c_int32), ("adam_step_dev", _P)]
         + [(n, c_float) for n in ("lr", "beta1", "beta2", "eps", "weight_decay", "grad_scale")]
-        + [("lr_dev", _P), ("tail_ws", _P), ("done_dev", _P), ("Wp", _P)])
+        + [("lr_dev", _P), ("tail_ws", _P), ("done_dev", _P), ("Wp", _P), ("tail_cnt", _P)])
 
 
 _lib = None
diff --git a/llm-guided-multimodal-mil_amd/csrc/gate_fwd.hip b/llm-guided-multimodal-mil_amd/csrc/gate_fwd.hip
--- a/llm-guided-multimodal-mil_amd/csrc/gate_fwd.hip
+++ b/llm-guided-multimodal-mil_amd/csrc/gate_fwd.hip
@@ -1,5 +1,6 @@
 #include "mil_internal.h"
 #include "philox.h"
+#include <stdlib.h>
 #include <type_traits>
 
 #define GF_TM 128
@@ -48,7 +49,15 @@
 #define GF_PRED_FLOATS(NQ) (4 * 2 * (NQ) * 256)
 static_assert(GF_SRED_OFF + 2 * GF_TM <= GF_SC_OFF && GF_SC_OFF + GF_TM <= GF_PRED_OFF, "epilogue LDS regions overlap");
 
-template <bool DROP>
+__device__ __forceinline__ void gate_publish_f32(float* p, float v) {
+    __hip_atomic_store(p, v, __ATOMIC_RELAXED, __HIP_MEMORY_SCOPE_AGENT);
+}
+typedef unsigned gf_u32x4 __attribute__((ext_vector_type(4)));
+__device__ __forceinline__ void gate_publish_f32x4(__amdgpu_buffer_rsrc_t srd, int byte_off, f32x4 v) {
+    __builtin_amdgcn_raw_buffer_store_b128(__builtin_bit_cast(gf_u32x4, v), srd, byte_off, 0, 16 );
+}
+
+template <bool DROP, bool PUBLISH = false>
 __device__ __forceinline__ void gate_fwd_scores_epilogue(const GateFwdCoord co, const f32x16 (&acc)[3][2], const float* bv,
                                                          const float* bu, const float* wvec, const float* battn,
                                                          float* scores, float* gates, int R, float xscale, lds_f32* smem,
@@ -84,7 +93,10 @@
     if (co.tid < GF_TM) {
         const int gr = co.row0 + co.tid;
         const float sc = sred[co.tid] + sred[GF_TM + co.tid] + battn[0];
-        if (gr < R) scores[gr] = sc;
+        if (gr < R) {
+            if constexpr (PUBLISH) gate_publish_f32(scores + gr, sc);
+            else scores[gr] = sc;
+        }
         if (copy_scores) smem[GF_SC_OFF + co.tid] = gr < R ? sc : -INFINITY;
     }
 }
@@ -457,7 +469,7 @@
             }
     }
 }
-template <bool DROP, bool GEN, int NQ>
+template <bool DROP, bool GEN, int NQ, bool PUBLISH = false>
 __device__ __forceinline__ void gate_fwd_pool_pass(const GateFwdCoord co, const GateKeepWords<DROP, GEN>& kw, GatePoolRows<NQ>& pv,
                                                    const uint32_t* xbits, int R, int L, float xscale, const GateFwdGen& gen,
                                                    const GateFwdPool& pool, lds_f32* smem) {
@@ -543,7 +555,11 @@
                 }
             const float tot = wave_reduce16(d16, lane);
             const int k = wave_reduce16_index(lane), rr = 2 * wc + j + 4 * (k >> 1);
-            if ((lane & 3) == 0) pool.hrow[(size_t)(trow0 + rr) * 2 + (k & 1)] = tot;
+            if ((lane & 3) == 0) {
+                float* hp = pool.hrow + (size_t)(trow0 + rr) * 2 + (k & 1);
+                if constexpr (PUBLISH) gate_publish_f32(hp, tot);
+                else *hp = tot;
+            }
         }
         if (wc == 1) {
 #pragma unroll
@@ -556,30 +572,333 @@
     __syncthreads();
     if (live && wc == 0) {
         float* out = pool.partials + (size_t)t * L;
+        __amdgpu_buffer_rsrc_t srd_o;
+        if constexpr (PUBLISH) srd_o = __builtin_amdgcn_make_buffer_rsrc((void*)out, 0, L * 4, MIL_SRD_FLAGS);
 #pragma unroll
         for (int q = 0; q < NQ; ++q) {
             f32x4 vv = pacc[0][q];
             vv += pacc[1][q];
             vv += *(lds_cf4*)(pred + ((wr * 2 + 0) * NQ + q) * 256 + 4 * lane);
             vv += *(lds_cf4*)(pred + ((wr * 2 + 1) * NQ + q) * 256 + 4 * lane);
-            *reinterpret_cast<f32x4*>(out + 256 * q + 4 * lane) = vv;
+            if constexpr (PUBLISH) gate_publish_f32x4(srd_o, (256 * q + 4 * lane) * 4, vv);
+            else *reinterpret_cast<f32x4*>(out + 256 * q + 4 * lane) = vv;
         }
         if (lane == 0) {
             float* ml = pool.partials + (size_t)pool.T * L + 2 * t;
-            ml[0] = m_;
-            ml[1] = l_;
-        }
-    }
-}
-
-template <bool DROP, bool GEN, int PQ, bool PW = false>
+            if constexpr (PUBLISH) {
+                gate_publish_f32(ml, m_);
+                gate_publish_f32(ml + 1, l_);
+            } else {
+                ml[0] = m_;
+                ml[1] = l_;
+            }
+        }
+    }
+}
+
+typedef __attribute__((address_space(3))) int lds_i32;
+#define GF_TL_RED_OFF 0
+#define GF_TL_CLOSE_OFF 64
+#define GF_TL_SCALE_OFF 128
+#define GF_TL_PART_OFF 1152
+static_assert(GF_TL_PART_OFF + 1024 <= gate_fwd2_smem_floats(false) && GF_TL_PART_OFF + 1024 <= gate_fwd2_smem_floats(true),
+              "the tail's regions must fit the LDS image of either K loop");
+
+__device__ __forceinline__ void tail_head_loss(const float (&sums)[5], float inv, const float (&bfr)[4], const float (&yr)[4], int C,
+                                               int loss_kind, float scale, float (&zz)[4], float (&pp)[4], float (&dzr)[4],
+                                               float& lossacc, float& dot) {
+    lossacc = 0.f;
+    dot = 0.f;
+#pragma unroll
+    for (int c = 0; c < 4; ++c) {
+        zz[c] = sums[1 + c] * inv + bfr[c];
+        pp[c] = 1.0f / (1.0f + expf(-zz[c]));
+        dzr[c] = 0.f;
+    }
+    if (loss_kind == 0) {
+#pragma unroll
+        for (int c = 0; c < 4; ++c)
+            if (c < C) {
+                lossacc += -(yr[c] * fmaxf(logf(pp[c]), -100.0f) + (1.0f - yr[c]) * fmaxf(logf(1.0f - pp[c]), -100.0f));
+                dzr[c] = (pp[c] - yr[c]) * scale;
+            }
+    } else {
+        float mx = -INFINITY, se = 0.f, sy = 0.f;
+#pragma unroll
+        for (int c = 0; c < 4; ++c) if (c < C) mx = fmaxf(mx, pp[c]);
+#pragma unroll
+        for (int c = 0; c < 4; ++c) if (c < C) se += expf(pp[c] - mx);
+        const float lse_p = mx + logf(se);
+#pragma unroll
+        for (int c = 0; c < 4; ++c)
+            if (c < C) {
+                sy += yr[c];
+                lossacc += -yr[c] * (pp[c] - lse_p);
+            }
+#pragma unroll
+        for (int c = 0; c < 4; ++c)
+            if (c < C) dzr[c] = (expf(pp[c] - lse_p) * sy - yr[c]) * scale * pp[c] * (1.0f - pp[c]);
+    }
+#pragma unroll
+    for (int c = 0; c < 4; ++c) dot += dzr[c] * (zz[c] - bfr[c]);
+}
+
+template <bool DROP, bool GEN, int NQ>
+__device__ __forceinline__ void gate_fwd_tail_bag(const GateFwdCoord co, const GateKeepWords<DROP, GEN>& kw, int b, const float* scores,
+                                                  const GateFwdGen& gen, const GateFwdPool& pool, const GateFwdTail& tl,
+                                                  lds_f32* smem) {
+    constexpr int NT = 256, NW = 4, L = 256 * NQ, JP = NQ, DSP = 4;
+    constexpr int L4 = L / 4, NG = NT / L4;
+    static_assert(NG * L == 1024 && NG >= 1, "part region");
+    const int half = co.wave >> 2, ht = co.tid & (NT - 1), hw = co.wave & 3, lane = co.lane;
+    const int t0 = tl.bag_tile_off[b], t1 = tl.bag_tile_off[b + 1], nt = t1 - t0;
+    lds_f32* red = smem + GF_TL_RED_OFF + half * 32;
+    lds_f32* scale_lds = smem + GF_TL_SCALE_OFF;
+    lds_f32* part_lds = smem + GF_TL_PART_OFF;
+    const float* ml = pool.partials + (size_t)pool.T * L;
+    float keepv[JP];
+#pragma unroll
+    for (int q = 0; q < JP; ++q) {
+        keepv[q] = 1.0f;
+        if (DROP) {
+            const int j = ht + q * NT, widx = b * (L >> 5) + (j >> 5);
+            unsigned wd;
+            if (GEN) {
+                const uint2 pr = philox_keep_words_quarter((uint64_t)(widx >> 1), kw.off, gen.mseed_lo, gen.mseed_hi);
+                wd = (widx & 1) ? pr.y : pr.x;
+            } else {
+                wd = pool.mbits[widx];
+            }
+            keepv[q] = ((wd >> (j & 31)) & 1u) ? pool.mscale : 0.f;
+        }
+    }
+    int ds_row[DSP];
+    float ds_sc[DSP], ds_h[DSP][4], wf[JP][4], bfr[4], yr[4];
+    float mt = -INFINITY, lt = 0.f, m;
+    f32x4 pre[8];
+    const int c4 = ht % L4, g = ht / L4;
+    if (half == 0) {
+#pragma unroll
+        for (int k = 0; k < DSP; ++k) {
+            const int g8 = t0 + (ht >> 5) + k * (NT / 32);
+            ds_row[k] = g8 < t1 ? MIL_POOL_TILE * g8 + (ht & 31) : -1;
+            ds_sc[k] = -INFINITY;
+#pragma unroll
+            for (int c = 0; c < 4; ++c) ds_h[k][c] = 0.f;
+        }
+#pragma unroll
+        for (int k = 0; k < DSP; ++k)
+            if (ds_row[k] >= 0) {
+                ds_sc[k] = scores[ds_row[k]];
+                ds_h[k][0] = pool.hrow[(size_t)ds_row[k] * 2];
+                ds_h[k][1] = pool.hrow[(size_t)ds_row[k] * 2 + 1];
+            }
+#pragma unroll
+        for (int q = 0; q < JP; ++q)
+#pragma unroll
+            for (int c = 0; c < 4; ++c) wf[q][c] = c < 2 ? pool.Wf[(size_t)c * L + ht + q * NT] : 0.f;
+#pragma unroll
+        for (int c = 0; c < 4; ++c) {
+            bfr[c] = c < 2 ? tl.bf[c] : 0.f;
+            yr[c] = c < 2 ? tl.y[b * 2 + c] : 0.f;
+        }
+        m = -INFINITY;
+#pragma unroll
+        for (int k = 0; k < DSP; ++k) m = fmaxf(m, ds_sc[k]);
+        for (int g8 = t0 + (ht >> 5) + DSP * (NT / 32); g8 < t1; g8 += NT / 32)
+            m = fmaxf(m, scores[MIL_POOL_TILE * g8 + (ht & 31)]);
+    } else {
+        if (ht < nt) { mt = ml[2 * (t0 + ht)]; lt = ml[2 * (t0 + ht) + 1]; }
+#pragma unroll
+        for (int e = 0; e < 8; ++e) {
+            pre[e] = f32x4{0, 0, 0, 0};
+            if (g + e * NG < min(nt, 1024)) pre[e] = *reinterpret_cast<const f32x4*>(pool.partials + (size_t)(t0 + g + e * NG) * L + 4 * c4);
+        }
+        m = mt;
+        for (int t = t0 + ht + NT; t < t1; t += NT) m = fmaxf(m, ml[2 * t]);
+    }
+    m = wave_allmax(m);
+    if (lane == 0) red[hw * 8] = m;
+    __syncthreads();
+    m = red[0];
+#pragma unroll
+    for (int w = 1; w < NW; ++w) m = fmaxf(m, red[w * 8]);
+    float ek[DSP], sums[5] = {0.f, 0.f, 0.f, 0.f, 0.f};
+    if (half == 0) {
+#pragma unroll
+        for (int k = 0; k < DSP; ++k) {
+            ek[k] = ds_row[k] >= 0 ? expf(ds_sc[k] - m) : 0.f;
+            sums[0] += ek[k];
+#pragma unroll
+            for (int c = 0; c < 4; ++c) sums[1 + c] += ek[k] * ds_h[k][c];
+        }
+        for (int g8 = t0 + (ht >> 5) + DSP * (NT / 32); g8 < t1; g8 += NT / 32) {
+            const size_t row = (size_t)(MIL_POOL_TILE * g8 + (ht & 31));
+            const float e = expf(scores[row] - m);
+            sums[0] += e;
+            for (int c = 0; c < 2; ++c) sums[1 + c] += e * pool.hrow[row * 2 + c];
+        }
+#pragma unroll
+        for (int i = 0; i < 5; ++i) sums[i] = wave_allsum(sums[i]);
+        if (lane == 0)
+#pragma unroll
+            for (int i = 0; i < 5; ++i) red[hw * 8 + 1 + i] = sums[i];
+    } else {
+        const float sc0 = ht < nt ? expf(mt - m) : 0.f;
+        float l = lt * sc0;
+        for (int t = t0 + ht + NT; t < t1; t += NT) l += ml[2 * t + 1] * expf(ml[2 * t] - m);
+        l = wave_allsum(l);
+        if (lane == 0) red[hw * 8 + 1] = l;
+        scale_lds[ht] = sc0;
+        for (int k = ht + NT; k < 1024; k += NT) scale_lds[k] = (k < nt) ? expf(ml[2 * (t0 + k)] - m) : 0.f;
+    }
+    __syncthreads();
+    float inv = 0.f;
+    if (half == 0) {
+#pragma unroll
+        for (int i = 0; i < 5; ++i) {
+            float v = red[1 + i];
+#pragma unroll
+            for (int w = 1; w < NW; ++w) v += red[w * 8 + 1 + i];
+            sums[i] = v;
+        }
+        const float l = sums[0];
+        inv = nt > 0 ? 1.0f / l : 0.f;
+        float zz[4], pp[4], dzr[4], lossacc, dot;
+        tail_head_loss(sums, inv, bfr, yr, 2, tl.loss_kind, tl.scale, zz, pp, dzr, lossacc, dot);
+#pragma unroll
+        for (int k = 0; k < DSP; ++k)
+            if (ds_row[k] >= 0) {
+                float gd = 0.f;
+#pragma unroll
+                for (int c = 0; c < 4; ++c) gd += dzr[c] * ds_h[k][c];
+                tl.ds[ds_row[k]] = ek[k] * inv * (gd - dot);
+            }
+        for (int g8 = t0 + (ht >> 5) + DSP * (NT / 32); g8 < t1; g8 += NT / 32) {
+            const size_t row = (size_t)(MIL_POOL_TILE * g8 + (ht & 31));
+            float gd = 0.f;
+            for (int c = 0; c < 2; ++c) gd += dzr[c] * pool.hrow[row * 2 + c];
+            tl.ds[row] = expf(scores[row] - m) * inv * (gd - dot);
+        }
+        if (ht == 0) {
+            tl.lse[b] = nt > 0 ? m + logf(l) : -INFINITY;
+            tl.cdot[b] = dot;
+            tl.loss_bag[b] = lossacc * tl.scale;
+        }
+#pragma unroll
+        for (int c = 0; c < 2; ++c)
+            if (ht == c) {
+                tl.z[b * 2 + c] = zz[c];
+                tl.p[b * 2 + c] = pp[c];
+                tl.dz[b * 2 + c] = dzr[c];
+            }
+#pragma unroll
+        for (int q = 0; q < JP; ++q) {
+            float d = 0.f;
+#pragma unroll
+            for (int c = 0; c < 4; ++c) d += dzr[c] * wf[q][c];
+            tl.dM[(size_t)b * L + ht + q * NT] = d * keepv[q];
+        }
+    } else {
+        float l = red[1];
+#pragma unroll
+        for (int w = 1; w < NW; ++w) l += red[w * 8 + 1];
+        inv = nt > 0 ? 1.0f / l : 0.f;
+    }
+    f32x4 acc = {0, 0, 0, 0};
+    for (int tb = 0; tb < nt; tb += 1024) {
+        if (tb > 0) {
+            __syncthreads();
+            if (half == 1)
+                for (int k = ht; k < 1024; k += NT) scale_lds[k] = (tb + k < nt) ? expf(ml[2 * (t0 + tb + k)] - m) : 0.f;
+            __syncthreads();
+        }
+        if (half == 1) {
+            const int cnt = min(1024, nt - tb);
+            int k = g;
+            if (tb == 0) {
+#pragma unroll
+                for (int e = 0; e < 8; ++e)
+                    if (k + e * NG < cnt) acc += scale_lds[k + e * NG] * pre[e];
+                k += 8 * NG;
+            }
+            for (; k + 7 * NG < cnt; k += 8 * NG) {
+                f32x4 v[8];
+#pragma unroll
+                for (int e = 0; e < 8; ++e)
+                    v[e] = *reinterpret_cast<const f32x4*>(pool.partials + (size_t)(t0 + tb + k + e * NG) * L + 4 * c4);
+#pragma unroll
+                for (int e = 0; e < 8; ++e) acc += scale_lds[k + e * NG] * v[e];
+            }
+            for (; k < cnt; k += NG)
+                acc += scale_lds[k] * *reinterpret_cast<const f32x4*>(pool.partials + (size_t)(t0 + tb + k) * L + 4 * c4);
+        }
+    }
+    if (half == 1) *(lds_f4*)(part_lds + g * L + 4 * c4) = acc;
+    __syncthreads();
+    if (half == 1) {
+#pragma unroll
+        for (int q = 0; q < JP; ++q) {
+            const int j = ht + q * NT;
+            float v = 0.f;
+            for (int gg = 0; gg < NG; ++gg) v += part_lds[gg * L + j];
+            v *= inv;
+            tl.M[(size_t)b * L + j] = v;
+            if (tl.Mdrop != nullptr) tl.Mdrop[(size_t)b * L + j] = v * keepv[q];
+        }
+    }
+    __syncthreads();
+}
+
+template <bool DROP, bool GEN, int NQ>
+__device__ __forceinline__ void gate_fwd_tail(const GateFwdCoord co, const GateKeepWords<DROP, GEN>& kw, const float* scores, int R,
+                                              const GateFwdGen& gen, const GateFwdPool& pool, const GateFwdTail& tl, lds_f32* smem) {
+    asm volatile("s_waitcnt vmcnt(0)" ::: "memory");
+    __syncthreads();
+    lds_i32* closed_lds = (lds_i32*)(smem + GF_TL_CLOSE_OFF);
+    if (co.wave == 0) {
+        int closed = -1;
+        if (co.lane < GF_TM / MIL_POOL_TILE) {
+            const int trow0 = co.row0 + MIL_POOL_TILE * co.lane;
+            if (trow0 < R) {
+                const int bag = pool.tile_map[4 * (trow0 / MIL_POOL_TILE)];
+                const int ntb = tl.bag_tile_off[bag + 1] - tl.bag_tile_off[bag];
+                const int ticket = __hip_atomic_fetch_add(tl.cnt + bag, 1, __ATOMIC_RELAXED, __HIP_MEMORY_SCOPE_AGENT);
+                if (ticket == ntb - 1) {
+                    closed = bag;
+                    __hip_atomic_store(tl.cnt + bag, 0, __ATOMIC_RELAXED, __HIP_MEMORY_SCOPE_AGENT);
+                }
+            }
+            closed_lds[co.lane] = closed;
+        }
+        if (__builtin_amdgcn_ballot_w64(closed >= 0) != 0) {
+            __builtin_amdgcn_fence(__ATOMIC_ACQUIRE, "agent");
+            asm volatile("s_waitcnt vmcnt(0)" ::: "memory");
+        }
+    }
+    __syncthreads();
+#pragma unroll 1
+    for (int i = 0; i < GF_TM / MIL_POOL_TILE; ++i) {
+        const int b = __builtin_amdgcn_readfirstlane(closed_lds[i]);
+        if (b >= 0) gate_fwd_tail_bag<DROP, GEN, NQ>(co, kw, b, scores, gen, pool, tl, smem);
+    }
+    if (blockIdx.x == 0) {
+#pragma unroll 1
+        for (int b = 0; b < tl.B; ++b)
+            if (tl.bag_tile_off[b + 1] == tl.bag_tile_off[b]) gate_fwd_tail_bag<DROP, GEN, NQ>(co, kw, b, scores, gen, pool, tl, smem);
+    }
+}
+
+template <bool DROP, bool GEN, int PQ, bool PW = false, bool TAIL = false>
 __global__ __launch_bounds__(512) void k_gate_fwd2(const float* __restrict__ x, const float* __restrict__ Wv,
                                                    const float* __restrict__ bv, const float* __restrict__ Wu,
                                                    const float* __restrict__ bu, const float* __restrict__ wvec,
                                                    const float* __restrict__ battn, float* __restrict__ scores,
                                                    float* __restrict__ gates, int R, int L,
                                                    const uint32_t* __restrict__ xbits, float xscale, GateFwdGen gen,
-                                                   GateFwdPool pool, const unsigned short* __restrict__ Wp = nullptr) {
+                                                   GateFwdPool pool, const unsigned short* __restrict__ Wp = nullptr,
+                                                   GateFwdTail tl = GateFwdTail{}) {
+    static_assert(!TAIL || PQ > 0, "the fused tail reads what the fused pool pass leaves");
     __shared__ __attribute__((aligned(16))) float smem[gate_fwd2_smem_floats(PW)];
     __shared__ __attribute__((aligned(16))) uint32_t mlds[GEN ? GF_TM * 32 : 4];
     const GateFwdCoord co = gate_fwd_coord(smem, R);
@@ -591,8 +910,9 @@
     else gate_kloop_f32<DROP, GEN>(co, kw, x, Wv, Wu, L, acc);
     GatePoolRows<(PQ > 0 ? PQ : 1)> pv;
     if constexpr (PQ > 0) gate_pool_request_rows(co, x, R, L, pv);
-    gate_fwd_scores_epilogue<DROP>(co, acc, bv, bu, wvec, battn, scores, gates, R, xscale, (lds_f32*)smem, PQ > 0);
-    if constexpr (PQ > 0) gate_fwd_pool_pass<DROP, GEN, PQ>(co, kw, pv, xbits, R, L, xscale, gen, pool, (lds_f32*)smem);
+    gate_fwd_scores_epilogue<DROP, TAIL>(co, acc, bv, bu, wvec, battn, scores, gates, R, xscale, (lds_f32*)smem, PQ > 0);
+    if constexpr (PQ > 0) gate_fwd_pool_pass<DROP, GEN, PQ, TAIL>(co, kw, pv, xbits, R, L, xscale, gen, pool, (lds_f32*)smem);
+    if constexpr (TAIL) gate_fwd_tail<DROP, GEN, PQ>(co, kw, scores, R, gen, pool, tl, (lds_f32*)smem);
 }
 
 #define GS_TM 32
@@ -748,7 +1068,12 @@
     int keep;
     bool pieces;
     bool fused_pool;
+    int C;
 };
+static bool fuse_tail_enabled() {
+    const char* e = getenv("MIL_FUSE_TAIL");
+    return e == nullptr || e[0] != '0';
+}
 int gate_tail_rows(int R, int tiles_per_round) {
     const int tail = R % GF_TM, full = R / GF_TM;
     return (tail >= 1 && tail <= MIL_SMALL_ROWS && full >= tiles_per_round && full % tiles_per_round == 0) ? tail : 0;
@@ -783,6 +1108,7 @@
     p.bits = in.keep == MIL_ROUTE_BITS_NONE || in.keep == MIL_ROUTE_BITS_GIVEN ? in.keep
              : all_fwd2 && L <= 1024 && (L % 128) == 0 ? MIL_ROUTE_BITS_IN_KERNEL : MIL_ROUTE_BITS_GENERATOR;
     p.pool_fused = in.fused_pool && all_fwd2 && L == 512 && (R % 32) == 0;
+    p.tail_fused = p.pool_fused && in.C == 2 && in.save_gates && fuse_tail_enabled();
     p.dw = -1;
     if ((L % 128) == 0) {
         const GateDwPlan d = gate_dw_plan(R, L, ncu);
@@ -798,7 +1124,7 @@
     if (!out || R <= 0 || L <= 0 || (L % GF_BK) != 0 || C <= 0) return MIL_EINVAL;
     if (keep != MIL_ROUTE_BITS_NONE && keep != MIL_ROUTE_BITS_GIVEN) keep = MIL_ROUTE_BITS_GENERATOR;
     (void)bucketed;
-    *out = gate_route_plan(GateRouteIn{R, L, save_gates != 0, keep, pieces != 0, fused_pool != 0}, ncu > 0 ? ncu : MIL_NUM_CU);
+    *out = gate_route_plan(GateRouteIn{R, L, save_gates != 0, keep, pieces != 0, fused_pool != 0, C}, ncu > 0 ? ncu : MIL_NUM_CU);
     return MIL_OK;
 }
 
@@ -807,10 +1133,16 @@
     {k_gate_fwd_r32<false, 1>, k_gate_fwd_r32<false, 2>, k_gate_fwd_r32<false, 3>},
     {k_gate_fwd_r32<true, 1>, k_gate_fwd_r32<true, 2>, k_gate_fwd_r32<true, 3>}};
 using GateFwd2Kernel = decltype(&k_gate_fwd2<false, false, 0, false>);
-static const GateFwd2Kernel GATE_FWD2_KERNELS[3][2][2] = {
-    {{k_gate_fwd2<false, false, 0, false>, k_gate_fwd2<false, false, 0, true>}, {k_gate_fwd2<false, false, 2, false>, k_gate_fwd2<false, false, 2, true>}},
-    {{k_gate_fwd2<true, false, 0, false>, k_gate_fwd2<true, false, 0, true>}, {k_gate_fwd2<true, false, 2, false>, k_gate_fwd2<true, false, 2, true>}},
-    {{k_gate_fwd2<true, true, 0, false>, k_gate_fwd2<true, true, 0, true>}, {k_gate_fwd2<true, true, 2, false>, k_gate_fwd2<true, true, 2, true>}}};
+static const GateFwd2Kernel GATE_FWD2_KERNELS[3][3][2] = {
+    {{k_gate_fwd2<false, false, 0, false>, k_gate_fwd2<false, false, 0, true>},
+     {k_gate_fwd2<false, false, 2, false>, k_gate_fwd2<false, false, 2, true>},
+     {k_gate_fwd2<false, false, 2, false, true>, k_gate_fwd2<false, false, 2, true, true>}},
+    {{k_gate_fwd2<true, false, 0, false>, k_gate_fwd2<true, false, 0, true>},
+     {k_gate_fwd2<true, false, 2, false>, k_gate_fwd2<true, false, 2, true>},
+     {k_gate_fwd2<true, false, 2, false, true>, k_gate_fwd2<true, false, 2, true, true>}},
+    {{k_gate_fwd2<true, true, 0, false>, k_gate_fwd2<true, true, 0, true>},
+     {k_gate_fwd2<true, true, 2, false>, k_gate_fwd2<true, true, 2, true>},
+     {k_gate_fwd2<true, true, 2, false, true>, k_gate_fwd2<true, true, 2, true, true>}}};
 
 static int launch_gate_fwd_r32(const float* x, const float* Wv, const float* bv, const float* Wu, const float* bu,
                                const float* w, const float* b, float* scores, float* gates, int R, int L,
@@ -822,29 +1154,40 @@
     MIL_CHECK_LAUNCH();
     return MIL_OK;
 }
-static void launch_gate_fwd2(bool draw, bool pool_fused, bool pw, dim3 grid, hipStream_t st, const float* x, const float* Wv,
-                             const float* bv, const float* Wu, const float* bu, const float* w, const float* b, float* scores,
-                             float* gates, int R, int L, const uint32_t* xbits, float xs, const GateFwdGen& gen,
-                             const GateFwdPool& pool, const uint16_t* Wp) {
-    hipLaunchKernelGGL(GATE_FWD2_KERNELS[draw ? 2 : xbits ? 1 : 0][pool_fused][pw], grid, dim3(512), 0, st, x, Wv, bv, Wu, bu, w, b,
-                       scores, gates, R, L, xbits, xs, gen, pool, pw ? (const unsigned short*)Wp : nullptr);
+static void launch_gate_fwd2(bool draw, bool pool_fused, bool tail_fused, bool pw, dim3 grid, hipStream_t st, const float* x,
+                             const float* Wv, const float* bv, const float* Wu, const float* bu, const float* w, const float* b,
+                             float* scores, float* gates, int R, int L, const uint32_t* xbits, float xs, const GateFwdGen& gen,
+                             const GateFwdPool& pool, const uint16_t* Wp, const GateFwdTail& tail) {
+    hipLaunchKernelGGL(GATE_FWD2_KERNELS[draw ? 2 : xbits ? 1 : 0][tail_fused ? 2 : pool_fused ? 1 : 0][pw], grid, dim3(512), 0, st, x,
+                       Wv, bv, Wu, bu, w, b, scores, gates, R, L, xbits, xs, gen, pool, pw ? (const unsigned short*)Wp : nullptr, tail);
 }
 
 static int gate_scores_fwd_impl(const float* x, const float* Wv, const float* bv, const float* Wu, const float* bu,
                                 const float* w, const float* b, float* scores, float* gates, int R, int L, int D,
                                 const uint32_t* xbits, float xscale, const GateFwdGen* gen, void* stream,
                                 const GateFwdPool* pool = nullptr, int* fused = nullptr, const int32_t* rows_dev = nullptr,
-                                const TileMapJob* tmap = nullptr, const uint16_t* Wp = nullptr) {
+                                const TileMapJob* tmap = nullptr, const uint16_t* Wp = nullptr, const GateFwdTail* tail = nullptr,
+                                int* tail_fused = nullptr, int B = 0, bool plan_only = false) {
     if (!x || !Wv || !bv || !Wu || !bu || !w || !b || !scores) return MIL_EINVAL;
     if (D != MIL_GATE_D || L <= 0 || (L % GF_BK) != 0 || R < 0) return MIL_EINVAL;
+    if (fused != nullptr) *fused = 0;
+    if (tail_fused != nullptr) *tail_fused = 0;
     if (R == 0) return MIL_OK;
     hipStream_t st = (hipStream_t)stream;
-    if (fused != nullptr) *fused = 0;
     const bool pool_ok = pool != nullptr && fused != nullptr && pool->T * MIL_POOL_TILE == R && pool->tile_map &&
                          pool->partials && pool->Wf && pool->hrow &&
                          (gen ? gen->mbits_out != nullptr : (xbits != nullptr) == (pool->mbits != nullptr));
     const int keep = gen ? MIL_ROUTE_BITS_GENERATOR : xbits ? MIL_ROUTE_BITS_GIVEN : MIL_ROUTE_BITS_NONE;
-    const mil_gate_route p = gate_route_plan(GateRouteIn{R, L, gates != nullptr, keep, Wp != nullptr, pool_ok}, MIL_NUM_CU);
+    const mil_gate_route p = gate_route_plan(GateRouteIn{R, L, gates != nullptr, keep, Wp != nullptr, pool_ok, pool_ok ? 2 : 0}, MIL_NUM_CU);
+    const bool tail_ok = p.tail_fused && tail != nullptr && tail_fused != nullptr && tail->cnt && tail->bag_tile_off && tail->bf &&
+                         tail->y && tail->M && tail->lse && tail->z && tail->p && tail->loss_bag && tail->dz && tail->dM &&
+                         tail->cdot && tail->ds && B > 0 && tail->B == B && pool->T < 64 * B &&
+                         pool_tail_route(pool->T, B, 2, true, false) == MIL_POOL_TAIL_SHORT;
+    if (plan_only) {
+        if (fused != nullptr) *fused = p.pool_fused;
+        if (tail_fused != nullptr) *tail_fused = tail_ok ? 1 : 0;
+        return MIL_OK;
+    }
 
     int rc = MIL_OK;
     if (p.bits == MIL_ROUTE_BITS_GENERATOR) {
@@ -878,8 +1221,9 @@
     } else {
         const GateFwdGen fgen = draw ? *gen : GateFwdGen{};
         const GateFwdPool fpool = p.pool_fused ? *pool : GateFwdPool{};
-        launch_gate_fwd2(draw, p.pool_fused, p.main == MIL_ROUTE_MAIN_FWD2_PW, grid, st, x, Wv, bv, Wu, bu, w, b, scores, gates, Rm, L,
-                         xbits, xs, fgen, fpool, Wp);
+        launch_gate_fwd2(draw, p.pool_fused, tail_ok, p.main == MIL_ROUTE_MAIN_FWD2_PW, grid, st, x, Wv, bv, Wu, bu, w, b, scores, gates,
+                         Rm, L, xbits, xs, fgen, fpool, Wp, tail_ok ? *tail : GateFwdTail{});
+        if (tail_ok) *tail_fused = 1;
     }
     if (p.pool_fused) *fused = 1;
     MIL_CHECK_LAUNCH();
@@ -945,7 +1289,7 @@
                        const float* b, float* scores, float* gates, int R, int L, int draw, uint32_t* xbits, float xscale,
                        uint32_t* mbits, float mscale, int B, uint64_t seed, uint64_t mseed, uint64_t offset,
                        const int32_t* offset_dev, const int32_t* tile_map, int T, float* partials, const float* Wf, float* hrow,
-                       int* fused, void* stream, const uint16_t* Wp) {
+                       int* fused, void* stream, const uint16_t* Wp, const GateFwdTail* tail, int* tail_fused, int plan_only) {
     if (draw && (!xbits || !mbits || (L % 64) != 0 || B <= 0)) return MIL_EINVAL;
     GateFwdPool pl{};
     pl.tile_map = tile_map;
@@ -957,7 +1301,7 @@
     pl.mscale = mscale;
     const GateFwdGen gen = gate_fwd_gen(xbits, mbits, B, seed, mseed, offset, offset_dev);
     return gate_scores_fwd_impl(x, Wv, bv, Wu, bu, w, b, scores, gates, R, L, MIL_GATE_D, draw ? nullptr : xbits, xscale,
-                                draw ? &gen : nullptr, stream, &pl, fused, nullptr, nullptr, Wp);
+                                draw ? &gen : nullptr, stream, &pl, fused, nullptr, nullptr, Wp, tail, tail_fused, B, plan_only != 0);
 }
 
 __global__ __launch_bounds__(256) void k_gate_pieces(const float* __restrict__ Wv, const float* __restrict__ Wu,
diff --git a/llm-guided-multimodal-mil_amd/csrc/head_loss.hip b/llm-guided-multimodal-mil_amd/csrc/head_loss.hip
--- a/llm-guided-multimodal-mil_amd/csrc/head_loss.hip
+++ b/llm-guided-multimodal-mil_amd/csrc/head_loss.hip
@@ -1,4 +1,4 @@
-#include "mil_common.h"
+#include "mil_internal.h"
 
 template <int NT>
 __device__ __forceinline__ float block_allsum_nt(float v, float* red) {
@@ -1008,6 +1008,14 @@
     }
 }
 
+int pool_tail_route(int T, int B, int C, bool have_h, bool have_ws) {
+    const char* tail_env = getenv("MIL_TAIL_H");
+    const bool short_chain = C <= 4 && have_h && !(tail_env != nullptr && tail_env[0] == '0');
+    if (!short_chain) return MIL_POOL_TAIL_MERGE_FIRST;
+    if (have_ws && T >= 64 * B && B <= 8 && (tail_env == nullptr || tail_env[0] != '1')) return MIL_POOL_TAIL_TWO_LAUNCH;
+    return MIL_POOL_TAIL_SHORT;
+}
+
 extern "C" size_t mil_pool_tail_workspace_floats(int B) { return (size_t)(B > 0 ? B : 0) * TAIL_S_MAX * 8; }
 
 extern "C" int mil_pool_merge_head_ws(const float* partials, const int32_t* bag_tile_off, int T, int B, int L,
@@ -1022,9 +1030,9 @@
     if (ds && (!y || !tile_map || !scores || !hrow)) return MIL_EINVAL;
     if (!(L == 256 || L == 512 || L == 768 || L == 1024) || C <= 0 || C > 32 || B < 0) return MIL_EINVAL;
     if (B == 0) return MIL_OK;
-    const char* tail_env = getenv("MIL_TAIL_H");
-    const bool short_chain = C <= 4 && y && ds && hrow && !(tail_env != nullptr && tail_env[0] == '0');
-    if (short_chain && tail_ws != nullptr && T >= 64 * B && B <= 8 && (tail_env == nullptr || tail_env[0] != '1')) {
+    const int route = pool_tail_route(T, B, C, y && ds && hrow, tail_ws != nullptr);
+    const bool short_chain = route != MIL_POOL_TAIL_MERGE_FIRST;
+    if (route == MIL_POOL_TAIL_TWO_LAUNCH) {
         int S = (T / B + 31) / 32;
         if (S > TAIL_S_MAX) S = TAIL_S_MAX;
         hipLaunchKernelGGL(k_tail_stats, dim3(B, S), dim3(256), 0, (hipStream_t)stream, bag_tile_off, tile_map, scores, hrow, C, S,
diff --git a/llm-guided-multimodal-mil_amd/csrc/mil_internal.h b/llm-guided-multimodal-mil_amd/csrc/mil_internal.h
--- a/llm-guided-multimodal-mil_amd/csrc/mil_internal.h
+++ b/llm-guided-multimodal-mil_amd/csrc/mil_internal.h
@@ -4,15 +4,30 @@
 #define MIL_HIDDEN __attribute__((visibility("hidden")))
 
 MIL_HIDDEN int gate_tail_rows(int R, int tiles_per_round);
+struct GateFwdTail {
+    int32_t* cnt;
+    int B;
+    const int32_t* bag_tile_off;
+    const float* bf;
+    const float* y;
+    float scale;
+    int loss_kind;
+    float *M, *Mdrop, *lse, *z, *p, *loss_bag, *dz, *dM, *cdot, *ds;
+};
 int gate_fwd_with_pool(const float* x, const float* Wv, const float* bv, const float* Wu, const float* bu, const float* w,
                        const float* b, float* scores, float* gates, int R, int L, int draw, uint32_t* xbits, float xscale,
                        uint32_t* mbits, float mscale, int B, uint64_t seed, uint64_t mseed, uint64_t offset,
                        const int32_t* offset_dev, const int32_t* tile_map, int T, float* partials, const float* Wf, float* hrow,
-                       int* fused, void* stream, const uint16_t* Wp);
+                       int* fused, void* stream, const uint16_t* Wp, const GateFwdTail* tail, int* tail_fused, int plan_only = 0);
 int gate_fwd_rows_dev(const float* x, const float* Wv, const float* bv, const float* Wu, const float* bu, const float* w,
                       const float* b, float* scores, float* gates, int R, int L, int draw, uint32_t* xbits, float xscale,
                       uint32_t* mbits, int B, uint64_t seed, uint64_t mseed, uint64_t offset, const int32_t* offset_dev,
                       const int32_t* rows_dev, void* stream, const TileMapJob* tmap, const uint16_t* Wp);
+
+#define MIL_POOL_TAIL_MERGE_FIRST 0
+#define MIL_POOL_TAIL_SHORT 1
+#define MIL_POOL_TAIL_TWO_LAUNCH 2
+MIL_HIDDEN int pool_tail_route(int T, int B, int C, bool have_h, bool have_ws);
 
 struct GateDwPlan {
     int dw, S, kc;
diff --git a/llm-guided-multimodal-mil_amd/csrc/step.hip b/llm-guided-multimodal-mil_amd/csrc/step.hip
--- a/llm-guided-multimodal-mil_amd/csrc/step.hip
+++ b/llm-guided-multimodal-mil_amd/csrc/step.hip
@@ -29,11 +29,13 @@
     return e != nullptr && e[0] != '0';
 }
 
-extern "C" int mil_abi_version(void) { return 12; }
-
-extern "C" int mil_image_only_step_run(const mil_image_only_step* a, void* stream) {
+extern "C" int mil_abi_version(void) { return 13; }
+
+static int step_run_impl(const mil_image_only_step* a, void* stream, int* plan_tail_fused) {
     int rc = step_check(a);
     if (rc != MIL_OK) return rc;
+    const bool plan = plan_tail_fused != nullptr;
+    if (plan) *plan_tail_fused = 0;
     const uint32_t st = a->stages;
     const bool train = a->train != 0;
     const bool grads = a->y != nullptr;
@@ -44,7 +46,7 @@
     const bool use_h = a->hrow != nullptr && grads && a->C <= 4;
     const uint16_t* Wp = (!a->x_bf16 && a->Wp) ? a->Wp : nullptr;
     bool adam_in_reduce = false;
-    int pool_fused = 0;
+    int pool_fused = 0, tail_fused = 0;
 
     const bool draw_in_fwd = (st & MIL_STAGE_DROPBITS) && (st & MIL_STAGE_GATE_FWD) && train && !a->x_bf16;
     const bool gen_launch = (st & MIL_STAGE_DROPBITS) && train && !draw_in_fwd;
@@ -52,6 +54,9 @@
     const TileMapJob tmj{a->bag_len_dev, a->B, const_cast<int32_t*>(a->tile_map), const_cast<int32_t*>(a->bag_tile_off), a->rows_dev,
                          a->T};
     const bool tmap_with_fwd = want_tmap && (st & MIL_STAGE_GATE_FWD) && !a->x_bf16 && a->rows_dev != nullptr && !gen_launch;
+    const bool fwd_pool_branch = (st & MIL_STAGE_GATE_FWD) && !a->x_bf16 && (st & MIL_STAGE_POOL) && (st & MIL_STAGE_POOL_FUSED) &&
+                                 use_h && a->C == 2 && !a->bag_len_dev && (!train || draw_in_fwd) && fuse_pool_enabled();
+    if (plan && !fwd_pool_branch) return MIL_OK;
     if (want_tmap && gen_launch) {
         rc = dropout_keep_bits_pair_tilemap(a->xbits, a->R, a->mbits, a->B, a->L, a->seed, a->seed ^ 0x9E3779B97F4A7C15ull,
                                             a->offset, a->offset_dev, tmj, stream);
@@ -78,13 +83,37 @@
             rc = mil_gate_scores_fwd_bf16((const uint16_t*)a->x, a->Wv16, a->bv, a->Wu16, a->bu, a->w, a->b, a->scores,
                                           g16 ? nullptr : gates, a->R, a->L, MIL_GATE_D, (grads && g16) ? a->gates16 : nullptr,
                                           xbits, xscale, stream);
-        else if ((st & MIL_STAGE_POOL) && (st & MIL_STAGE_POOL_FUSED) && use_h && a->C == 2 && !a->bag_len_dev &&
-                 (!train || draw_in_fwd) && fuse_pool_enabled())
+        else if (fwd_pool_branch) {
+            GateFwdTail tl{};
+            const bool want_tail = (st & MIL_STAGE_TAIL) && a->tail_cnt != nullptr;
+            if (want_tail) {
+                tl.cnt = a->tail_cnt;
+                tl.B = a->B;
+                tl.bag_tile_off = a->bag_tile_off;
+                tl.bf = a->bf;
+                tl.y = a->y;
+                tl.scale = a->loss_scale;
+                tl.loss_kind = a->loss_kind;
+                tl.M = a->M;
+                tl.Mdrop = train ? a->Mdrop : nullptr;
+                tl.lse = a->lse;
+                tl.z = a->logits;
+                tl.p = a->prob;
+                tl.loss_bag = a->loss_bag;
+                tl.dz = a->dz;
+                tl.dM = a->dM;
+                tl.cdot = a->cdot;
+                tl.ds = a->ds;
+            }
             rc = gate_fwd_with_pool((const float*)a->x, a->Wv, a->bv, a->Wu, a->bu, a->w, a->b, a->scores, gates, a->R, a->L,
                                     draw_in_fwd ? 1 : 0, a->xbits, xscale, a->mbits, mscale, a->B, a->seed,
                                     a->seed ^ 0x9E3779B97F4A7C15ull, a->offset, a->offset_dev, a->tile_map, a->T, a->partials,
-                                    a->Wf, a->hrow, &pool_fused, stream, Wp);
-        else if (a->bag_len_dev && a->rows_dev)
+                                    a->Wf, a->hrow, &pool_fused, stream, Wp, want_tail ? &tl : nullptr, &tail_fused, plan ? 1 : 0);
+            if (plan) {
+                *plan_tail_fused = tail_fused;
+                return rc;
+            }
+        } else if (a->bag_len_dev && a->rows_dev)
             rc = gate_fwd_rows_dev((const float*)a->x, a->Wv, a->bv, a->Wu, a->bu, a->w, a->b, a->scores, gates, a->R, a->L,
                                    draw_in_fwd ? 1 : 0, a->xbits, xscale, a->mbits, a->B, a->seed, a->seed ^ 0x9E3779B97F4A7C15ull,
                                    a->offset, a->offset_dev, a->rows_dev, stream, tmap_with_fwd ? &tmj : nullptr, Wp);
@@ -116,7 +145,7 @@
         }
         if (rc != MIL_OK) return rc;
     }
-    if (st & MIL_STAGE_TAIL) {
+    if ((st & MIL_STAGE_TAIL) && !tail_fused) {
         rc = mil_pool_merge_head_ws(a->partials, a->bag_tile_off, a->T, a->B, a->L, a->Wf, a->bf, a->C, a->y, a->loss_scale, a->M,
                                     a->lse, a->logits, a->prob, grads ? a->loss_bag : nullptr, grads ? a->dz : nullptr,
                                     grads ? a->dM : nullptr, grads ? a->cdot : nullptr, use_h ? a->tile_map : nullptr,
@@ -216,6 +245,13 @@
         }
     }
     return MIL_OK;
+}
+
+extern "C" int mil_image_only_step_run(const mil_image_only_step* a, void* stream) { return step_run_impl(a, stream, nullptr); }
+
+extern "C" int mil_image_only_step_tail_fused(const mil_image_only_step* a, int* tail_fused) {
+    if (!tail_fused) return MIL_EINVAL;
+    return step_run_impl(a, nullptr, tail_fused);
 }
 
 extern "C" int mil_image_only_step_time(const mil_image_only_step* a, uint32_t stages, int warm, int iters, float* ms_out,
diff --git a/llm-guided-multimodal-mil_amd/trainer.py b/llm-guided-multimodal-mil_amd/trainer.py
--- a/llm-guided-multimodal-mil_amd/trainer.py
+++ b/llm-guided-multimodal-mil_amd/trainer.py
@@ -104,6 +104,29 @@
         if t is None or t.numel() < numel or t.dtype != dtype:
             t = self._ws[name] = torch.empty(max(1, numel), device=self.device, dtype=dtype)
         return t
+
+    def _tickets(self, B: int) -> torch.Tensor:
+        n = (max(1, B) + 3) // 4 * 4
+        t = self._ws.get("tail_cnt")
+        if t is None or t.numel() < n:
+            t = self._ws["tail_cnt"] = torch.zeros(n, device=self.device, dtype=torch.int32)
+        return t
+
+    def _stages(self, stages: int, keep=None) -> int:
+        keep = self._keep if keep is None else keep
+        if getattr(keep[2], "aligned32", False) and (stages & _lib.STAGE_GATE_FWD) and (stages & _lib.STAGE_POOL):
+            stages |= _lib.STAGE_POOL_FUSED
+        return stages
+
+    def tail_fused(self, a=None, stages: int = _lib.STAGE_ALL) -> bool:
+        a = self._args if a is None else a
+        if a is None:
+            return False
+        q = _lib.ImageOnlyStep.from_buffer_copy(a)
+        q.stages = self._stages(stages)
+        out = ctypes.c_int(0)
+        _lib.checked().mil_image_only_step_tail_fused(ctypes.byref(q), ctypes.byref(out))
+        return bool(out.value)
 
     def _shadows(self):
         fp = self.fp
@@ -188,6 +211,8 @@
                       Mdrop=self._buf("Mdrop", B * L), loss_bag=self._buf("loss_bag", B), dz=self._buf("dz", B * C),
                       dM=self._buf("dM", B * L), cdot=self._buf("cdot", B))
             a.dw_ws_floats = st["dw_ws"].numel()
+            if not b16:
+                st.update(tail_cnt=self._tickets(B))
         if train:
             st.update(xbits=self._buf("xbits", R * (L // 32), torch.int32), mbits=self._buf("mbits", B * (L // 32), torch.int32))
         for k, t in st.items():
@@ -224,10 +249,7 @@
         self._sync_lr()
         if a.Wp and self._wp_version != self._param_version:
             self._pieces()
-        keep = self._keep if keep is None else keep
-        if getattr(keep[2], "aligned32", False) and (stages & _lib.STAGE_GATE_FWD) and (stages & _lib.STAGE_POOL):
-            stages |= _lib.STAGE_POOL_FUSED
-        a.stages = stages
+        a.stages = self._stages(stages, keep)
         a.accumulate = int(self._micro > 0)
         a.lr = self.lr
         a.adam_step = self.step_count + 1
@@ -376,7 +398,10 @@
             groups.append(("gate_fwd_with_pool_fused", fwd | S.STAGE_POOL | S.STAGE_POOL_FUSED))
         else:
             groups += [("gate_fwd", fwd), ("pool_partial", S.STAGE_POOL)]
-        groups.append(("merge_head_loss_ds", S.STAGE_TAIL))
+        if fused_pool and self.tail_fused(a):
+            groups[-1] = ("gate_fwd_with_pool_fused", groups[-1][1] | S.STAGE_TAIL)
+        else:
+            groups.append(("merge_head_loss_ds", S.STAGE_TAIL))
         collective = self.world > 1 or self.force_collectives
         if a.x_bf16 and collective:
             groups += [("gate_bwd_dw_reduce_head", S.STAGE_GATE_BWD | S.STAGE_REDUCE), ("adam", S.STAGE_ADAM)]
```

Result: no change. 187,700 bags/s (-0.1%).
